# r3fang/alignTools.C

Hardware: AMD Instinct MI355X
Metric: GCUPS (DP cell updates/s), SW affine-gap 150bp pairs (higher is better)
Workload: dtype int16; 1 GPU; C2: local affine-gap, 100000 x (150x150 bp) pairs per GPU, uniform ACGT, m=2 u=-2 o=-5 e=-2, scores+tracebacks+rendered strings; pairs_per_gpu=100000, l1=150, l2=150, bits_per_base=2, streams=3, parallelism=pairs sharded over 1 GPU(s), one process per GPU

## Files before the change

aligntools/c_amd/csrc/at_hip.hip:

```cpp
#include "at_launch.h"
#include "at_classes.h"
#include "at_ragplan.h"
#include "at_pack.hip.h"
#include "at_render.hip.h"
#include "at_myers.hip.h"
#include "at_search.hip.h"
#include "at_revcomp.hip.h"
#include "at_cigar.hip.h"
#include "at_edit_tb.hip.h"
#include "at_infix.hip.h"
#include "at_scan.hip.h"
#include "at_scanhits.hip.h"
#include "at_pairhits.hip.h"
#include "../../../include/aligntools_hip.h"

#include <algorithm>
#include <chrono>
#include <condition_variable>
#include <mutex>
#include <cstdarg>
#include <cstdio>
#include <cstdlib>
#include <cstring>
#include <functional>
// ... 921 lines not shown
			HIP_TRY(h, hipGetLastError());
			snprintf(h->cfg, sizeof h->cfg, "myers-infix bits=2 words/lane=%d (64 pairs/wave) lds=%zuB waves/cu<=%d grid=%lld", w, lds, occ, grid);
			return AT_OK;
		}
		if (!d_ops || !d_ops_off || !d_nops) return fail(h, AT_ERR_ARG, "traceback wanted but ops buffers are NULL");
		const long long slab_words = (long long)std::max(max_len2, 1) * w * 128;
		const long long cap = env_ll("AT_WS_CAP_MB", 16384) << 20;
		if (slab_words * 4 > cap)
			return fail(h, AT_ERR_NOMEM, "edit infix alignments: one work item needs %lld workspace bytes (cap %lld)", slab_words * 4, cap);
		const long long per_cu = std::max(1LL, std::min<long long>(occ, env_ll("AT_WAVES_PER_CU", 16)));
		const long long grid = std::max(1LL, std::min<long long>(std::min<long long>((npairs + 63) / 64, per_cu * h->ncu), cap / (slab_words * 4)));
		{
			void *p = h->d_ws; size_t have = h->ws_bytes;
			int rc = grow(h, &p, &have, (size_t)(grid * slab_words * 4), "ws");
			h->d_ws = (uint32_t *)p; h->ws_bytes = have;
			if (rc) return rc;
		}
		ia.ops = d_ops; ia.ops_off = (const long long *)d_ops_off;
		ia.slab = h->d_ws; ia.slab_words = slab_words;
		ia.anchor_end = h->infix_anchor;
		if (int rcq = ensure_queue(h, stream)) return rcq;
		ia.m.queue = h->d_queue;
		hipLaunchKernelGGL(fn, dim3((unsigned)grid), dim3(64), lds, stream, ia);
		HIP_TRY(h, hipGetLastError());
		snprintf(h->cfg, sizeof h->cfg, "myers-infix-tb bits=2 words/lane=%d (64 pairs/wave) lds=%zuB slab=%lldB waves/cu<=%lld grid=%lld", w, lds,
		         slab_words * 4, per_cu, grid);
		return AT_OK;
	}

	int thresh16 = 0, ts = 0;
	if (!uniform_shape && !rag && !only_if && ap_n == 0 && npairs >= 4096 && !d_order && kmode <= at::K_FITJ &&
	    env_ll("AT_AUTO_UNIFORM", 1) && (bits == 8 || scores_fit_byte(h, mode)) &&
	    packed_ok(h, mode, bits, max_len1, max_len2, 4, &thresh16)) {
		int *flag = h->d_rflag + 8;
		HIP_TRY(h, hipMemsetAsync(flag, 0xff, 4, stream));
		const unsigned cg = (unsigned)std::min<int64_t>((npairs + 255) / 256, 4LL * h->ncu);
		hipLaunchKernelGGL(at::at_check_uniform, dim3(cg), dim3(256), 0, stream, d_len1, d_len2, (long long)npairs, max_len1, max_len2, flag);
		int rc = align_device(h, mode, npairs, d_seq, bits, d_woff1, d_len1, d_woff2, d_len2, max_len1, max_len2, 1, want_traceback,
		                      d_score, d_end_i, d_end_j, d_state, d_ops, d_ops_off, d_nops, stream_, 0, 0, nullptr, 0, flag, -1);
		if (rc) return rc;
		std::string packed_cfg = h->cfg;
		rc = align_device(h, mode, npairs, d_seq, bits, d_woff1, d_len1, d_woff2, d_len2, max_len1, max_len2, 0, want_traceback,
		                  d_score, d_end_i, d_end_j, d_state, d_ops, d_ops_off, d_nops, stream_, 0, 0, nullptr, 0, flag, 0);
		if (rc) return rc;
		snprintf(h->cfg, sizeof h->cfg, "auto: [%.140s] if every pair is %dx%d, else [%.120s]", packed_cfg.c_str(), max_len1, max_len2,
		         std::string(h->cfg).c_str());
		return AT_OK;
	}
	if ((uniform_shape || rag) && ap_n == 0) {
		if (packed_ok(h, mode, bits, max_len1, max_len2, 4, &thresh16)) ts = 4;
		else if ((!rag || kmode == at::K_OVERLAP) && packed_ok(h, mode, bits, max_len1, max_len2, 2, &thresh16)) ts = 2;
		if (kmode == at::K_OVERLAP && (!tb || getenv("AT_NO_PACKED_OVERLAP"))) ts = 0;
	}
	if (rag && (!ts || (kmode > at::K_FITJ && !(kmode == at::K_OVERLAP && rag == 64)) || max_len1 > at::rag_group_top(rag) || !d_order))
		return fail(h, AT_ERR_ARG, "ragged packed launch outside its domain");
	Layout16 P;
	if (ts) {
		P = layout16_for(tb, kmode == at::K_FITJ, max_len1, max_len2, ts, rag, kmode == at::K_OVERLAP, kmode,
		                 rag && kmode == at::K_OVERLAP ? at::class_rows(at::kClassOvl, max_len1) : 0);
		const double min_rounds = getenv("AT_PACKED_MIN_ROUNDS") ? atof(getenv("AT_PACKED_MIN_ROUNDS")) : 1.0;
		if (!rag && P.g == 64 && (double)((npairs + 1) / 2) < min_rounds * 12.0 * h->ncu) ts = 0;
		if (P.words >= (1LL << 24)) { if (rag) return fail(h, AT_ERR_ARG, "ragged packed launch outside its domain (slot too large)"); ts = 0; }
		Layout16 PTq = P;
		const bool tailq = !rag && !only_if && P.g <= 16 && kmode != at::K_OVERLAP && env_ll("AT_TAIL_SPLIT", 1);
		if (tailq) PTq = layout16_for(tb, kmode == at::K_FITJ, max_len1, max_len2, ts, at::AT_TAIL_G, false, kmode, at::at_tail_k(P.g, P.k));
		if (ts && !packed16_kernel_exists(kmode, P, tb, ts, bits, rag, tailq ? &PTq : nullptr)) {
			if (rag) return fail(h, AT_ERR_ARG, "ragged packed launch outside its domain (frame too long for LDS)");
			ts = 0;
		}
	}
	bool two_pass = false;
	int tp_split = 0;
	const char *ck_note = "";
	const long long tp_mode = env_ll("AT_TWO_PASS", 1);
	if (ts && tb && !rag && kmode <= at::K_FITJ && tp_mode) {
		Layout16 P2 = layout16_for(false, kmode == at::K_FITJ, max_len1, max_len2, ts, 0, false, kmode, 0, 1);
		const bool narrow_default = P2.g == 8 && tp_split_narrow_default(kmode, max_len1, max_len2);
		const bool split_default = P2.g == 64 || narrow_default;
		const bool split_want = env_ll("AT_TP_SPLIT", split_default ? 1 : 0) && at_pick_walk16(kmode, P2.g, P2.k, ts, bits);
		const int split_req = split_want && !h->ck_alloc_failed && !h->ck_skip ? 1 : 0;
		if (split_want && !split_req) ck_note = h->ck_skip ? " [one work item's checkpoints exceed AT_CK_CAP_MB: no separate pass 2]"
		                                                   : " [checkpoint buffer unavailable on this handle: no separate pass 2]";
		if ((P2.g == 64 || tp_mode >= 2 || (split_req && narrow_default)) && (long long)P2.g * P2.k >= max_len1 && at_pick16_tp(kmode, P2.g, P2.k, ts, bits) &&
		    choose_store(P2.off_ptr, 1, true) == 1) {
			two_pass = true;
			tp_split = split_req;
			if (tp_split) P2 = layout16_for(false, kmode == at::K_FITJ, max_len1, max_len2, ts, 0, false, kmode, 0, 2);
			P = P2;
		}
	}
	if (ts) {
		const int per_wave = 2 * (64 / P.g);
		const bool tail_ok = !rag && !only_if && P.g <= 16 && kmode != at::K_OVERLAP && env_ll("AT_TAIL_SPLIT", 1) &&
		                     (!tp_split || P.g == 8);
		Layout16 PT = P;
		if (tail_ok) PT = layout16_for(tb && !two_pass, kmode == at::K_FITJ, max_len1, max_len2, ts, at::AT_TAIL_G, false, kmode, at::at_tail_k(P.g, P.k), two_pass ? (tp_split ? 2 : 1) : 0);
		TpLayout tpm{}, tpt{};
		if (two_pass) { tpm = tp_layout(P, kmode, max_len2, tp_split != 0); tpt = tp_layout(PT, kmode, max_len2, tp_split != 0); }
		int64_t piece = npairs;
		int64_t brow_words = 0;
		if (tp_split) {
			const long long cap = env_ll("AT_CK_CAP_MB", 8192) << 20;
			brow_words = (tpm.brow_words + 63) & ~63LL;
			const long long tail_reserve = tail_ok ? 16LL * h->ncu * tpt.words * 4 : 0;
			const long long items = (cap - tail_reserve - brow_words * 4) / (tpm.words * 4 + 16LL * per_wave);
			if (items < 1) {
				struct SkipForThisCall {
					at_handle *h;
					explicit SkipForThisCall(at_handle *hh) : h(hh) { h->ck_skip = true; }
					~SkipForThisCall() { h->ck_skip = false; }
				} skip(h);
				return align_device(h, mode, npairs, d_seq, bits, d_woff1, d_len1, d_woff2, d_len2, max_len1, max_len2, uniform_shape, want_traceback,
				                    d_score, d_end_i, d_end_j, d_state, d_ops, d_ops_off, d_nops, stream_, ap_n, ap_first, d_order, rag, only_if, only_val);
			}
			piece = std::min<int64_t>(npairs, items * per_wave);
			const long long forced = env_ll("AT_CK_PIECE_PAIRS", 0);
			if (forced > 0) piece = std::min<int64_t>(piece, std::max<long long>(1, forced / per_wave) * per_wave);
		}
		auto walk_lane_words = [&](const Layout16 &L) -> long long {
			const int cb = at::ck_steps(L.g);
			return L.k * (cb / 4) + (kmode == at::K_FITJ ? (L.k + 3) / 4 * (cb / 4) : 0);
		};
		auto walk_lds = [&](const Layout16 &L, bool ptr_in_lds) -> size_t {
			const int cb = at::ck_steps(L.g), nsm = kmode == at::K_FITJ ? L.nsm : 0;
			return (size_t)((nsm + 1) / 2 * 2 + (L.k > 16 ? 0 : (cb + 1) * 128) + (ptr_in_lds ? 64 * walk_lane_words(L) : 0)) * 4;
		};
		std::string cfg_first, walk_last;
		for (int64_t first = 0; first < npairs; first += piece) {
		const int64_t np = std::min<int64_t>(piece, npairs - first);
		Sweep16Args b;
		memset(&b, 0, sizeof b);
		b.npairs = np; b.seq = d_seq;
		b.woff1 = (const long long *)d_woff1 + first; b.woff2 = (const long long *)d_woff2 + first;
		b.len1 = d_len1 + first; b.len2 = d_len2 + first;
		b.l1 = max_len1; b.l2 = max_len2;
		const int sc = 1 << ts;
		b.m16 = h->m * sc; b.u16 = h->u * sc; b.o16 = h->o * sc; b.e16 = h->e * sc; b.g16 = h->j * sc; b.thresh16 = thresh16;
		if (kmode == at::K_FITJ) {
			int rcs = ensure_sitemask(h, max_len2, stream);
			if (rcs) return rcs;
			b.sitemask = h->d_sitemask;
		}
		b.score = d_score + first; b.end_i = d_end_i ? d_end_i + first : nullptr; b.end_j = d_end_j ? d_end_j + first : nullptr;
		b.state = d_state ? d_state + first : nullptr;
		b.ops = d_ops; b.ops_off = d_ops_off ? (const long long *)d_ops_off + first : nullptr; b.nops = d_nops ? d_nops + first : nullptr;
		b.order = rag ? d_order : nullptr;
		b.only_if = only_if; b.only_val = only_val;
		b.off_refb = P.off_refb; b.off_bound = P.off_bound; b.ptr_lanes = P.ptr_lanes; b.off_sm = P.off_sm; b.nsm = P.nsm;
		Plan pl;
		char tag16[128];
		snprintf(tag16, sizeof tag16, "packed16 x%d bits=%d %dx%d-lane groups (%d pairs/wave)%s", 1 << ts, bits, 64 / P.g, P.g, per_wave,
		         rag ? " ragged frames" : "");
		if (two_pass) snprintf(tag16 + strlen(tag16), sizeof tag16 - strlen(tag16), " two-pass%s ck=%d", tp_split ? " (walk kernel)" : "", at::ck_steps(P.g));
		auto pick = [&](int st) {
			if (two_pass) return st == 1 ? at_pick16_tp(kmode, P.g, P.k, ts, bits, tp_split) : (at_sweep16_fn) nullptr;
			return rag ? at_pick16_rag(kmode, P.g, P.k, st, tb, bits) : at_pick16(kmode, P.g, P.k, ts, st, tb, bits);
		};
		const long long nwork = (np + per_wave - 1) / per_wave;
		int rc = plan_launch(h, tag16, P.k, nwork, std::max(P.off_ptr, PT.off_ptr),
		                     tp_split ? 64 : two_pass ? std::max(tpm.words, tpt.words) : std::max(P.words - P.off_ptr, PT.words - PT.off_ptr), &pl, stream,
		                     [&](int st) { return (const void *)pick(st); }, P.g < 64 || rag || two_pass);
		if (rc) return rc;
		if (tp_split) {
			const long long rsv = env_ll("AT_TP_RESERVE", 0) * h->ncu;
			if (rsv > 0 && pl.grid > rsv && nwork > pl.grid - rsv) {
				pl.grid = std::max<long long>(h->ncu, pl.grid - rsv);
				cfg_append(h, " (AT_TP_RESERVE: sweep grid=%lld)", pl.grid);
			}
		}
		int64_t n_tail = 0;
		if (tail_ok && nwork > pl.grid) {
			const long long sliver = nwork % pl.grid;
			if (sliver > 0 && sliver * 4 <= pl.grid) n_tail = np - (nwork - sliver) * per_wave;
		}
		Sweep16Args bt = b;
		bt.npairs = 0;
		const int64_t nm = np - n_tail;
		if (n_tail > 0) {
			b.npairs = nm;
			bt.npairs = n_tail;
			bt.woff1 += nm; bt.woff2 += nm; bt.len1 += nm; bt.len2 += nm;
			bt.score += nm;
			if (bt.end_i) bt.end_i += nm;
			if (bt.end_j) bt.end_j += nm;
			if (bt.state) bt.state += nm;
			if (bt.ops_off) bt.ops_off += nm;
			if (bt.nops) bt.nops += nm;
			bt.off_refb = PT.off_refb; bt.off_bound = PT.off_bound; bt.ptr_lanes = PT.ptr_lanes; bt.off_sm = PT.off_sm; bt.nsm = PT.nsm;
		}
		b.off_ptr = pl.off_ptr; b.ws = pl.ws; b.ws_slot_words = pl.slot_words; b.queue = h->d_queue;
		bt.off_ptr = pl.store == 1 ? 0 : PT.off_ptr; bt.ws = pl.ws; bt.ws_slot_words = pl.slot_words; bt.queue = h->d_queue;
		if (two_pass) {
			if (pl.store != 1) return fail(h, AT_ERR_RANGE, "two-pass tracebacks need the s2 windows in LDS (store=%d)", pl.store);
			b.off_brow = tpm.off_brow; b.off_rck = tpm.off_rck; b.off_cck = tpm.off_cck; b.off_rptr = tpm.off_rptr; b.off_rjpl = tpm.off_rjpl;
			bt.off_brow = tpt.off_brow; bt.off_rck = tpt.off_rck; bt.off_cck = tpt.off_cck; bt.off_rptr = tpt.off_rptr; bt.off_rjpl = tpt.off_rjpl;
		}
		if (tp_split) {
			const long long n_main_items = (nm + per_wave - 1) / per_wave, n_tail_items = (n_tail + 2 * (64 / at::AT_TAIL_G) - 1) / (2 * (64 / at::AT_TAIL_G));
			const long long end_words = ((np * 4) + 63) & ~63LL;
			const size_t need = (size_t)(brow_words + end_words + n_main_items * tpm.words + n_tail_items * tpt.words) * 4;
			void *pc = h->d_ck; size_t have = h->ck_bytes;
			const std::string err_before = h->err, g_err_before = g_err;
			rc = grow(h, &pc, &have, need, "ck");
			h->d_ck = (uint32_t *)pc; h->ck_bytes = have;
			if (rc && first == 0) {
				h->ck_alloc_failed = true;
				rc = align_device(h, mode, npairs, d_seq, bits, d_woff1, d_len1, d_woff2, d_len2, max_len1, max_len2, uniform_shape, want_traceback,
				                  d_score, d_end_i, d_end_j, d_state, d_ops, d_ops_off, d_nops, stream_, ap_n, ap_first, d_order, rag, only_if, only_val);
				if (rc == AT_OK) {
					snprintf(h->err, sizeof h->err, "%s", err_before.c_str());
					snprintf(g_err, sizeof g_err, "%s", g_err_before.c_str());
				}
				return rc;
			}
			if (rc) return rc;
			b.ck_brow = h->d_ck; bt.ck_brow = h->d_ck;
			b.tp_end = (int4 *)(h->d_ck + brow_words); bt.tp_end = b.tp_end + nm;
			b.ck = h->d_ck + brow_words + end_words; b.ck_item_words = tpm.words;
			bt.ck = b.ck + n_main_items * tpm.words; bt.ck_item_words = tpt.words;
		}
		at_sweep16_fn fn16 = pick(pl.store);
		if (!fn16 || (P.g != 64 && pl.store == 2)) return fail(h, AT_ERR_RANGE, "no packed kernel for this shape (rows/lane=%d, store=%d)", P.k, pl.store);
		if (pl.dyn_lds > 48 * 1024)
			HIP_TRY(h, hipFuncSetAttribute((const void *)fn16, hipFuncAttributeMaxDynamicSharedMemorySize, (int)pl.dyn_lds));
		hipLaunchKernelGGL(fn16, dim3((unsigned)pl.grid), dim3(64), pl.dyn_lds, stream, b, bt);
		HIP_TRY(h, hipGetLastError());
		if (tp_split && !(AT_DIAG_SWEEP_ONLY && env_ll("AT_DIAG_NO_WALK_KERNEL", 0))) {
			const bool teams = env_ll("AT_WALK_TEAMS", P.g == 64 ? 1 : 0) && at_pick_walk16(kmode, P.g, P.k, ts, bits, 1);
			at_walk16_fn wf = at_pick_walk16(kmode, P.g, P.k, ts, bits, teams);
			if (!wf) return fail(h, AT_ERR_RANGE, "no walk kernel for %d-lane groups x %d rows", P.g, P.k);
			const size_t lds = std::max(walk_lds(P, true), tail_ok ? walk_lds(PT, true) : 0);
			if (lds > 48 * 1024) HIP_TRY(h, hipFuncSetAttribute((const void *)wf, hipFuncAttributeMaxDynamicSharedMemorySize, (int)lds));
			const long long wcap = env_ll("AT_WALK_WAVES_PER_CU", 0);
			const long long wmain = std::max<long long>(1, wcap > 0 ? std::min<long long>((nm + 127) / 128, wcap * h->ncu) : (nm + 127) / 128);
			HIP_TRY(h, hipMemsetAsync(h->d_queue + 8, 0, 16, stream));
			const int tpw = 64 / at_walk16_team_lanes(P.g);
			const long long wteams = ((nm + 1) / 2 + tpw - 1) / tpw;
			hipLaunchKernelGGL(wf, dim3((unsigned)((teams ? wteams : wmain) + (n_tail + 127) / 128)), dim3(64), lds, stream, b, bt);
			char wnote[128];
			snprintf(wnote, sizeof wnote, " [walkers: %lld wavefronts%s for %lld alignments]", teams ? wteams : wmain, teams ? " of teams" : "", (long long)nm);
			cfg_append(h, "%s", wnote);
			walk_last = wnote;
			HIP_TRY(h, hipGetLastError());
		}
		if (n_tail > 0)
			cfg_append(h, " + last %lld pairs as 32-lane items (rows/lane=%d)", (long long)n_tail, PT.k);
		if (first == 0) cfg_first = h->cfg;
		}
		if (piece < npairs) snprintf(h->cfg, sizeof h->cfg, "%.360s; in pieces of %lld pairs%s%s", cfg_first.c_str(), (long long)piece,
		                              walk_last.empty() ? "" : "; last piece", walk_last.c_str());
		if (ck_note[0]) cfg_append(h, "%s", ck_note);
		return AT_OK;
	}

	if (edit_tb) {
		const size_t lds = at::myers_window_bytes(64, max_len2);
		if (h->u != 1) return fail(h, AT_ERR_DOMAIN, "edit alignments need the unit mismatch cost: u = %d, not 1", h->u);
		if (bits != 2) return fail(h, AT_ERR_DOMAIN, "edit alignments need a 2-bit batch: some base is not one of ACGT");
		if (max_len1 > 1024) return fail(h, AT_ERR_DOMAIN, "edit alignments: max_len1 = %d exceeds 1024", max_len1);
		if (lds > 60 * 1024) return fail(h, AT_ERR_DOMAIN, "edit alignments: max_len2 = %d exceeds 3792 (64 windows of packed words in 60 KB of LDS)", max_len2);
		const int w = at::class_rows(at::kMyersLaneWords, max_len1);
		at_edit_tb_fn fn = at_pick_edit_tb(w);
		if (!fn) return fail(h, AT_ERR_ARG, "no edit alignment kernel for %d words per lane", w);
		const long long slab_words = (long long)std::max(max_len2, 1) * w * 128;
		const long long cap = env_ll("AT_WS_CAP_MB", 16384) << 20;
		if (slab_words * 4 > cap)
			return fail(h, AT_ERR_NOMEM, "edit alignments: one work item needs %lld workspace bytes (cap %lld)", slab_words * 4, cap);
		int occ = 0;
		if (hipOccupancyMaxActiveBlocksPerMultiprocessor(&occ, (const void *)fn, 64, lds) != hipSuccess || occ <= 0) occ = 8;
		const long long per_cu = std::max(1LL, std::min<long long>(occ, env_ll("AT_WAVES_PER_CU", 16)));
		const long long grid = std::max(1LL, std::min<long long>(std::min<long long>((npairs + 63) / 64, per_cu * h->ncu), cap / (slab_words * 4)));
		{
			void *p = h->d_ws; size_t have = h->ws_bytes;
			int rc = grow(h, &p, &have, (size_t)(grid * slab_words * 4), "ws");
			h->d_ws = (uint32_t *)p; h->ws_bytes = have;
			if (rc) return rc;
		}
		at::EditTbArgs ea;
		memset(&ea, 0, sizeof ea);
		ea.m.npairs = npairs; ea.m.seq = d_seq;
		ea.m.woff1 = (const long long *)d_woff1; ea.m.woff2 = (const long long *)d_woff2; ea.m.len1 = d_len1; ea.m.len2 = d_len2;
		ea.m.max_l1 = max_len1; ea.m.max_l2 = max_len2;
		ea.m.score = d_score; ea.m.end_i = d_end_i; ea.m.end_j = d_end_j; ea.m.state = d_state; ea.m.nops = d_nops;
		ea.m.order = d_order;
		ea.ops = d_ops; ea.ops_off = (const long long *)d_ops_off;
		ea.slab = h->d_ws; ea.slab_words = slab_words;
		if (int rcq = ensure_queue(h, stream)) return rcq;
		ea.m.queue = h->d_queue;
		hipLaunchKernelGGL(fn, dim3((unsigned)grid), dim3(64), lds, stream, ea);
		HIP_TRY(h, hipGetLastError());
		snprintf(h->cfg, sizeof h->cfg, "myers-tb bits=2 words/lane=%d (64 pairs/wave) lds=%zuB slab=%lldB waves/cu<=%lld grid=%lld", w, lds,
		         slab_words * 4, per_cu, grid);
		return AT_OK;
	}

	auto myers_windows = [&](int n) { return at::myers_window_bytes(n, max_len2); };
	if (kmode == at::K_EDIT && h->u == 1 && bits == 2 && max_len1 <= 32768 && myers_windows(2) <= 60 * 1024 && env_ll("AT_MYERS", 1)) {
		const long long lane_max = env_ll("AT_MYERS_LANE_MAX", 1024);
		const bool per_lane = max_len1 <= lane_max && max_len1 <= 1024 && myers_windows(64) <= 60 * 1024 &&
		                      (max_len1 <= 256 || npairs >= env_ll("AT_MYERS_LANE_MIN_PAIRS", 16384)) && env_ll("AT_MYERS_GROUP", 1) == 1;
		const int g = per_lane ? 1 : max_len1 <= 256 && myers_windows(8) <= 60 * 1024 ? 8 : 32;
		const int w = per_lane ? at::class_rows(at::kMyersLaneWords, max_len1) : at::class_rows(at::kMyersGroupWords, max_len1);
		at_myers_fn fn = at_pick_myers(w, g);
		const int per_wave = 64 / g;
		at::MyersArgs m;
		memset(&m, 0, sizeof m);
		m.npairs = npairs; m.seq = d_seq;
		m.woff1 = (const long long *)d_woff1; m.woff2 = (const long long *)d_woff2; m.len1 = d_len1; m.len2 = d_len2;
		m.max_l1 = max_len1; m.max_l2 = max_len2;
// ... 1940 lines not shown
```

aligntools/c_amd/csrc/at_k16.hip:

```cpp
#include "at_launch.h"
#define AT_DECL(b)                                                                 \
	at_sweep16_fn at_pick16_g64_ts4_b##b(int kmode, int k, int store, bool tb);    \
	at_sweep16_fn at_pick16_g64_ts2_b##b(int kmode, int k, int store, bool tb);    \
	at_sweep16_fn at_pick16_g16_b##b(int kmode, int k, int store, bool tb);        \
	at_sweep16_fn at_pick16_g32_b##b(int kmode, int k, int store, bool tb);        \
	at_sweep16_fn at_pick16_g8_b##b(int kmode, int k, int store, bool tb);         \
	at_sweep16_fn at_pick16_g4_b##b(int kmode, int k, int store, bool tb);         \
	at_sweep16_fn at_pick16_rag_impl_b##b(int k, int store, bool tb);                \
	at_sweep16_fn at_pick16_rag8a_b##b(int kmode, int k, int store, bool tb);      \
	at_sweep16_fn at_pick16_rag8b_b##b(int kmode, int k, int store, bool tb);      \
	at_sweep16_fn at_pick16_rag8c_b##b(int kmode, int k, int store, bool tb);      \
	at_sweep16_fn at_pick16_rag8d_b##b(int kmode, int k, int store, bool tb);      \
	at_sweep16_fn at_pick16_rag16_b##b(int kmode, int k, int store, bool tb);      \
	at_sweep16_fn at_pick16_rag16b_b##b(int kmode, int k, int store, bool tb);     \
	at_sweep16_fn at_pick16_rag32_b##b(int kmode, int k, int store, bool tb);      \
	at_sweep16_fn at_pick16_ragovl_b##b(int k, int store);                           \
	at_sweep16_fn at_pick16_tp8_b##b(int kmode, int k, int split);                             \
	at_sweep16_fn at_pick16_tp64_b##b(int kmode, int k, int ts, int split);                  \
	at_walk16_fn at_pick_walk16_g8_b##b(int kmode, int g, int k, bool teams);                    \
	at_walk16_fn at_pick_walk16_g64_b##b(int kmode, int k, int ts, bool teams);
AT_DECL(2)
AT_DECL(8)
#undef AT_DECL
at_sweep16_fn at_pick16(int kmode, int g, int k, int ts, int store, bool tb, int bits)
{
	if (g == 8) return ts != 4 ? nullptr : bits == 8 ? at_pick16_g8_b8(kmode, k, store, tb) : at_pick16_g8_b2(kmode, k, store, tb);
	if (g == 4) return ts != 4 ? nullptr : bits == 8 ? at_pick16_g4_b8(kmode, k, store, tb) : at_pick16_g4_b2(kmode, k, store, tb);
	if (g == 32) return ts != 4 ? nullptr : bits == 8 ? at_pick16_g32_b8(kmode, k, store, tb) : at_pick16_g32_b2(kmode, k, store, tb);
	if (bits == 8) {
		if (g == 16) return ts == 4 ? at_pick16_g16_b8(kmode, k, store, tb) : nullptr;
		return ts == 4 ? at_pick16_g64_ts4_b8(kmode, k, store, tb) : at_pick16_g64_ts2_b8(kmode, k, store, tb);
	}
	if (g == 16) return ts == 4 ? at_pick16_g16_b2(kmode, k, store, tb) : nullptr;
	return ts == 4 ? at_pick16_g64_ts4_b2(kmode, k, store, tb) : at_pick16_g64_ts2_b2(kmode, k, store, tb);
}
at_sweep16_fn at_pick16_rag(int kmode, int g, int k, int store, bool tb, int bits)
{
	if (g == 8) {
		if (k == 6 || k == 8) return bits == 8 ? at_pick16_rag8d_b8(kmode, k, store, tb) : at_pick16_rag8d_b2(kmode, k, store, tb);
		if (bits == 8) return k >= 19 ? at_pick16_rag8c_b8(kmode, k, store, tb) : k >= 13 ? at_pick16_rag8b_b8(kmode, k, store, tb) : at_pick16_rag8a_b8(kmode, k, store, tb);
		return k >= 19 ? at_pick16_rag8c_b2(kmode, k, store, tb) : k >= 13 ? at_pick16_rag8b_b2(kmode, k, store, tb) : at_pick16_rag8a_b2(kmode, k, store, tb);
	}
	if (kmode == at::K_OVERLAP) return g != 64 || !tb ? nullptr : bits == 8 ? at_pick16_ragovl_b8(k, store) : at_pick16_ragovl_b2(k, store);
	if (g == 32) return bits == 8 ? at_pick16_rag32_b8(kmode, k, store, tb) : at_pick16_rag32_b2(kmode, k, store, tb);
	if (g != 16) return nullptr;
	if (k >= 16) return bits == 8 ? at_pick16_rag16b_b8(kmode, k, store, tb) : at_pick16_rag16b_b2(kmode, k, store, tb);
	if (kmode == at::K_LOCAL) return bits == 8 ? at_pick16_rag_impl_b8(k, store, tb) : at_pick16_rag_impl_b2(k, store, tb);
	return bits == 8 ? at_pick16_rag16_b8(kmode, k, store, tb) : at_pick16_rag16_b2(kmode, k, store, tb);
}
at_sweep16_fn at_pick16_tp(int kmode, int g, int k, int ts, int bits, int split)
{
	if (g == 8) return ts != 4 ? nullptr : bits == 8 ? at_pick16_tp8_b8(kmode, k, split) : at_pick16_tp8_b2(kmode, k, split);
	if (g == 64) return bits == 8 ? at_pick16_tp64_b8(kmode, k, ts, split) : at_pick16_tp64_b2(kmode, k, ts, split);
	return nullptr;
}
int at_walk16_team_lanes_b2();
int at_walk16_team_lanes8_b2();
int at_walk16_team_lanes(int g) { return g == 64 ? at_walk16_team_lanes_b2() : at_walk16_team_lanes8_b2(); }
at_walk16_fn at_pick_walk16(int kmode, int g, int k, int ts, int bits, int teams)
{
	if (g == 64) return bits == 8 ? at_pick_walk16_g64_b8(kmode, k, ts, teams != 0) : at_pick_walk16_g64_b2(kmode, k, ts, teams != 0);
	if (ts != 4) return nullptr;
	return bits == 8 ? at_pick_walk16_g8_b8(kmode, g, k, teams != 0) : at_pick_walk16_g8_b2(kmode, g, k, teams != 0);
}
```

aligntools/c_amd/csrc/at_k16_g16a.hip:

```cpp
#include "at_launch.h"
template <int MODE, int K>
static at_sweep16_fn q3(int store, bool tb)
{
	if (!tb) return at::at_sweep16<MODE, 16, K, 4, true, true, false, false, AT_BITS16>;
	if (store == 0) return at::at_sweep16<MODE, 16, K, 4, true, true, true, false, AT_BITS16>;
	return at::at_sweep16<MODE, 16, K, 4, true, false, true, false, AT_BITS16>;
}
template <int MODE>
static at_sweep16_fn q2(int k, int store, bool tb)
{
	switch (k) {
	case 4: return q3<MODE, 4>(store, tb);
	case 5: return q3<MODE, 5>(store, tb);
	case 6: return q3<MODE, 6>(store, tb);
	case 7: return q3<MODE, 7>(store, tb);
	default: return nullptr;
	}
}
at_sweep16_fn AT_NAME(at_pick16_g16a)(int kmode, int k, int store, bool tb)
{
	switch (kmode) {
	case at::K_GLOBAL: return q2<at::K_GLOBAL>(k, store, tb);
	case at::K_LOCAL: return q2<at::K_LOCAL>(k, store, tb);
	case at::K_FITJ: return q2<at::K_FITJ>(k, store, tb);
	default: return q2<at::K_FIT>(k, store, tb);
	}
}
```

aligntools/c_amd/csrc/at_k16_g16b.hip:

```cpp
#include "at_launch.h"
template <int MODE, int K>
static at_sweep16_fn q3(int store, bool tb)
{
	if (!tb) return at::at_sweep16<MODE, 16, K, 4, true, true, false, false, AT_BITS16>;
	if (store == 0) return at::at_sweep16<MODE, 16, K, 4, true, true, true, false, AT_BITS16>;
	return at::at_sweep16<MODE, 16, K, 4, true, false, true, false, AT_BITS16>;
}
template <int MODE>
static at_sweep16_fn q2(int k, int store, bool tb)
{
	switch (k) {
	case 10: return q3<MODE, 10>(store, tb);
	case 13: return q3<MODE, 13>(store, tb);
	default: return nullptr;
	}
}
at_sweep16_fn AT_NAME(at_pick16_g16b)(int kmode, int k, int store, bool tb)
{
	switch (kmode) {
	case at::K_GLOBAL: return q2<at::K_GLOBAL>(k, store, tb);
	case at::K_LOCAL: return q2<at::K_LOCAL>(k, store, tb);
	case at::K_FITJ: return q2<at::K_FITJ>(k, store, tb);
	default: return q2<at::K_FIT>(k, store, tb);
	}
}
```

aligntools/c_amd/csrc/at_k16_g16c.hip:

```cpp
#include "at_launch.h"
template <int MODE, int K>
static at_sweep16_fn r3(bool tb)
{
	if (!tb) return at::at_sweep16<MODE, 16, K, 4, true, true, false, false, AT_BITS16>;
	return at::at_sweep16<MODE, 16, K, 4, true, false, true, false, AT_BITS16>;
}
template <int MODE>
static at_sweep16_fn r2(int k, bool tb)
{
	switch (k) {
	case 16: return r3<MODE, 16>(tb);
	case 19: return r3<MODE, 19>(tb);
	default: return nullptr;
	}
}
at_sweep16_fn AT_NAME(at_pick16_g16c)(int kmode, int k, int store, bool tb)
{
	if (tb && store != 1) return nullptr;
	switch (kmode) {
	case at::K_GLOBAL: return r2<at::K_GLOBAL>(k, tb);
	case at::K_LOCAL: return r2<at::K_LOCAL>(k, tb);
	case at::K_FITJ: return r2<at::K_FITJ>(k, tb);
	default: return r2<at::K_FIT>(k, tb);
	}
}
```

aligntools/c_amd/csrc/at_k16_g32.hip:

```cpp
#include "at_launch.h"
template <int MODE, int K>
static at_sweep16_fn g3(int store, bool tb)
{
	if (!tb) return at::at_sweep16<MODE, 32, K, 4, true, true, false, false, AT_BITS16>;
	if (store == 0) return at::at_sweep16<MODE, 32, K, 4, true, true, true, false, AT_BITS16>;
	return at::at_sweep16<MODE, 32, K, 4, true, false, true, false, AT_BITS16>;
}
template <int MODE>
static at_sweep16_fn g2(int k, int store, bool tb)
{
	switch (k) {
	case 7: return g3<MODE, 7>(store, tb);
	case 8: return g3<MODE, 8>(store, tb);
	case 10: return g3<MODE, 10>(store, tb);
	case 13: return g3<MODE, 13>(store, tb);
	default: return nullptr;
	}
}
at_sweep16_fn AT_NAME(at_pick16_g32b)(int kmode, int k, int store, bool tb);
at_sweep16_fn AT_NAME(at_pick16_g32)(int kmode, int k, int store, bool tb)
{
	if (k == 12 || k >= 16) return AT_NAME(at_pick16_g32b)(kmode, k, store, tb);
	switch (kmode) {
	case at::K_GLOBAL: return g2<at::K_GLOBAL>(k, store, tb);
	case at::K_LOCAL: return g2<at::K_LOCAL>(k, store, tb);
	case at::K_FITJ: return g2<at::K_FITJ>(k, store, tb);
	default: return g2<at::K_FIT>(k, store, tb);
	}
}
```

aligntools/c_amd/csrc/at_k16_g32b.hip:

```cpp
#include "at_launch.h"
template <int MODE, int K>
static at_sweep16_fn s3(bool tb)
{
	if (!tb) return at::at_sweep16<MODE, 32, K, 4, true, true, false, false, AT_BITS16>;
	return at::at_sweep16<MODE, 32, K, 4, true, false, true, false, AT_BITS16>;
}
template <int MODE>
static at_sweep16_fn s2(int k, bool tb)
{
	switch (k) {
	case 12: return s3<MODE, 12>(tb);
	case 16: return s3<MODE, 16>(tb);
	case 19: return s3<MODE, 19>(tb);
	default: return nullptr;
	}
}
at_sweep16_fn AT_NAME(at_pick16_g32b)(int kmode, int k, int store, bool tb)
{
	if (tb && store != 1) return nullptr;
	switch (kmode) {
	case at::K_GLOBAL: return s2<at::K_GLOBAL>(k, tb);
	case at::K_LOCAL: return s2<at::K_LOCAL>(k, tb);
	case at::K_FITJ: return s2<at::K_FITJ>(k, tb);
	default: return s2<at::K_FIT>(k, tb);
	}
}
```

aligntools/c_amd/csrc/at_k16_g4.hip:

```cpp
#include "at_launch.h"
template <int MODE, int K>
static at_sweep16_fn f3(bool tb)
{
	if (!tb) return at::at_sweep16<MODE, 4, K, 4, true, true, false, false, AT_BITS16>;
	return at::at_sweep16<MODE, 4, K, 4, true, false, true, false, AT_BITS16>;
}
template <int MODE>
static at_sweep16_fn f2(int k, bool tb)
{
	switch (k) {
	case 9: return f3<MODE, 9>(tb);
	case 10: return f3<MODE, 10>(tb);
	case 13: return f3<MODE, 13>(tb);
	default: return nullptr;
	}
}
at_sweep16_fn AT_NAME(at_pick16_g4b)(int kmode, int k, int store, bool tb);
at_sweep16_fn AT_NAME(at_pick16_g4)(int kmode, int k, int store, bool tb)
{
	if (k >= 16) return AT_NAME(at_pick16_g4b)(kmode, k, store, tb);
	if (tb && store != 1) return nullptr;
	switch (kmode) {
	case at::K_GLOBAL: return f2<at::K_GLOBAL>(k, tb);
	case at::K_LOCAL: return f2<at::K_LOCAL>(k, tb);
	case at::K_FITJ: return f2<at::K_FITJ>(k, tb);
	default: return f2<at::K_FIT>(k, tb);
	}
}
```

aligntools/c_amd/csrc/at_k16_g4b.hip:

```cpp
#include "at_launch.h"
template <int MODE, int K>
static at_sweep16_fn f3(bool tb)
{
	if (!tb) return at::at_sweep16<MODE, 4, K, 4, true, true, false, false, AT_BITS16>;
	return at::at_sweep16<MODE, 4, K, 4, true, false, true, false, AT_BITS16>;
}
template <int MODE>
static at_sweep16_fn f2(int k, bool tb)
{
	switch (k) {
	case 16: return f3<MODE, 16>(tb);
	case 19: return f3<MODE, 19>(tb);
	default: return nullptr;
	}
}
at_sweep16_fn AT_NAME(at_pick16_g4b)(int kmode, int k, int store, bool tb)
{
	if (tb && store != 1) return nullptr;
	switch (kmode) {
	case at::K_GLOBAL: return f2<at::K_GLOBAL>(k, tb);
	case at::K_LOCAL: return f2<at::K_LOCAL>(k, tb);
	case at::K_FITJ: return f2<at::K_FITJ>(k, tb);
	default: return f2<at::K_FIT>(k, tb);
	}
}
```

aligntools/c_amd/csrc/at_k16_g64.hip:

```cpp
#include "at_launch.h"
template <int MODE, int K>
static at_sweep16_fn p3(int store, bool tb)
{
	if (!tb) return store < 2 ? at::at_sweep16<MODE, 64, K, 4, true, true, false, false, AT_BITS16> : at::at_sweep16<MODE, 64, K, 4, false, false, false, false, AT_BITS16>;
	if (store == 0) return at::at_sweep16<MODE, 64, K, 4, true, true, true, false, AT_BITS16>;
	if (store == 1) return at::at_sweep16<MODE, 64, K, 4, true, false, true, false, AT_BITS16>;
	return at::at_sweep16<MODE, 64, K, 4, false, false, true, false, AT_BITS16>;
}
template <int MODE>
static at_sweep16_fn p2(int k, int store, bool tb)
{
	switch (k) {
	case 1: return p3<MODE, 1>(store, tb);
	case 2: return p3<MODE, 2>(store, tb);
	case 3: return p3<MODE, 3>(store, tb);
	default: return p3<MODE, 4>(store, tb);
	}
}
at_sweep16_fn AT_NAME(at_pick16_g64_ts4)(int kmode, int k, int store, bool tb)
{
	switch (kmode) {
	case at::K_GLOBAL: return p2<at::K_GLOBAL>(k, store, tb);
	case at::K_LOCAL: return p2<at::K_LOCAL>(k, store, tb);
	case at::K_FITJ: return p2<at::K_FITJ>(k, store, tb);
	default: return p2<at::K_FIT>(k, store, tb);
	}
}
```

aligntools/c_amd/csrc/at_k16_g8a.hip:

```cpp
#include "at_launch.h"
template <int MODE, int K>
static at_sweep16_fn h3(bool tb)
{
	if (!tb) return at::at_sweep16<MODE, 8, K, 4, true, true, false, false, AT_BITS16>;
	return at::at_sweep16<MODE, 8, K, 4, true, false, true, false, AT_BITS16>;
}
template <int MODE>
static at_sweep16_fn h2(int k, bool tb)
{
	switch (k) {
	case 5: return h3<MODE, 5>(tb);
	case 7: return h3<MODE, 7>(tb);
	case 10: return h3<MODE, 10>(tb);
	default: return nullptr;
	}
}
at_sweep16_fn AT_NAME(at_pick16_g8a)(int kmode, int k, int store, bool tb)
{
	if (tb && store != 1) return nullptr;
	switch (kmode) {
	case at::K_GLOBAL: return h2<at::K_GLOBAL>(k, tb);
	case at::K_LOCAL: return h2<at::K_LOCAL>(k, tb);
	case at::K_FITJ: return h2<at::K_FITJ>(k, tb);
	default: return h2<at::K_FIT>(k, tb);
	}
}
```

aligntools/c_amd/csrc/at_k16_g8b.hip:

```cpp
#include "at_launch.h"
template <int MODE, int K>
static at_sweep16_fn h3(bool tb)
{
	if (!tb) return at::at_sweep16<MODE, 8, K, 4, true, true, false, false, AT_BITS16>;
	return at::at_sweep16<MODE, 8, K, 4, true, false, true, false, AT_BITS16>;
}
template <int MODE>
static at_sweep16_fn h2(int k, bool tb)
{
	switch (k) {
	case 13: return h3<MODE, 13>(tb);
	case 16: return h3<MODE, 16>(tb);
	default: return nullptr;
	}
}
at_sweep16_fn AT_NAME(at_pick16_g8b)(int kmode, int k, int store, bool tb)
{
	if (tb && store != 1) return nullptr;
	switch (kmode) {
	case at::K_GLOBAL: return h2<at::K_GLOBAL>(k, tb);
	case at::K_LOCAL: return h2<at::K_LOCAL>(k, tb);
	case at::K_FITJ: return h2<at::K_FITJ>(k, tb);
	default: return h2<at::K_FIT>(k, tb);
	}
}
```

aligntools/c_amd/csrc/at_k16_g8c.hip:

```cpp
#include "at_launch.h"
template <int MODE, int K>
static at_sweep16_fn h3(bool tb)
{
	if (!tb) return at::at_sweep16<MODE, 8, K, 4, true, true, false, false, AT_BITS16>;
	return at::at_sweep16<MODE, 8, K, 4, true, false, true, false, AT_BITS16>;
}
template <int MODE>
static at_sweep16_fn h2(int k, bool tb)
{
	switch (k) {
	case 19: return h3<MODE, 19>(tb);
	default: return nullptr;
	}
}
at_sweep16_fn AT_NAME(at_pick16_g8c)(int kmode, int k, int store, bool tb)
{
	if (tb && store != 1) return nullptr;
	switch (kmode) {
	case at::K_GLOBAL: return h2<at::K_GLOBAL>(k, tb);
	case at::K_LOCAL: return h2<at::K_LOCAL>(k, tb);
	case at::K_FITJ: return h2<at::K_FITJ>(k, tb);
	default: return h2<at::K_FIT>(k, tb);
	}
}
```

aligntools/c_amd/csrc/at_k16_g8d.hip:

```cpp
#include "at_launch.h"
template <int MODE, int K>
static at_sweep16_fn h3(bool tb)
{
	if (!tb) return at::at_sweep16<MODE, 8, K, 4, true, true, false, false, AT_BITS16>;
	return at::at_sweep16<MODE, 8, K, 4, true, false, true, false, AT_BITS16>;
}
template <int MODE>
static at_sweep16_fn h2(int k, bool tb)
{
	switch (k) {
	case 6: return h3<MODE, 6>(tb);
	case 8: return h3<MODE, 8>(tb);
	default: return nullptr;
	}
}
at_sweep16_fn AT_NAME(at_pick16_g8d)(int kmode, int k, int store, bool tb)
{
	if (tb && store != 1) return nullptr;
	switch (kmode) {
	case at::K_GLOBAL: return h2<at::K_GLOBAL>(k, tb);
	case at::K_LOCAL: return h2<at::K_LOCAL>(k, tb);
	case at::K_FITJ: return h2<at::K_FITJ>(k, tb);
	default: return h2<at::K_FIT>(k, tb);
	}
}
```

aligntools/c_amd/csrc/at_k16_rag.hip:

```cpp
#include "at_launch.h"
template <int K>
static at_sweep16_fn r3(int store, bool tb)
{
	if (!tb) return at::at_sweep16<at::K_LOCAL, 16, K, 4, true, true, false, true, AT_BITS16>;
	if (store == 0) return at::at_sweep16<at::K_LOCAL, 16, K, 4, true, true, true, true, AT_BITS16>;
	return at::at_sweep16<at::K_LOCAL, 16, K, 4, true, false, true, true, AT_BITS16>;
}
at_sweep16_fn AT_NAME(at_pick16_rag_impl)(int k, int store, bool tb)
{
	switch (k) {
	case 4: return r3<4>(store, tb);
	case 5: return r3<5>(store, tb);
	case 6: return r3<6>(store, tb);
	case 7: return r3<7>(store, tb);
	case 10: return r3<10>(store, tb);
	case 13: return r3<13>(store, tb);
	default: return nullptr;
	}
}
```

aligntools/c_amd/csrc/at_k16_rag16b.hip:

```cpp
#include "at_launch.h"
template <int MODE, int K>
static at_sweep16_fn x3(bool tb)
{
	if (!tb) return at::at_sweep16<MODE, 16, K, 4, true, true, false, true, AT_BITS16>;
	return at::at_sweep16<MODE, 16, K, 4, true, false, true, true, AT_BITS16>;
}
template <int MODE>
static at_sweep16_fn x2(int k, bool tb)
{
	switch (k) {
	case 16: return x3<MODE, 16>(tb);
	case 19: return x3<MODE, 19>(tb);
	default: return nullptr;
	}
}
at_sweep16_fn AT_NAME(at_pick16_rag16b)(int kmode, int k, int store, bool tb)
{
	if (tb && store != 1) return nullptr;
	switch (kmode) {
	case at::K_GLOBAL: return x2<at::K_GLOBAL>(k, tb);
	case at::K_LOCAL: return x2<at::K_LOCAL>(k, tb);
	case at::K_FITJ: return x2<at::K_FITJ>(k, tb);
	default: return x2<at::K_FIT>(k, tb);
	}
}
```

aligntools/c_amd/csrc/at_k16_rag32.hip:

```cpp
#include "at_launch.h"
template <int MODE, int K>
static at_sweep16_fn y3(bool tb)
{
	if (!tb) return at::at_sweep16<MODE, 32, K, 4, true, true, false, true, AT_BITS16>;
	return at::at_sweep16<MODE, 32, K, 4, true, false, true, true, AT_BITS16>;
}
template <int MODE>
static at_sweep16_fn y2(int k, bool tb)
{
	switch (k) {
	case 10: return y3<MODE, 10>(tb);
	case 12: return y3<MODE, 12>(tb);
	case 13: return y3<MODE, 13>(tb);
	case 16: if constexpr (MODE == at::K_LOCAL || MODE == at::K_GLOBAL) return y3<MODE, 16>(tb); else return nullptr;
	case 19: if constexpr (MODE == at::K_LOCAL) return y3<MODE, 19>(tb); else return nullptr;
	default: return nullptr;
	}
}
at_sweep16_fn AT_NAME(at_pick16_rag32)(int kmode, int k, int store, bool tb)
{
	if (tb && store != 1) return nullptr;
	switch (kmode) {
	case at::K_GLOBAL: return y2<at::K_GLOBAL>(k, tb);
	case at::K_LOCAL: return y2<at::K_LOCAL>(k, tb);
	case at::K_FITJ: return y2<at::K_FITJ>(k, tb);
	default: return y2<at::K_FIT>(k, tb);
	}
}
at_sweep16_fn AT_NAME(at_pick16_ragovl)(int k, int store)
{
	if (store != 1) return nullptr;
	if (k == 16) return at::at_sweep16<at::K_OVERLAP, 64, 16, 2, true, false, true, true, AT_BITS16>;
	if (k == 4) return at::at_sweep16<at::K_OVERLAP, 64, 4, 2, true, false, true, true, AT_BITS16>;
	return nullptr;
}
```

aligntools/c_amd/csrc/at_k16_tp.hip:

```cpp
#include "at_launch.h"
template <int MODE>
static at_sweep16_fn tp8(int k, int split)
{
	if (k != 19) return nullptr;
	return split ? at::at_sweep16<MODE, 8, 19, 4, true, false, false, false, AT_BITS16, at::ck_steps(8), 1>
	             : at::at_sweep16<MODE, 8, 19, 4, true, false, false, false, AT_BITS16, at::ck_steps(8)>;
}
at_sweep16_fn AT_NAME(at_pick16_tp8)(int kmode, int k, int split)
{
	switch (kmode) {
	case at::K_GLOBAL: return tp8<at::K_GLOBAL>(k, split);
	case at::K_LOCAL: return tp8<at::K_LOCAL>(k, split);
	case at::K_FITJ: return tp8<at::K_FITJ>(k, split);
	default: return tp8<at::K_FIT>(k, split);
	}
}
```

aligntools/c_amd/csrc/at_k16_tp64.hip:

```cpp
#include "at_launch.h"
template <int MODE, int TS>
static at_sweep16_fn tp64(int k, int split)
{
	switch (k) {
	case 16: return split ? at::at_sweep16<MODE, 64, 16, TS, true, false, false, false, AT_BITS16, at::ck_steps(64), 1>
	                      : at::at_sweep16<MODE, 64, 16, TS, true, false, false, false, AT_BITS16, at::ck_steps(64)>;
	default: return nullptr;
	}
}
at_sweep16_fn AT_NAME(at_pick16_tp64)(int kmode, int k, int ts, int split)
{
	if (ts == 2) {
		switch (kmode) {
		case at::K_GLOBAL: return tp64<at::K_GLOBAL, 2>(k, split);
		case at::K_LOCAL: return tp64<at::K_LOCAL, 2>(k, split);
		case at::K_FIT: return tp64<at::K_FIT, 2>(k, split);
		default: return nullptr;
		}
	}
	switch (kmode) {
	case at::K_GLOBAL: return tp64<at::K_GLOBAL, 4>(k, split);
	case at::K_LOCAL: return tp64<at::K_LOCAL, 4>(k, split);
	case at::K_FITJ: return tp64<at::K_FITJ, 4>(k, split);
	default: return tp64<at::K_FIT, 4>(k, split);
	}
}
```

aligntools/c_amd/csrc/at_launch.h:

```cpp
#pragma once
#include "at_sweep16.hip.h"

typedef void (*at_sweep_fn)(const at::SweepArgs);
typedef void (*at_sweep16_fn)(const at::Sweep16Args, const at::Sweep16Args);
namespace at { struct MyersArgs; }
typedef void (*at_myers_fn)(const at::MyersArgs);
at_myers_fn at_pick_myers(int w, int g);
at_myers_fn at_pick_myers_semi(int w);

at_sweep_fn at_pick32_b2(int kmode, int k, int store, bool tb);
at_sweep_fn at_pick32_b8(int kmode, int k, int store, bool tb);
at_sweep16_fn at_pick16_rag(int kmode, int g, int k, int store, bool tb, int bits);
at_sweep16_fn at_pick16(int kmode, int g, int k, int ts, int store, bool tb, int bits);
at_sweep16_fn at_pick16_tp(int kmode, int g, int k, int ts, int bits, int split = 0);
typedef void (*at_walk16_fn)(const at::Sweep16Args, const at::Sweep16Args);
at_walk16_fn at_pick_walk16(int kmode, int g, int k, int ts, int bits, int teams = 0);
int at_walk16_team_lanes(int g);
#ifndef AT_BITS16
#define AT_BITS16 2
#endif
#define AT_CAT_(a, b) a##b
#define AT_CAT(a, b) AT_CAT_(a, b)
#define AT_NAME(f) AT_CAT(f, AT_CAT(_b, AT_BITS16))

template <int MODE, int BITS, int K>
static at_sweep_fn at_pick3(int store, bool tb)
{
	if constexpr (MODE == at::K_EDIT) {
		return store < 2 ? at::at_sweep<MODE, BITS, K, true, true, false> : at::at_sweep<MODE, BITS, K, false, false, false>;
	} else {
		if (!tb) return store < 2 ? at::at_sweep<MODE, BITS, K, true, true, false> : at::at_sweep<MODE, BITS, K, false, false, false>;
		if (store == 0) return at::at_sweep<MODE, BITS, K, true, true, true>;
		if (store == 1) return at::at_sweep<MODE, BITS, K, true, false, true>;
		return at::at_sweep<MODE, BITS, K, false, false, true>;
	}
}
template <int MODE, int BITS>
static at_sweep_fn at_pick2(int k, int store, bool tb)
{
	if constexpr (MODE == at::K_OVERLAP || MODE == at::K_EDIT) {
		if (!tb || MODE == at::K_EDIT) {
			if (k == 8) return store < 2 ? at::at_sweep<MODE, BITS, 8, true, true, false> : at::at_sweep<MODE, BITS, 8, false, false, false>;
			if (k == 16) return store < 2 ? at::at_sweep<MODE, BITS, 16, true, true, false> : at::at_sweep<MODE, BITS, 16, false, false, false>;
		}
	}
	switch (k) {
	case 1: return at_pick3<MODE, BITS, 1>(store, tb);
	case 2: return at_pick3<MODE, BITS, 2>(store, tb);
	case 3: return at_pick3<MODE, BITS, 3>(store, tb);
	default: return at_pick3<MODE, BITS, 4>(store, tb);
	}
}
template <int BITS>
static at_sweep_fn at_pick1(int kmode, int k, int store, bool tb)
{
	switch (kmode) {
	case at::K_GLOBAL: return at_pick2<at::K_GLOBAL, BITS>(k, store, tb);
	case at::K_LOCAL: return at_pick2<at::K_LOCAL, BITS>(k, store, tb);
	case at::K_FIT: return at_pick2<at::K_FIT, BITS>(k, store, tb);
	case at::K_FITJ: return at_pick2<at::K_FITJ, BITS>(k, store, tb);
	case at::K_OVERLAP: return at_pick2<at::K_OVERLAP, BITS>(k, store, tb);
	default: return at_pick2<at::K_EDIT, BITS>(k, store, tb);
	}
}
```

aligntools/c_amd/csrc/at_sweep16.hip.h:

```cpp
#pragma once
#include "at_sweep.hip.h"
#include <utility>

#ifndef AT_WALK_AHEAD
#define AT_WALK_AHEAD 4
#endif
#ifndef AT_DIAG_NO_WALK
#define AT_DIAG_NO_WALK 0
#endif
#ifndef AT_GLOBAL_WALK_AHEAD
#define AT_GLOBAL_WALK_AHEAD 1
#endif
#ifndef AT_LOCAL_WALK_AHEAD
#define AT_LOCAL_WALK_AHEAD 1
#endif
#ifndef AT_WALK_PRIO
#define AT_WALK_PRIO 2
#endif
#ifndef AT_JPLANE
#define AT_JPLANE 1
#endif
#ifndef AT_OVL_BITS
#define AT_OVL_BITS 2
#endif
// ... 31 lines not shown
	int4 *tp_end;
};

AT_DEV uint32_t pk2(int v) { return ((uint32_t)v & 0xffffu) | ((uint32_t)v << 16); }
AT_DEV uint32_t pminu(uint32_t a, uint32_t b)
{
	uint32_t d;
	asm("v_pk_min_u16 %0, %1, %2" : "=v"(d) : "v"(a), "v"(b));
	return d;
}
AT_DEV uint32_t pmad(uint32_t a, uint32_t b, uint32_t c)
{
	uint32_t d;
	asm("v_pk_mad_i16 %0, %1, %2, %3" : "=v"(d) : "v"(a), "v"(b), "v"(c));
	return d;
}
AT_DEV uint32_t padd(uint32_t a, uint32_t b)
{
	return __builtin_bit_cast(uint32_t, __builtin_elementwise_add_sat(__builtin_bit_cast(s16x2, a), __builtin_bit_cast(s16x2, b)));
}
AT_DEV uint32_t psub(uint32_t a, uint32_t b)
{
	return __builtin_bit_cast(uint32_t, __builtin_elementwise_sub_sat(__builtin_bit_cast(s16x2, a), __builtin_bit_cast(s16x2, b)));
}
AT_DEV uint32_t pmax(uint32_t a, uint32_t b)
{
	return __builtin_bit_cast(uint32_t, __builtin_elementwise_max(__builtin_bit_cast(s16x2, a), __builtin_bit_cast(s16x2, b)));
}
AT_DEV uint32_t pshl4(uint32_t a)
{
	return __builtin_bit_cast(uint32_t, __builtin_bit_cast(s16x2, a) << (s16x2)(4));
}
template <int N>
AT_DEV uint32_t pshln(uint32_t a)
{
	return __builtin_bit_cast(uint32_t, __builtin_bit_cast(s16x2, a) << (s16x2)(N));
}
AT_DEV uint32_t pshl8(uint32_t a)
{
	return __builtin_bit_cast(uint32_t, __builtin_bit_cast(s16x2, a) << (s16x2)(8));
}
AT_DEV uint32_t pneg(uint32_t a)
{
	return __builtin_bit_cast(uint32_t, __builtin_bit_cast(s16x2, a) >> (s16x2)(15));
}
AT_DEV int half(uint32_t v, int h) { return (int)(short)(h ? (v >> 16) : (v & 0xffffu)); }

constexpr uint32_t kClean2 = 0xfff0fff0u, kTagL2 = 0x000f000fu, kTagM2 = 0x000a000au, kTagU2 = 0x00010001u;
constexpr int kNeg16 = -32768;

template <int MODE>
AT_DEV void border16(int i, int j, int o16, int e16, int &L, int &M, int &U)
{
	if constexpr (MODE == K_GLOBAL) {
		if (i == 0 && j == 0) { L = o16; M = 0; U = o16; }
		else if (j == 0) { L = o16 + e16 * i; M = kNeg16; U = kNeg16; }
		else { L = kNeg16; M = kNeg16; U = o16 + e16 * j; }
	} else if constexpr (MODE == K_LOCAL) {
		L = 0; M = 0; U = 0;
	} else {
		if (i == 0) { L = kNeg16; M = 0; U = 0; }
		else { L = kNeg16; M = kNeg16; U = kNeg16; }
	}
}
AT_DEV int sat16(int v) { return v < -32768 ? -32768 : (v > 32767 ? 32767 : v); }

#ifndef AT_WAVES16
#define AT_WAVES16(G, K) ((G) == 8 || (G) == 4 ? ((K) >= 16 ? 2 : (K) >= 10 ? 3 : 1) : ((G) == 16 && (K) >= 16) || ((G) == 32 && (K) >= 10) ? 2 : (G) == 16 && (K) >= 10 ? 3 : 1)
#endif

template <int G>
AT_DEV uint32_t grp_up1(uint32_t old, uint32_t src)
{
	if constexpr (G == 64) return (uint32_t)__builtin_amdgcn_update_dpp((int)old, (int)src, 0x138 , 0xf, 0xf, false);
	else if constexpr (G == 32) {
		const uint32_t v = (uint32_t)__builtin_amdgcn_update_dpp((int)old, (int)src, 0x138 , 0xf, 0xf, false);
		return threadIdx.x == 32 ? old : v;
	}
	else if constexpr (G == 8) {
		const uint32_t v = (uint32_t)__builtin_amdgcn_update_dpp((int)old, (int)src, 0x111 , 0xf, 0xf, false);
		return (threadIdx.x & 15) == 8 ? old : v;
	}
	else if constexpr (G == 4) {
		const uint32_t v = (uint32_t)__builtin_amdgcn_update_dpp((int)old, (int)src, 0x111 , 0xf, 0xf, false);
		return (threadIdx.x & 3) == 0 ? old : v;
	}
	else return (uint32_t)__builtin_amdgcn_update_dpp((int)old, (int)src, 0x111 , 0xf, 0xf, false);
}

template <int PB>
AT_DEV int cell_shift(int sw)
{
	return PB == 8 ? 8 * sw : PB == 4 ? 8 * (sw & 1) + 4 * (sw >> 1) : 8 * (sw & 1) + 4 * ((sw >> 1) & 1) + 2 * (sw >> 2);
}

template <int MODE, int TS, int CK>
struct PtrTags {
	static constexpr bool XOR3 = MODE == K_LOCAL && TS == 4 && CK == 0;
	static constexpr int L = XOR3 ? 12 : TS == 4 ? 15 : 3, M = XOR3 ? 6 : TS == 4 ? 10 : 2, U = XOR3 ? 3 : 1;
};
__host__ __device__ constexpr uint32_t xor3_cell(uint32_t m, uint32_t l, uint32_t u) { return m ^ ~(l | u); }
constexpr uint32_t kXor3Lut = xor3_cell(0xf0u, 0xccu, 0xaau) & 0xffu;
static_assert(kXor3Lut == 0xe1u, "v_bitop3_b32 computes xor3_cell");
AT_DEV uint32_t xor3_cell_v(uint32_t m, uint32_t l, uint32_t u)
{
#if __has_builtin(__builtin_amdgcn_bitop3_b32)
	return __builtin_amdgcn_bitop3_b32(m, l, u, kXor3Lut);
#else
	return xor3_cell(m, l, u);
#endif
}
__host__ __device__ constexpr int xor3_next(int st, uint32_t n)
{
	const uint32_t code = (n >> 1) & 3u;
	const uint32_t m3 = (n >> 2) & ~(n >> 1) & 1u, m0 = ~(n >> 2) & (n >> 1) & 1u;
	return st == 3 ? (((n >> 3) & 1u) == m3 ? 3 : 2) : st == 2 ? (int)((0xB4u >> (2 * code)) & 3u) : ((n & 1u) == m0 ? 1 : 2);
}
__host__ __device__ constexpr uint32_t xor3_table(int st)
{
	uint32_t t = 0;
	for (uint32_t n = 0; n < 16; ++n) t |= (uint32_t)xor3_next(st, n) << (2 * n);
	return t;
}
constexpr bool xor3_proof()
{
	for (int st = 1; st <= 3; ++st)
		for (uint32_t n = 0; n < 16; ++n)
			if ((int)((xor3_table(st) >> (2 * n)) & 3u) != xor3_next(st, n | 0xabcdef00u)) return false;
	using T = PtrTags<K_LOCAL, 4, 0>;
	const uint32_t ms[4] = {(uint32_t)T::L, (uint32_t)T::M, (uint32_t)T::U, 0u}, ls[2] = {(uint32_t)T::L, (uint32_t)T::M}, us[2] = {(uint32_t)T::M, (uint32_t)T::U};
	const int mstate[4] = {3, 2, 1, 0};
	const uint32_t junk[4] = {0u, 0xfffffff0u, 0x5a5aa5a0u, 0xa5a55a50u};
	uint32_t seen = 0;
	for (int m = 0; m < 4; ++m)
		for (int l = 0; l < 2; ++l)
			for (int u = 0; u < 2; ++u)
				for (int j = 0; j < 64; ++j) {
					const uint32_t c = xor3_cell(ms[m] | junk[j & 3], ls[l] | junk[(j >> 2) & 3], us[u] | junk[j >> 4]);
					if (xor3_next(2, c) != mstate[m]) return false;
					if ((xor3_next(3, c) == 3) != (l == 0)) return false;
					if ((xor3_next(1, c) == 1) != (u == 1)) return false;
					if (xor3_next(3, c) != 3 && xor3_next(3, c) != 2) return false;
					if (xor3_next(1, c) != 1 && xor3_next(1, c) != 2) return false;
					if (j == 0) {
						if (seen & (1u << (c & 15u))) return false;
						seen |= 1u << (c & 15u);
					}
				}
	return seen == 0xffffu && T::L > T::M && T::M > T::U && T::U > 0 && T::L < 16;
}
static_assert(xor3_proof(), "XOR3 cells: the decode returns m's state, `L extended` and `U extended` for all 16 inputs");
static_assert(PtrTags<K_GLOBAL, 4, 0>::L == 15 && PtrTags<K_LOCAL, 4, 16>::M == 10 && PtrTags<K_LOCAL, 2, 0>::L == 3 && PtrTags<K_FIT, 4, 0>::U == 1, "every other family keeps its tags");

template <bool LDS, int K>
AT_DEV int pidx(int wr, int r, int lane, int NL)
{
	constexpr int KF = K / 4 * 4, KR = K - KF;
	if constexpr (LDS) return __mul24(wr * K + r, NL) + lane;
	else return r < KF ? __mul24(wr, NL * K) + __mul24(r & ~3, NL) + lane * 4 + (r & 3) : __mul24(wr, NL * K) + KF * NL + lane * KR + (r - KF);
}

#ifndef AT_TP_STATS
#define AT_TP_STATS 0
#endif
#ifndef AT_TP_ONEBODY
#define AT_TP_ONEBODY 1
#endif
#ifndef AT_CK_STEPS
#define AT_CK_STEPS 16
#endif
#ifndef AT_CK_STEPS64
#define AT_CK_STEPS64 32
#endif
#ifndef AT_TP_WAVES64
#define AT_TP_WAVES64 2
#endif
#ifndef AT_CK_W64
#define AT_CK_W64 3
#endif
constexpr int ck_steps(int g) { return g == 64 ? AT_CK_STEPS64 : AT_CK_STEPS; }
template <int MODE> constexpr int ck_es() { return 2; }
template <int MODE, int K> constexpr int ck_nq() { return ((MODE == K_FITJ ? 3 : 2) * K + 3) / 4; }
constexpr int ck_log2(int v) { return v <= 1 ? 0 : 1 + ck_log2(v / 2); }
#ifndef AT_CK_ROW_TILE
#define AT_CK_ROW_TILE 4
#endif
#ifndef AT_CK_COL_QUAD
#define AT_CK_COL_QUAD 4
#endif
template <int ES>
AT_DEV int ck_rck_word(int e, int slot_lane)
{
	constexpr int RT = AT_CK_ROW_TILE;
	const int t = e - 1;
	return e <= 0 ? slot_lane * ES : 64 * ES + ((t / RT) * 64 + slot_lane) * (RT * ES) + (t % RT) * ES;
}
template <int ES> constexpr int ck_rck_step() { return AT_CK_ROW_TILE > 1 ? ES : 64 * ES; }
template <int NQ>
AT_DEV int ck_cck_word(int c, int slot_lane, int q)
{
	constexpr int Q = AT_CK_COL_QUAD, NQQ = (NQ + Q - 1) / Q;
	return (((c * NQQ + q / Q) * 64 + slot_lane) * Q + q % Q) * 4;
}

template <int G, int K, int CB>
struct CkPattern {
	static constexpr int LCB = ck_log2(CB);
	static constexpr bool FIXED = G == 64;
	static constexpr int W = AT_CK_W64, NB = G / W;
	static constexpr int MHr = (W * CB - K) / 2, MH = MHr < 0 ? 0 : MHr > CB ? CB : MHr;
	static constexpr int MU = 3, ML = 3;
	int b, c0, thi1, horiz;
	AT_DEV void set(int ci, int cj, bool hz)
	{
		b = (ci - 1) / K;
		const int rho = (ci - 1) - b * K, T0 = cj - 1 + b;
		c0 = T0 >> LCB; thi1 = T0 - rho - 2; horiz = hz ? 1 : 0;
	}
	AT_DEV int ctop(int dr) const { return dr == 0 ? c0 : (thi1 - (dr - 1) * (K + 1) + MH) >> LCB; }
	AT_DEV void band(int dr, int &chi, int &n) const
	{
		if constexpr (FIXED) { chi = ctop(dr); n = W; }
		else {
			const int thi = thi1 - (dr - 1) * (K + 1);
			const int tlo = dr == 0 ? thi1 + 2 : thi - (K - 1);
			chi = dr == 0 ? c0 : (thi + MU) >> LCB;
			const int clo = imax((tlo - ML) >> LCB, 0);
			n = imax(chi - clo + 1, 0);
		}
	}
	AT_DEV void block(int q, int T, int &bl, int &c, bool &valid) const
	{
		bl = -1; c = 0;
		if (horiz) { bl = b; c = c0 - q; }
		else if constexpr (FIXED) { const int dr = q / W; if (dr < NB) { bl = b - dr; c = ctop(dr) - q % W; } }
		else {
			int ql = q;
			for (int dr = 0; dr <= b; ++dr) {
				int chi, n;
				band(dr, chi, n);
				if (ql < n) { bl = b - dr; c = chi - ql; break; }
				ql -= n;
			}
		}
		valid = bl >= 0 && c >= 0 && c * CB < T && (c + 1) * CB > bl;
	}
	AT_DEV int slot(int bl, int c) const
	{
		const int dr = b - bl;
		if (horiz) { const int w = c0 - c; return dr == 0 && w >= 0 && w < G ? w : -1; }
		if constexpr (FIXED) {
			if (dr < 0 || dr >= NB) return -1;
			const int w = ctop(dr) - c;
			return w >= 0 && w < W ? dr * W + w : -1;
		} else {
			if (dr < 0) return -1;
			int chi, n, s0 = 0;
			for (int d = 0; d < dr; ++d) { band(d, chi, n); s0 += n; if (s0 >= G) return -1; }
			band(dr, chi, n);
			const int w = chi - c;
			return w >= 0 && w < n && s0 + w < G ? s0 + w : -1;
		}
	}
};

template <typename F, int... Q>
AT_DEV void static_for_impl(F &f, std::integer_sequence<int, Q...>) { (f(std::integral_constant<int, Q>{}), ...); }
template <int N, typename F>
AT_DEV void static_for(F &f) { static_for_impl(f, std::make_integer_sequence<int, N>{}); }

template <int KQ>
AT_DEV int ridx(int s4, int r, int lane) { return (s4 * KQ + (r >> 2)) * 256 + lane * 4 + (r & 3); }
constexpr int ck_stage_words(int cb) { return 64 * (cb + 1) * 2; }
template <int G> constexpr int ck_walk_blocks() { return G == 64 ? 4 : 1; }
template <int MODE, int K, int CB>
constexpr int ck_walk_words() { return (K + 3) / 4 * CB + (MODE == K_FITJ ? ((K + 3) / 4 + 3) / 4 * CB : 0); }

AT_DEV uint32_t pk2h(int lo, int hi) { return ((uint32_t)lo & 0xffffu) | ((uint32_t)hi << 16); }
AT_DEV uint32_t lohi(uint32_t lo, uint32_t hi)
{
	return __builtin_amdgcn_perm(hi, lo, 0x07060100u);
}
struct ck_u3 { uint32_t x, y, z; };
template <bool HASJ>
AT_DEV uint2 ck_entry(uint32_t eL, uint32_t eM, uint32_t eU, uint32_t eJ, uint32_t e2, uint32_t o2, uint32_t tagL, uint32_t tagM, uint32_t tagU)
{
	const uint32_t tl = eL | tagL, tm = eM | tagM;
	uint32_t xx = pmax(pmax(tl, tm), eU | tagU);
	if constexpr (HASJ) xx = pmax(xx, eJ);
	return make_uint2(xx, pmax(padd(tl, e2), padd(tm, o2)));
}

#ifndef AT_REPLAY_INLINE
#define AT_REPLAY_INLINE 1
#endif
#if AT_REPLAY_INLINE
#define AT_REPLAY_FN AT_DEV
#else
#define AT_REPLAY_FN __device__ __noinline__
#endif
template <int MODE, int G, int K, int TS, bool SMALL, int BITS, int CB>
AT_REPLAY_FN void replay16_block(const Sweep16Args &a, const Slot<SMALL> &mem, uint32_t *gs, const int refoff,
                           const uint32_t *qA, const uint32_t *qB, const int l1A, const int l1B,
                           const int blA, const int cA, const int blB, const int cB)
{
	constexpr bool HASJ = MODE == K_FITJ;
	static_assert(!HASJ || (TS == 4 && AT_JPLANE), "two-pass jump state: scores x16, 4-bit cells + bit plane");
	static_assert(MODE == K_GLOBAL || MODE == K_LOCAL || MODE == K_FIT || MODE == K_FITJ, "two-pass tracebacks: the affine modes");
	static_assert(CB % 4 == 0, "pointer words hold 4 steps");
	constexpr int TMASK = (1 << TS) - 1;
	constexpr int TGL = TS == 4 ? 15 : 3, TGM = TS == 4 ? 10 : 2, TGU = 1;
	constexpr int KG = (K + 3) / 4, ES = ck_es<MODE>(), NQ = ck_nq<MODE, K>();
	constexpr int PADW = kPad / 4;
	(void)PADW;
	const int lane = threadIdx.x, grp = lane / G;
	const int o16 = a.o16, e16 = a.e16;
	uint32_t o2 = pk2(o16), e2 = pk2(e16);
	uint32_t lut_lo = ((uint32_t)a.m16 & 0xffu) | (((uint32_t)a.u16 & 0xffu) * 0x01010100u);
	uint32_t lut_hi = (((uint32_t)a.m16 >> 8) & 0xffu) | ((((uint32_t)a.u16 >> 8) & 0xffu) * 0x01010100u);
	uint32_t cClean = (uint32_t)(0xffff & ~TMASK) * 0x00010001u, cTagM = (uint32_t)TGM * 0x00010001u;
	uint32_t cTagL = (uint32_t)TGL * 0x00010001u, cTagU = (uint32_t)TGU * 0x00010001u;
	uint32_t cM3 = 0x00030003u, cM7 = 0x00070007u, cF0 = 0x00f000f0u, cF000 = 0xf000f000u, c8888 = 0x88888888u;
	uint32_t gmo2 = pk2(a.g16 - a.o16), neg2 = 0x80008000u;
	uint32_t c1 = 0x00010001u, umm2 = pk2(a.u16 - a.m16), m2 = pk2(a.m16);
	asm volatile("" : "+v"(c8888), "+v"(gmo2), "+v"(neg2), "+v"(c1), "+v"(umm2), "+v"(m2));
	asm volatile("" : "+v"(o2), "+v"(e2), "+v"(lut_lo), "+v"(lut_hi));
	asm volatile("" : "+v"(cClean), "+v"(cTagM), "+v"(cTagL), "+v"(cTagU), "+v"(cM3), "+v"(cM7), "+v"(cF0), "+v"(cF000));

	const int orgA = imax(cA * CB, blA), orgB = imax(cB * CB, blB);
	const uint32_t mck = (cA * CB > blA ? 0x0000ffffu : 0u) | (cB * CB > blB ? 0xffff0000u : 0u);
	const int i0A = blA * K, i0B = blB * K;
	auto entA = [&](int x) { return blA == 0 ? a.off_brow + (orgA + x) * ES : a.off_rck + ck_rck_word<ES>(orgA - 1 + x, grp * G + blA - 1); };
	auto entB = [&](int x) { return blB == 0 ? a.off_brow + (orgB + x) * ES : a.off_rck + ck_rck_word<ES>(orgB - 1 + x, grp * G + blB - 1); };
	const int stg = a.off_bound + lane * 2;
	{
		static_assert(ES == 2, "row checkpoint entries: (X', L of the row below), ck_entry");
		uint2 ra[CB + 1], rb[CB + 1];
#pragma unroll
		for (int x = 0; x <= CB; ++x) { ra[x] = *(const uint2 *)(gs + entA(x)); rb[x] = *(const uint2 *)(gs + entB(x)); }
#pragma unroll
		for (int x = 0; x <= CB; ++x) mem.st2(stg + x * 128, lohi(ra[x].x, rb[x].x), lohi(ra[x].y, rb[x].y));
	}

	uint32_t Mo_l[K], U_l[K], Xl[2][K], J_l[HASJ ? K : 1], qsel[K], acc[K];
	uint32_t jA[HASJ ? KG : 1], jB[HASJ ? KG : 1];
	(void)jA; (void)jB; (void)J_l;
	uint32_t Ad, lraw0;
	{
		const uint2 e0 = mem.ld2(stg);
		Ad = e0.x; lraw0 = e0.y;
	}
	{
		const int ckA = a.off_cck, ckB = a.off_cck;
		auto put = [&](auto XC, uint32_t val) {
			constexpr int x = decltype(XC)::value;
			if constexpr (x < K) Mo_l[x] = val;
			else if constexpr (x < 2 * K) U_l[x - K] = val;
			else if constexpr (HASJ && x < 3 * K) J_l[x - 2 * K] = val;
		};
		uint4 cva[NQ], cvb[NQ];
#pragma unroll
		for (int q = 0; q < NQ; ++q) { cva[q] = *(const uint4 *)(gs + ckA + ck_cck_word<NQ>(cA, grp * G + blA, q)); cvb[q] = *(const uint4 *)(gs + ckB + ck_cck_word<NQ>(cB, grp * G + blB, q)); }
		auto chunk = [&](auto QC) {
			constexpr int q = decltype(QC)::value;
			const uint4 va = cva[q], vb = cvb[q];
			put(std::integral_constant<int, 4 * q>{}, lohi(va.x, vb.x)); put(std::integral_constant<int, 4 * q + 1>{}, lohi(va.y, vb.y));
			put(std::integral_constant<int, 4 * q + 2>{}, lohi(va.z, vb.z)); put(std::integral_constant<int, 4 * q + 3>{}, lohi(va.w, vb.w));
		};
		static_for<NQ>(chunk);
		uint32_t lraw = lraw0;
		constexpr int BPW = 32 / BITS, LBP = BITS == 2 ? 4 : 2, NWQ = (K + BPW - 2) / BPW + 1;
		const int wqa = imin(i0A, l1A - 1) >> LBP, wqb = imin(i0B, l1B - 1) >> LBP;
		const int lwa = (l1A - 1) >> LBP, lwb = (l1B - 1) >> LBP;
		uint32_t qwa[NWQ], qwb[NWQ];
#pragma unroll
		for (int x = 0; x < NWQ; ++x) { qwa[x] = qA[imin(wqa + x, lwa)]; qwb[x] = qB[imin(wqb + x, lwb)]; }
#pragma unroll
		for (int r = 0; r < K; ++r) {
			const uint32_t vMo = Mo_l[r], vU = U_l[r];
			uint32_t vJ = neg2;
			if constexpr (HASJ) vJ = J_l[r];
			int La, Ma, Ua, Lb, Mb, Ub;
			border16<MODE>(i0A + r + 1, 0, o16, e16, La, Ma, Ua);
			border16<MODE>(i0B + r + 1, 0, o16, e16, Lb, Mb, Ub);
			La = sat16(La); Lb = sat16(Lb);
			const uint32_t bMo = pk2h(sat16((Ma | TGM) + o16), sat16((Mb | TGM) + o16));
			const uint32_t bU = pk2h(Ua | TGU, Ub | TGU);
			const uint32_t bX = pk2h(imax3(La | TGL, Ma | TGM, Ua | TGU), imax3(Lb | TGL, Mb | TGM, Ub | TGU));
			const uint32_t kMo = vMo | cTagM, kU = vU | cTagU;
			const uint32_t Lc = lraw | cTagL, Mc = psub(vMo, o2) | cTagM;
			uint32_t kX = pmax(pmax(Lc, Mc), kU);
			if constexpr (HASJ) kX = pmax(kX, vJ);
			lraw = pmax(padd(Lc, e2), kMo);
			Mo_l[r] = vbfi(mck, kMo, bMo);
			U_l[r] = vbfi(mck, kU, bU);
			Xl[0][r] = vbfi(mck, kX, bX);
			Xl[1][r] = Xl[0][r];
			if constexpr (HASJ) J_l[r] = vbfi(mck, vJ, neg2);
			const int qi = imin(i0A + r, l1A - 1), qj = imin(i0B + r, l1B - 1);
			const uint32_t wa = pick<NWQ>(qwa, (qi >> LBP) - wqa), wb = pick<NWQ>(qwb, (qj >> LBP) - wqb);
			uint32_t ca, cb;
			if constexpr (BITS == 2) { ca = (wa >> ((qi & 15) * 2)) & 3u; cb = (wb >> ((qj & 15) * 2)) & 3u; }
			else { ca = (wa >> ((qi & 3) * 8)) & 0xffu; cb = (wb >> ((qj & 3) * 8)) & 0xffu; }
			qsel[r] = (ca * 0x00000101u + cb * 0x01010000u) | (BITS == 2 ? 0x04000400u : 0u);
			acc[r] = 0;
		}
	}
	if constexpr (HASJ) {
#pragma unroll
		for (int g = 0; g < KG; ++g) { jA[g] = 0; jB[g] = 0; }
	}
	const int jA0 = orgA - blA, jB0 = orgB - blB;

	for (int s4 = 0; s4 < CB / 4; ++s4) {
		uint32_t wA, wB, smA = 0, smB = 0;
		{
			const int eA = jA0 + 4 * s4 + kPad, eB = jB0 + 4 * s4 + kPad;
			const int xa = refoff + (eA >> 2), xb = refoff + a.off_refb + (eB >> 2);
			const uint32_t a0 = mem.ld(xa), a1 = mem.ld(xa + 1), b0 = mem.ld(xb), b1 = mem.ld(xb + 1);
			wA = __builtin_amdgcn_alignbit(a1, a0, (eA & 3) * 8);
			wB = __builtin_amdgcn_alignbit(b1, b0, (eB & 3) * 8);
		}
		if constexpr (HASJ) {
			const int eA = jA0 + 4 * s4 + 1 + 64, eB = jB0 + 4 * s4 + 1 + 64;
			smA = __builtin_amdgcn_alignbit(mem.ld(a.off_sm + (eA >> 5) + 1), mem.ld(a.off_sm + (eA >> 5)), eA & 31);
			smB = __builtin_amdgcn_alignbit(mem.ld(a.off_sm + (eB >> 5) + 1), mem.ld(a.off_sm + (eB >> 5)), eB & 31);
		}
		auto step = [&](auto KC) {
			constexpr int k = decltype(KC)::value;
			constexpr uint32_t SELK = (uint32_t)k * 0x00000101u + (uint32_t)(4 + k) * 0x01010000u;
			const uint2 eup = mem.ld2(stg + (1 + 4 * s4 + k) * 128);
			const uint32_t Aup = eup.x, Bup = eup.y;
			uint32_t gopen = neg2;
			if constexpr (HASJ) gopen = lohi(((smA >> k) & 1u) ? gmo2 : neg2, ((smB >> k) & 1u) ? gmo2 : neg2);
			const uint32_t selw = __builtin_amdgcn_perm(wB, wA, SELK);
			uint32_t diag = Ad, lraw = Bup, jn = 0;
			(void)jn;
#pragma unroll
			for (int r = 0; r < K; ++r) {
				uint32_t S;
				if constexpr (BITS == 2) S = __builtin_amdgcn_perm(lut_hi, lut_lo, selw ^ qsel[r]);
				else S = pmad(pminu(selw ^ qsel[r], c1), umm2, m2);
				uint32_t Mraw = padd(diag, S);
				if constexpr (MODE == K_LOCAL) Mraw = pmax(Mraw, 0u);
				const uint32_t Mc = vandor(Mraw, cClean, cTagM);
				const uint32_t Lc = lraw | cTagL;
				const uint32_t Uraw = pmax(Mo_l[r], padd(U_l[r], e2));
				const uint32_t Uc = vandor(Uraw, cClean, cTagU);
				const uint32_t Mo = padd(Mc, o2);
				uint32_t Xo = pmax(pmax(Lc, Mc), Uc);
				uint32_t Jraw = 0;
				if constexpr (HASJ) {
					Jraw = pmax(padd(Mo_l[r], gopen), J_l[r]);
					const uint32_t Jc = Jraw & cClean;
					Xo = pmax(Xo, Jc);
					J_l[r] = Jc;
				}
				const uint32_t Ld = pmax(padd(Lc, e2), Mo);
				uint32_t c;
				if constexpr (TS == 4) c = vbfi(cM7, vbfi(cM3, Mraw, lraw), Uraw);
				else c = vbfi(cM7, vbfi(cM3, Mraw, pshln<2>(lraw)), pshln<3>(Uraw));
				if constexpr (HASJ) {
					const int q = r & 3, gq = r >> 2;
					if (q == 0) jn = Jraw;
					else if (q == 1) jn = __builtin_amdgcn_perm(Jraw, jn, 0x06020400u);
					else if (q == 2) jn = vbfi(cF0, pshln<4>(Jraw), jn);
					else jn = vbfi(cF000, pshln<12>(Jraw), jn);
					if (q == 3 || r == K - 1) {
						if (q == 0) jn &= 0x000f000fu; else if (q == 1) jn &= 0x0f0f0f0fu; else if (q == 2) jn &= 0x0fff0fffu;
						if constexpr (k == 0) jA[gq] = jn;
						else if constexpr (k == 1) jA[gq] = vbfi(c8888, jn, jA[gq]);
						else if constexpr (k == 2) jB[gq] = jn;
						else jB[gq] = vbfi(c8888, jn, jB[gq]);
					}
				}
				if constexpr (k == 0) acc[r] = c;
				else if constexpr (k == 1) acc[r] = __builtin_amdgcn_perm(c, acc[r], 0x06020400u);
				else if constexpr (k == 2) acc[r] = vbfi(cF0, pshln<4>(c), acc[r]);
				else acc[r] = vbfi(cF000, pshln<12>(c), acc[r]);
				diag = Xl[k & 1][r];
				Xl[(k & 1) ^ 1][r] = Xo;
				lraw = Ld;
				Mo_l[r] = Mo; U_l[r] = Uc;
			}
			Ad = Aup;
		};
		step(std::integral_constant<int, 0>{}); step(std::integral_constant<int, 1>{});
		step(std::integral_constant<int, 2>{}); step(std::integral_constant<int, 3>{});
		{
			constexpr int KQ = (K + 3) / 4;
#pragma unroll
			for (int r = 0; r < K; r += 4)
				*(uint4 *)(gs + a.off_rptr + ridx<KQ>(s4, r, lane)) = make_uint4(acc[r], r + 1 < K ? acc[r + 1 < K ? r + 1 : 0] : 0u, r + 2 < K ? acc[r + 2 < K ? r + 2 : 0] : 0u, r + 3 < K ? acc[r + 3 < K ? r + 3 : 0] : 0u);
		}
		if constexpr (HASJ) {
			constexpr int GQ = (KG + 3) / 4;
			uint32_t jO[KG];
#pragma unroll
			for (int g = 0; g < KG; ++g) jO[g] = jA[g] | (jB[g] >> 1);
#pragma unroll
			for (int g = 0; g < KG; g += 4)
				*(uint4 *)(gs + a.off_rjpl + ridx<GQ>(s4, g, lane)) = make_uint4(jO[g], g + 1 < KG ? jO[g + 1 < KG ? g + 1 : 0] : 0u, g + 2 < KG ? jO[g + 2 < KG ? g + 2 : 0] : 0u, g + 3 < KG ? jO[g + 3 < KG ? g + 3 : 0] : 0u);
		}
	}
}

template <int MODE, int G, int K, int TS, bool SMALL, bool PTRLDS, bool TB, bool RAG = false, int BITS = 2, int CK = 0, int SPLIT = 0>
AT_DEV long long sweep16_items(const Sweep16Args &a, long long wnext, const long long wbase)
{
	static_assert(!SPLIT || CK > 0, "a walk kernel follows a sweep that leaves checkpoints");
	constexpr bool TP = CK > 0;
	static_assert(!TP || (!TB && !RAG && MODE != K_OVERLAP && !PTRLDS), "two-pass tracebacks: uniform batches of the affine modes, checkpoints in the global slot");
	static_assert(BITS == 2 || BITS == 8, "sequence words: 16 two-bit codes or 4 bytes");
	static_assert(!RAG || G <= 32 || MODE == K_OVERLAP, "ragged frames: one strip (the host sizes the frame for it)");
	static_assert(MODE == K_GLOBAL || MODE == K_LOCAL || MODE == K_FIT || MODE == K_FITJ || MODE == K_OVERLAP, "packed path: the affine modes, overlap");
	constexpr bool OVL = MODE == K_OVERLAP;
	static_assert(!OVL || (TB && TS == 2), "packed overlap: scores x4 with 2-bit tags, tracebacks");
	constexpr bool HASJ = MODE == K_FITJ;
	constexpr bool ISFIT = MODE == K_FIT || MODE == K_FITJ;
	static_assert(TS == 4 || TS == 2, "scores x16 or x4");
	constexpr int TMASK = (1 << TS) - 1;
	constexpr int CS = TMASK + 1, NCH = (K + CS - 1) / CS;
	using Tags = PtrTags<MODE, TS, CK>;
	constexpr bool X3 = Tags::XOR3;
	constexpr int OTGL = Tags::L, OTGM = Tags::M, OTGU = Tags::U;
	constexpr uint32_t XT1 = xor3_table(1), XT2 = xor3_table(2), XT3 = xor3_table(3);
	constexpr int TGL = TB ? OTGL : 0, TGM = TB ? OTGM : 0, TGU = TB ? OTGU : 0;
	constexpr bool JPL = HASJ && TB && TS == 4 && AT_JPLANE;
	constexpr int KG = (K + 3) / 4;
	constexpr int PB = OVL ? AT_OVL_BITS : (HASJ && !JPL) ? 8 : 4;
	static_assert(!OVL || G == 64, "packed overlap: one 64-lane group");
	constexpr int SPW = 16 / PB;
	static_assert(G == 64 || G == 32 || G == 16 || G == 8 || G == 4, "group width");
	constexpr int NG = 64 / G;
	constexpr int BLK = G <= 16 ? 4 : 8;
	constexpr bool ONEBODY = G <= 16 || (CK > 0 && AT_TP_ONEBODY);
	constexpr int RPB = BLK / SPW;
	constexpr int RS = G * K;
	constexpr int PADW = kPad / 4;
	const int lane = threadIdx.x;
	const int grp = lane / G, lg = lane % G;
	Slot<SMALL> mem;
	mem.g = SMALL ? nullptr : a.ws + (long long)blockIdx.x * a.ws_slot_words;
	PtrStore<PTRLDS> pm;
	pm.g = PTRLDS ? nullptr : a.ws + (long long)blockIdx.x * a.ws_slot_words;
	const int l1 = a.l1, l2 = a.l2, NL = a.ptr_lanes;
	const int o16 = a.o16, e16 = a.e16;
	uint32_t o2 = pk2(a.o16), e2 = pk2(a.e16);
	const int mS = OVL ? a.m16 | 2 : a.m16, uS = OVL ? a.u16 | 2 : a.u16;
	uint32_t lut_lo = ((uint32_t)mS & 0xffu) | (((uint32_t)uS & 0xffu) * 0x01010100u);
	uint32_t lut_hi = (((uint32_t)mS >> 8) & 0xffu) | ((((uint32_t)uS >> 8) & 0xffu) * 0x01010100u);
	uint32_t oL2 = pk2(a.o16 | 3), oR2 = pk2(a.o16 | 1);
	asm volatile("" : "+v"(oL2), "+v"(oR2));
	uint32_t cClean = (uint32_t)(0xffff & ~TMASK) * 0x00010001u, cTagM = (uint32_t)TGM * 0x00010001u;
	uint32_t cTagL = (uint32_t)TGL * 0x00010001u, cTagU = (uint32_t)TGU * 0x00010001u;
	uint32_t cM3 = 0x00030003u, cM7 = 0x00070007u, cNib = 0x000f000fu, cF0 = 0x00f000f0u, cF000 = 0xf000f000u;
	uint32_t c8888 = 0x88888888u, c3333 = 0x33333333u;
	asm volatile("" : "+v"(c8888), "+v"(c3333));
	uint32_t cRTagL = (uint32_t)OTGL * 0x00010001u, cRTagM = (uint32_t)OTGM * 0x00010001u, cRTagU = (uint32_t)OTGU * 0x00010001u;
	(void)cRTagL; (void)cRTagM; (void)cRTagU;
	if constexpr (CK > 0) asm volatile("" : "+v"(cRTagL), "+v"(cRTagM), "+v"(cRTagU));
	uint32_t gmo2 = pk2(a.g16 - a.o16), neg2 = 0x80008000u;
	asm volatile("" : "+v"(gmo2), "+v"(neg2));
	uint32_t c1 = 0x00010001u, umm2 = pk2(a.u16 - a.m16), m2 = pk2(mS);
	asm volatile("" : "+v"(c1), "+v"(umm2), "+v"(m2));
	asm volatile("" : "+v"(o2), "+v"(e2), "+v"(lut_lo), "+v"(lut_hi));
	if constexpr (X3) asm volatile("" : "+v"(cClean), "+v"(cTagM), "+v"(cTagL), "+v"(cTagU), "+v"(cNib), "+v"(cF0), "+v"(cF000));
	else asm volatile("" : "+v"(cClean), "+v"(cTagM), "+v"(cTagL), "+v"(cTagU), "+v"(cM3), "+v"(cM7), "+v"(cNib), "+v"(cF0), "+v"(cF000));
	const int nstrips = (l1 + RS - 1) / RS;
	const int tbk_frame = (l2 + G - 1 + BLK - 1) / BLK;
	const int wps = tbk_frame * RPB * K;
	const int wpj = tbk_frame * (BLK / 4) * KG;
	const int jpl_base0 = a.off_ptr + __mul24(nstrips * wps, NL);
	const long long nwork = (a.npairs + 2 * NG - 1) / (2 * NG);
	const int refoff = grp * 2 * a.off_refb;
	uint32_t *gs = TP ? a.ws + (long long)blockIdx.x * a.ws_slot_words : nullptr;
	constexpr int ES = ck_es<MODE>();
	const int ck_T = tbk_frame * BLK;
	(void)gs; (void)ck_T;
	if constexpr (TP) {
		uint32_t *const brow = SPLIT ? a.ck_brow : gs + a.off_brow;
		for (int j = lane; j <= l2; j += 64) {
			int L, M, U;
			border16<MODE>(0, j, o16, e16, L, M, U);
			const uint2 en = ck_entry<HASJ>(pk2(sat16(L)), pk2(M), pk2(U), 0x80008000u, e2, o2, cRTagL, cRTagM, cRTagU);
			brow[j * ES] = en.x; brow[j * ES + 1] = en.y;
		}
	}

	while (wnext - wbase < nwork) {
		const long long wk = wnext - wbase;
		long long st_item = 0;
		(void)st_item;
		if (TP && AT_TP_STATS) st_item = (long long)__builtin_amdgcn_s_memtime();
		wnext = next_work(a.queue, lane);
		if constexpr (TP && SPLIT) gs = a.ck + wk * a.ck_item_words;
		const long long last = a.npairs - 1;
		long long pA = (wk * NG + grp) * 2 < a.npairs ? (wk * NG + grp) * 2 : last;
		long long pB = (wk * NG + grp) * 2 + 1 < a.npairs ? (wk * NG + grp) * 2 + 1 : last;
		int l1A = l1, l1B = l1, l2A = l2, l2B = l2;
		int il1 = l1, il2 = l2;
		long long pout = 0;
		bool filler = false;
		int own_len = l1 + l2;
		if constexpr (RAG) {
			const long long pc = wk * 2 * NG + lane < a.npairs ? wk * 2 * NG + lane : last;
			const int oraw = lane < 2 * NG ? a.order[pc] : 0;
			filler = oraw < 0;
			pout = filler ? (long long)~oraw : (long long)oraw;
			const int o1 = lane < 2 * NG ? a.len1[pout] : 0, o2l = lane < 2 * NG ? a.len2[pout] : 0;
			own_len = o1 + o2l;
			pA = __shfl((int)pout, 2 * grp); pB = __shfl((int)pout, 2 * grp + 1);
			l1A = __shfl(o1, 2 * grp); l1B = __shfl(o1, 2 * grp + 1);
			l2A = __shfl(o2l, 2 * grp); l2B = __shfl(o2l, 2 * grp + 1);
			int mx = o2l;
#pragma unroll
			for (int d = 1; d < 2 * NG; d <<= 1) mx = imax(mx, __shfl_xor(mx, d));
			il2 = __builtin_amdgcn_readfirstlane(mx);
			if constexpr (MODE != K_LOCAL) il1 = __builtin_amdgcn_readfirstlane(o1);
			const bool bad = lane < 2 * NG && (o1 > l1 || o2l > l2 || o1 < 1 || o2l < 1 || (MODE != K_LOCAL && o1 != il1));
			if (__any(bad)) {
				if (lane < 2 * NG && wk * 2 * NG + lane < a.npairs && !filler) {
					a.score[pout] = INT32_MIN;
					if (a.nops) a.nops[pout] = -1;
				}
				continue;
			}
		} else {
			const long long pc = wk * 2 * NG + lane;
			pout = pc;
			const bool bad = lane < 2 * NG && pc < a.npairs && (a.len1[pc] != l1 || a.len2[pc] != l2);
			if (__any(bad)) {
				if (lane < 2 * NG && pc < a.npairs) {
					a.score[pc] = INT32_MIN;
					if (a.nops) a.nops[pc] = -1;
				}
				continue;
			}
		}
		const int tbk = RAG ? (il2 + G - 1 + BLK - 1) / BLK : tbk_frame;
		const int lastlane = il1 > 0 ? ((il1 - 1) % RS) / K : 0;
		const int rl = il1 > 0 ? ((il1 - 1) % RS) % K : 0;
		const uint32_t *qA = a.seq + a.woff1[pA], *qB = a.seq + a.woff1[pB];
		const uint32_t *rA = a.seq + a.woff2[pA], *rB = a.seq + a.woff2[pB];

		{
			constexpr int BPW = 32 / BITS;
			const int nw2 = (il2 + BPW - 1) / BPW;
			const int nwA = (l2A + BPW - 1) / BPW, nwB = (l2B + BPW - 1) / BPW;
			for (int w = lg; w < nw2; w += G) {
				const uint32_t va = rA[RAG ? imin(w, nwA - 1) : w], vb = rB[RAG ? imin(w, nwB - 1) : w];
				if constexpr (BITS == 8) {
					mem.st(refoff + PADW + w, va);
					mem.st(refoff + a.off_refb + PADW + w, vb);
				} else {
#pragma unroll
					for (int q = 0; q < 4; ++q) {
						const uint32_t ba = (va >> (8 * q)) & 0xffu, bb = (vb >> (8 * q)) & 0xffu;
						mem.st(refoff + PADW + 4 * w + q, (ba & 3u) | ((ba & 0xcu) << 6) | ((ba & 0x30u) << 12) | ((ba & 0xc0u) << 18));
						mem.st(refoff + a.off_refb + PADW + 4 * w + q, (bb & 3u) | ((bb & 0xcu) << 6) | ((bb & 0x30u) << 12) | ((bb & 0xc0u) << 18));
					}
				}
			}
		}
		if constexpr (HASJ) {
			for (int w = lane; w < a.nsm; w += 64) mem.st(a.off_sm + w, a.sitemask[w]);
		}
		for (int j = lane; j <= l2; j += 64) {
			int L, M, U;
			border16<MODE>(0, j, o16, e16, L, M, U);
			int x = imax3(L | TGL, M | TGM, U | TGU);
			const int ld = imax(sat16((L | TGL) + e16), sat16((M | TGM) + o16));
			if constexpr (OVL) x = j == 0 ? 0 : kNeg16;
			mem.st2(a.off_bound + 2 * j, pk2(x), pk2(ld));
		}
		mem.sync();

		int gbi[2] = {INT32_MAX, INT32_MAX}, gbj[2] = {INT32_MAX, INT32_MAX}, gbs[2] = {INT32_MIN, INT32_MIN};
		uint32_t bestM = pk2(a.thresh16), bestMj = 0, bestL = pk2(a.thresh16), bestLj = 0;
		uint32_t capL = 0, capM = 0, capU = 0;
		uint32_t Mo_l[K], U_l[K], Xl[2][K], L_l[K], J_l[K];
		uint32_t Lrow = 0;

		for (int s = 0; s < nstrips; ++s) {
			const int base = s * RS;
			const int i0 = base + lg * K;
			const int nl = imin(G, (il1 - base + K - 1) / K);
			const bool laststrip = s == nstrips - 1;
			const bool wb = G == 64 && !laststrip;
			uint32_t qsel[K], acc[K], keymask[K];
			uint32_t accH[OVL && PB == 2 ? K : 1];
			uint32_t jA[JPL ? KG : 1], jB[JPL ? KG : 1];
			(void)accH; (void)jA; (void)jB;
			if constexpr (JPL) {
#pragma unroll
				for (int g = 0; g < KG; ++g) { jA[g] = 0; jB[g] = 0; }
			}
			const int jpl_base = jpl_base0 + __mul24(s * wpj, NL);
#pragma unroll
			for (int r = 0; r < K; ++r) {
				const int qi = imin(i0 + r, l1A - 1), qj = imin(i0 + r, l1B - 1);
				uint32_t ca, cb;
				if constexpr (BITS == 2) { ca = (qA[qi >> 4] >> ((qi & 15) * 2)) & 3u; cb = (qB[qj >> 4] >> ((qj & 15) * 2)) & 3u; }
				else { ca = (qA[qi >> 2] >> ((qi & 3) * 8)) & 0xffu; cb = (qB[qj >> 2] >> ((qj & 3) * 8)) & 0xffu; }
				qsel[r] = (ca * 0x00000101u + cb * 0x01010000u) | (BITS == 2 ? 0x04000400u : 0u);
				acc[r] = 0;
				keymask[r] = (i0 + r < l1A ? (uint32_t)(0xffff & ~TMASK) : 0u) | (i0 + r < l1B ? (uint32_t)(0xffff & ~TMASK) << 16 : 0u);
				int L, M, U;
				border16<MODE>(i0 + r + 1, 0, o16, e16, L, M, U);
				L = sat16(L);
				Mo_l[r] = pk2(sat16((M | TGM) + o16));
				U_l[r] = pk2(U | TGU);
				L_l[r] = pk2(L | TGL);
				if constexpr (ISFIT) Lrow = L_l[r];
				J_l[r] = neg2;
				Xl[0][r] = pk2(imax3(L | TGL, M | TGM, U | TGU));
				if constexpr (OVL) Xl[0][r] = 0;
				Xl[1][r] = Xl[0][r];
			}
			uint32_t ckL = 0, ckM = 0, ckU = 0, ckJ = neg2;
			int ck_p = 0;
			(void)ckL; (void)ckM; (void)ckU; (void)ckJ; (void)ck_p;
			if constexpr (TP) {
				int L, M, U;
				border16<MODE>(i0 + K, 0, o16, e16, L, M, U);
				ckL = pk2(sat16(L)); ckM = pk2(M); ckU = pk2(U);
				const int p0 = a.off_rck + ck_rck_word<ES>(0, lane);
				const uint2 en = ck_entry<HASJ>(ckL, ckM, ckU, ckJ, e2, o2, cRTagL, cRTagM, cRTagU);
				gs[p0] = en.x; gs[p0 + 1] = en.y;
			}
			uint32_t A_prev = Xl[0][K - 1], B_prev = 0, Ad;
			{
				int L, M, U;
				border16<MODE>(base, 0, o16, e16, L, M, U);
				L = sat16(L);
				Ad = pk2(imax3(L | TGL, M | TGM, U | TGU));
				if constexpr (OVL) Ad = 0;
			}
			uint32_t best[NCH], bt[NCH];
#pragma unroll
			for (int c = 0; c < NCH; ++c) { best[c] = 0x80008000u; bt[c] = 0; }
			auto load_bound = [&](int t0, uint32_t &bx, uint32_t &bl) {
				const int jn = imin(t0 + 1 + (lane & (BLK - 1)), l2);
				const uint2 v = mem.ld2(a.off_bound + 2 * jn);
				bx = v.x; bl = v.y;
			};
			uint32_t bx, bl, bxn, bln;
			load_bound(0, bx, bl);
			const int ptr_base = a.off_ptr + s * wps * NL;

			for (int blk = 0; blk < tbk; ++blk) {
				const int t0 = blk * BLK;
				if constexpr (TP) ck_p = a.off_rck + ck_rck_word<ES>(t0 + 1, lane);
				load_bound(t0 + BLK, bxn, bln);
				uint32_t wA[2], wB[2];
				{
					const int e0 = t0 - lg + kPad;
					const int w = refoff + (e0 >> 2);
					const int sh = (e0 & 3) * 8;
					const uint32_t a0 = mem.ld(w), a1 = mem.ld(w + 1);
					const uint32_t b0 = mem.ld(a.off_refb + w), b1 = mem.ld(a.off_refb + w + 1);
					wA[0] = __builtin_amdgcn_alignbit(a1, a0, sh);
					wB[0] = __builtin_amdgcn_alignbit(b1, b0, sh);
					wA[1] = 0; wB[1] = 0;
					if constexpr (BLK == 8) {
						const uint32_t a2 = mem.ld(w + 2), b2 = mem.ld(a.off_refb + w + 2);
						wA[1] = __builtin_amdgcn_alignbit(a2, a1, sh);
						wB[1] = __builtin_amdgcn_alignbit(b2, b1, sh);
					}
				}
				uint32_t sm = 0;
				if constexpr (HASJ) {
					const int e0 = t0 - lg + 1 + 64;
					const uint32_t w0 = mem.ld(a.off_sm + (e0 >> 5)), w1 = mem.ld(a.off_sm + (e0 >> 5) + 1);
					sm = __builtin_amdgcn_alignbit(w1, w0, e0 & 31);
				}
				const int jm1_0 = t0 - lg;

				auto step = [&](auto KC, auto MASKED) {
					constexpr int k = decltype(KC)::value;
					constexpr bool masked = decltype(MASKED)::value;
					constexpr int kk = k & 3, hw = k >> 2;
					constexpr uint32_t SELK = (uint32_t)kk * 0x00000101u + (uint32_t)(4 + kk) * 0x01010000u;
					const int t = t0 + k;
					uint32_t tpk = pk2(t);
					asm("" : "+v"(tpk));
					const uint32_t Aup = grp_up1<G>((uint32_t)row_shl<k>((int)bx), A_prev);
					const uint32_t Bup = grp_up1<G>((uint32_t)row_shl<k>((int)bl), B_prev);
					const int jm1 = jm1_0 + k;
					bool active = true;
					if constexpr (masked) active = lg < nl && (unsigned)jm1 < (unsigned)il2;
					if (active) {
						uint32_t gopen = neg2;
						if constexpr (HASJ) gopen = ((sm >> k) & 1u) ? gmo2 : neg2;
						if constexpr (OVL) {
							if (laststrip) {
								const uint32_t jpk = pk2(jm1);
								uint32_t vM = pick<K>(Xl[k & 1], rl);
								if constexpr (RAG) {
									const uint32_t cm = (((uint32_t)((jm1 - l2A) >> 31)) & 0xffffu) | (((uint32_t)((jm1 - l2B) >> 31)) << 16);
									vM = vbfi(cm, vM, neg2);
								}
								uint32_t dM = psub(bestM, vM);
								asm("" : "+v"(dM));
								bestMj = vbfi(pneg(dM), jpk, bestMj); bestM = pmax(bestM, vM);
							}
						}
						if constexpr (ISFIT) {
							if (laststrip) {
								const uint32_t jpk = pk2(jm1);
								uint32_t vM = psub(pick<K>(Mo_l, rl), o2);
								uint32_t vL = Lrow;
								if constexpr (RAG) {
									const uint32_t cm = (((uint32_t)((jm1 - l2A) >> 31)) & 0xffffu) | (((uint32_t)((jm1 - l2B) >> 31)) << 16);
									vM = vbfi(cm, vM, neg2); vL = vbfi(cm, vL, neg2);
								}
								uint32_t dM = psub(bestM, vM);
								asm("" : "+v"(dM));
								bestMj = vbfi(pneg(dM), jpk, bestMj); bestM = pmax(bestM, vM);
								uint32_t dL = psub(bestL, vL);
								asm("" : "+v"(dL));
								bestLj = vbfi(pneg(dL), jpk, bestLj); bestL = pmax(bestL, vL);
							}
						}
						const uint32_t selw = __builtin_amdgcn_perm(wB[hw], wA[hw], SELK);
						uint32_t diag = Ad, lraw = Bup, up = 0, cmax[NCH];
						uint32_t capmask = 0;
						if constexpr (RAG && MODE == K_GLOBAL) {
							if (lg == lastlane) capmask = (jm1 + 1 == l2A ? 0xffffu : 0u) | (jm1 + 1 == l2B ? 0xffff0000u : 0u);
						}
						uint32_t upv = Aup;
						uint32_t jn = 0;
						(void)jn;
#pragma unroll
						for (int r = 0; r < K; ++r) {
							uint32_t S;
							if constexpr (BITS == 2) {
								S = __builtin_amdgcn_perm(lut_hi, lut_lo, selw ^ qsel[r]);
							} else {
								const uint32_t z = pminu(selw ^ qsel[r], c1);
								S = pmad(z, umm2, m2);
							}
							if constexpr (OVL) {
								const uint32_t left = Xl[k & 1][r];
								const uint32_t x = pmax(pmax(padd(left, oL2), padd(diag, S)), padd(upv, oR2));
								const uint32_t Mcl = x & cClean;
								constexpr int sw = k % SPW;
								if constexpr (PB == 4) {
									if constexpr (sw == 0) acc[r] = x;
									else if constexpr (sw == 1) acc[r] = __builtin_amdgcn_perm(x, acc[r], 0x06020400u);
									else if constexpr (sw == 2) acc[r] = vbfi(cF0, pshln<4>(x), acc[r]);
									else acc[r] = vbfi(cF000, pshln<12>(x), acc[r]);
								} else {
									if constexpr (sw == 0) acc[r] = x;
									else if constexpr (sw == 1) acc[r] = __builtin_amdgcn_perm(x, acc[r], 0x06020400u);
									else if constexpr (sw == 2) acc[r] = vbfi(cF0, pshln<4>(x), acc[r]);
									else if constexpr (sw == 3) acc[r] = vbfi(cF000, pshln<12>(x), acc[r]);
									else if constexpr (sw == 4) accH[r] = x;
									else if constexpr (sw == 5) accH[r] = __builtin_amdgcn_perm(x, accH[r], 0x06020400u);
									else if constexpr (sw == 6) accH[r] = vbfi(cF0, pshln<4>(x), accH[r]);
									else accH[r] = vbfi(cF000, pshln<12>(x), accH[r]);
								}
								diag = left;
								upv = Mcl;
								up = Mcl;
								Xl[(k & 1) ^ 1][r] = Mcl;
								continue;
							}
							uint32_t Mraw = padd(diag, S);
							if constexpr (MODE == K_LOCAL) Mraw = pmax(Mraw, 0u);
							const uint32_t Mc = TB ? vandor(Mraw, cClean, cTagM) : Mraw;
							const uint32_t Lc = !TB ? lraw : X3 ? vandor(lraw, cClean, cTagL) : (lraw | cTagL);
							const uint32_t Uraw = pmax(Mo_l[r], padd(U_l[r], e2));
							const uint32_t Uc = TB ? vandor(Uraw, cClean, cTagU) : Uraw;
							const uint32_t Mo = padd(Mc, o2);
							uint32_t Xo = pmax(pmax(Lc, Mc), Uc);
							uint32_t Jraw = 0;
							if constexpr (HASJ) {
								Jraw = pmax(padd(Mo_l[r], gopen), J_l[r]);
								const uint32_t Jc = TB ? (Jraw & cClean) : Jraw;
								Xo = pmax(Xo, Jc);
								J_l[r] = Jc;
							}
							const uint32_t Ld = pmax(padd(Lc, e2), Mo);
							if (TP && r == K - 1) {
								ckL = Lc; ckM = Mc; ckU = Uc;
								if constexpr (HASJ) ckJ = J_l[r];
							}
							if constexpr (RAG && MODE == K_GLOBAL) {
								if (r == rl) { capL = vbfi(capmask, Lc, capL); capM = vbfi(capmask, Mc, capM); capU = vbfi(capmask, Uc, capU); }
							}
							if constexpr (TB) {
								uint32_t c;
								if constexpr (X3) {
									c = xor3_cell_v(Mraw, lraw, Uraw);
								} else if constexpr (TS == 4) {
									c = vbfi(cM7, vbfi(cM3, Mraw, lraw), Uraw);
								} else {
									c = vbfi(cM7, vbfi(cM3, Mraw, pshln<2>(lraw)), pshln<3>(Uraw));
								}
								if constexpr (HASJ && !JPL) c = vbfi(cNib, c, pshln<TS == 4 ? 1 : 3>(Jraw));
								if constexpr (JPL) {
									const int q = r & 3, gq = r >> 2;
									if (q == 0) jn = Jraw;
									else if (q == 1) jn = __builtin_amdgcn_perm(Jraw, jn, 0x06020400u);
									else if (q == 2) jn = vbfi(cF0, pshln<4>(Jraw), jn);
									else jn = vbfi(cF000, pshln<12>(Jraw), jn);
									if (q == 3 || r == K - 1) {
										if (q == 0) jn &= 0x000f000fu; else if (q == 1) jn &= 0x0f0f0f0fu; else if (q == 2) jn &= 0x0fff0fffu;
										constexpr int sj = k & 3;
										if constexpr (sj == 0) jA[gq] = jn;
										else if constexpr (sj == 1) jA[gq] = vbfi(c8888, jn, jA[gq]);
										else if constexpr (sj == 2) jB[gq] = jn;
										else jB[gq] = vbfi(c8888, jn, jB[gq]);
									}
								}
								constexpr int sw = k % SPW;
								if constexpr (sw == 0) acc[r] = c;
								else if constexpr (sw == 1) acc[r] = __builtin_amdgcn_perm(c, acc[r], 0x06020400u);
								else if constexpr (sw == 2) acc[r] = vbfi(cF0, pshln<4>(c), acc[r]);
								else acc[r] = vbfi(cF000, pshln<12>(c), acc[r]);
							}
							if constexpr (MODE == K_LOCAL) {
								uint32_t rt = (uint32_t)(TMASK - r % CS) * 0x00010001u;
								const uint32_t key = (Mraw & keymask[r]) | rt;
								cmax[r / CS] = r % CS == 0 ? key : pmax(cmax[r / CS], key);
							}
							diag = Xl[k & 1][r];
							Xl[(k & 1) ^ 1][r] = Xo;
							lraw = Ld;
							up = Xo;
							Mo_l[r] = Mo; U_l[r] = Uc;
							if constexpr (MODE == K_GLOBAL) L_l[r] = Lc;
							if constexpr (ISFIT) Lrow = r == rl ? Lc : Lrow;
						}
						if constexpr (MODE == K_LOCAL) {
							if constexpr (RAG) {
								const uint32_t cm = (((uint32_t)((jm1 - l2A) >> 31)) & 0xffffu) | (((uint32_t)((jm1 - l2B) >> 31)) << 16);
#pragma unroll
								for (int c = 0; c < NCH; ++c) cmax[c] = vbfi(cm, cmax[c], neg2);
							}
#pragma unroll
							for (int c = 0; c < NCH; ++c) {
								uint32_t dlt = psub(best[c], cmax[c]);
								asm("" : "+v"(dlt));
								const uint32_t g = pneg(dlt);
								bt[c] = vbfi(g, tpk, bt[c]);
								best[c] = pmax(best[c], cmax[c]);
							}
						}
						A_prev = up; B_prev = lraw;
						if (wb && lane == 63) mem.st2(a.off_bound + 2 * (jm1 + 1), up, lraw);
					}
					Ad = Aup;
					if constexpr (TP) {
						static_assert(!TP || AT_CK_ROW_TILE <= 1 || BLK % AT_CK_ROW_TILE == 0 || AT_CK_ROW_TILE % BLK == 0, "a tile of row checkpoints and a block of steps: one holds the other");
						constexpr int RT = AT_CK_ROW_TILE > 1 ? AT_CK_ROW_TILE : 1;
						constexpr int so = RT >= BLK ? k * ES : (k / RT) * 64 * RT * ES + (k % RT) * ck_rck_step<ES>();
						*(uint2 *)(gs + ck_p + so) = ck_entry<HASJ>(ckL, ckM, ckU, ckJ, e2, o2, cRTagL, cRTagM, cRTagU);
					}
					if constexpr (TB) {
						if constexpr (OVL && PB == 2) {
							if constexpr ((k + 1) % SPW == 0) {
#pragma unroll
								for (int r = 0; r < K; ++r) acc[r] = vbfi(c3333, acc[r], accH[r] << 2);
							}
						}
						if ((k + 1) % SPW == 0 && lane < NL) {
							if constexpr (PTRLDS) {
#pragma unroll
								for (int r = 0; r < K; ++r) pm.st(ptr_base + pidx<true, K>(blk * RPB + k / SPW, r, lane, NL), acc[r]);
							} else {
								const int wr = blk * RPB + k / SPW;
#pragma unroll
								for (int r = 0; r + 3 < K; r += 4)
									pm.st4(ptr_base + pidx<false, K>(wr, r, lane, NL), acc[r], acc[r + 1], acc[r + 2], acc[r + 3]);
								constexpr int R4 = K / 4 * 4;
								if constexpr (K - R4 == 3) {
									pm.st(ptr_base + pidx<false, K>(wr, R4, lane, NL), acc[R4]);
									pm.st(ptr_base + pidx<false, K>(wr, R4 + 1, lane, NL), acc[R4 + 1]);
									pm.st(ptr_base + pidx<false, K>(wr, R4 + 2, lane, NL), acc[R4 + 2]);
								} else if constexpr (K - R4 == 2) {
									pm.st2(ptr_base + pidx<false, K>(wr, R4, lane, NL), acc[R4], acc[R4 + 1]);
								} else if constexpr (K - R4 == 1) {
									pm.st(ptr_base + pidx<false, K>(wr, R4, lane, NL), acc[R4]);
								}
							}
						}
						if constexpr (JPL) {
							if ((k & 3) == 3 && lane < NL) {
								const int wr = blk * (BLK / 4) + k / 4;
								uint32_t jO[KG];
#pragma unroll
								for (int g = 0; g < KG; ++g) jO[g] = jA[g] | (jB[g] >> 1);
								if constexpr (PTRLDS) {
#pragma unroll
									for (int g = 0; g < KG; ++g) pm.st(jpl_base + pidx<true, KG>(wr, g, lane, NL), jO[g]);
								} else {
#pragma unroll
									for (int g = 0; g + 3 < KG; g += 4)
										pm.st4(jpl_base + pidx<false, KG>(wr, g, lane, NL), jO[g], jO[g + 1], jO[g + 2], jO[g + 3]);
									constexpr int G4 = KG / 4 * 4;
									if constexpr (KG - G4 == 3) {
										pm.st(jpl_base + pidx<false, KG>(wr, G4, lane, NL), jO[G4]);
										pm.st(jpl_base + pidx<false, KG>(wr, G4 + 1, lane, NL), jO[G4 + 1]);
										pm.st(jpl_base + pidx<false, KG>(wr, G4 + 2, lane, NL), jO[G4 + 2]);
									} else if constexpr (KG - G4 == 2) {
										pm.st2(jpl_base + pidx<false, KG>(wr, G4, lane, NL), jO[G4], jO[G4 + 1]);
									} else if constexpr (KG - G4 == 1) {
										pm.st(jpl_base + pidx<false, KG>(wr, G4, lane, NL), jO[G4]);
									}
								}
							}
						}
					}
				};
				using T = std::true_type;
				using F = std::false_type;
#define AT_STEPS16(M)                                                                                    \
	step(std::integral_constant<int, 0>{}, M{}); step(std::integral_constant<int, 1>{}, M{});            \
	step(std::integral_constant<int, 2>{}, M{}); step(std::integral_constant<int, 3>{}, M{});            \
	if constexpr (BLK == 8) {                                                                            \
		step(std::integral_constant<int, 4>{}, M{}); step(std::integral_constant<int, 5>{}, M{});        \
// ... 2 lines not shown
				if constexpr (ONEBODY) { AT_STEPS16(T) }
				else if (t0 >= nl - 1 && t0 + BLK <= il2) { AT_STEPS16(F) }
				else { AT_STEPS16(T) }
#undef AT_STEPS16
				bx = bxn; bl = bln;
				if constexpr (TP) {
					if ((t0 + BLK) % CK == 0) {
						constexpr int NV = HASJ ? 3 : 2, NQ = ck_nq<MODE, K>();
						const int cb = a.off_cck, cidx = (t0 + BLK) / CK;
						auto val = [&](auto XC) -> uint32_t {
							constexpr int x = decltype(XC)::value;
							if constexpr (x < K) return Mo_l[x];
							else if constexpr (x < 2 * K) return U_l[x - K];
							else if constexpr (x < NV * K) return J_l[x - 2 * K];
							else return 0u;
						};
						auto chunk = [&](auto QC) {
							constexpr int q = decltype(QC)::value;
							*(uint4 *)(gs + cb + ck_cck_word<NQ>(cidx, lane, q)) = make_uint4(val(std::integral_constant<int, 4 * q>{}), val(std::integral_constant<int, 4 * q + 1>{}),
							                                          val(std::integral_constant<int, 4 * q + 2>{}), val(std::integral_constant<int, 4 * q + 3>{}));
						};
						static_for<NQ>(chunk);
					}
				}
			}
			if constexpr (MODE == K_LOCAL) {
#pragma unroll
				for (int c = 0; c < NCH; ++c) {
#pragma unroll
					for (int h = 0; h < 2; ++h) {
						const int key = half(best[c], h);
						const int sc = key & ~TMASK;
						const int row = i0 + c * CS + (TMASK - (key & TMASK)) + 1;
						if (key != kNeg16 && row <= (h == 0 ? l1A : l1B) && sc > gbs[h]) {
							gbs[h] = sc;
							gbi[h] = row;
							gbj[h] = (int)((bt[c] >> (16 * h)) & 0xffffu) - lg + 1;
						}
					}
				}
			}
			mem.sync();
		}

		pm.ready();
		int my_sc = 0, my_ci = 0, my_cj = 0, my_st = 2;
		bool my_ok = true;
		if constexpr (MODE == K_LOCAL) {
#pragma unroll
			for (int h = 0; h < 2; ++h) {
				int bs = gbs[h], bi = gbi[h], bj = gbj[h];
				for (int d = G / 2; d >= 1; d >>= 1) {
					const int ob = __shfl_xor(bs, d), oi = __shfl_xor(bi, d), oj = __shfl_xor(bj, d);
					const bool take = ob > bs || (ob == bs && (oi < bi || (oi == bi && oj < bj)));
					if (take) { bs = ob; bi = oi; bj = oj; }
				}
				gbs[h] = bs; gbi[h] = bi; gbj[h] = bj;
			}
		}
		{
			const int h = lane & 1;
			const int glane = (lane >> 1) * G;
			const int own = (glane + lastlane) & 63;
			int sc16 = 0, ci = 0, cj = 0, st = 2;
			bool ok = true;
			auto from = [&](uint32_t v, int src) { return (uint32_t)__shfl((int)v, src & 63); };
			if constexpr (MODE == K_LOCAL) {
				const int s0 = (int)from((uint32_t)gbs[0], glane), s1 = (int)from((uint32_t)gbs[1], glane);
				const int i0 = (int)from((uint32_t)gbi[0], glane), i1 = (int)from((uint32_t)gbi[1], glane);
				const int j0 = (int)from((uint32_t)gbj[0], glane), j1 = (int)from((uint32_t)gbj[1], glane);
				sc16 = h ? s1 : s0; ci = h ? i1 : i0; cj = h ? j1 : j0;
				st = 2;
			} else if constexpr (MODE == K_GLOBAL) {
				int eL, eM, eU;
				if constexpr (RAG) {
					eL = half(from(capL, own), h);
					eM = half(from(capM, own), h);
					eU = half(from(capU, own), h);
					const int ca = (int)from((uint32_t)l2A, glane), cb = (int)from((uint32_t)l2B, glane);
					cj = h ? cb : ca;
				} else {
					eL = half(from(pick<K>(L_l, rl), own), h);
					eM = half(psub(from(pick<K>(Mo_l, rl), own), pk2(o16)), h);
					eU = half(from(pick<K>(U_l, rl), own), h);
					cj = l2;
				}
				const int x = TB ? imax3(eL, eM, eU) : imax3(eL | OTGL, eM | OTGM, eU | OTGU);
				sc16 = x; st = x & 3; ci = il1;
			} else if constexpr (OVL) {
				sc16 = half(from(bestM, own), h);
				cj = half(from(bestMj, own), h);
				ci = il1; st = 2;
				ok = sc16 > a.thresh16;
			} else {
				const int bM = half(from(bestM, own), h);
				const int jM = half(from(bestMj, own), h);
				const int bL = half(from(bestL, own), h);
				const int jL = half(from(bestLj, own), h);
				ci = il1;
				if ((bL >> TS) > (bM >> TS) && bL > a.thresh16) { sc16 = bL; st = 3; cj = jL; }
				else { sc16 = bM; st = 2; cj = jM; }
				ok = sc16 > a.thresh16;
			}
			my_sc = sc16; my_ci = ci; my_cj = cj; my_st = st; my_ok = ok;
		}
		if constexpr (TP && SPLIT) {
			const long long pin = wk * 2 * NG + lane;
			if (lane < 2 * NG && pin < a.npairs) {
				a.score[pin] = my_ok ? (my_sc >> TS) : INT32_MIN;
				if (a.end_i) a.end_i[pin] = my_ci;
				if (a.end_j) a.end_j[pin] = my_cj;
				if (a.state) a.state[pin] = my_st == 3 ? 1 : my_st == 2 ? 2 : 3;
				a.tp_end[pin] = make_int4(my_ci, my_cj, my_st, my_ok ? 1 : 0);
			}
		} else if constexpr (TP) {
			constexpr int LCB = ck_log2(CK);
			constexpr int KG2 = (K + 3) / 4;
			const int g2 = lane >> 1, h = lane & 1;
			const long long pin = wk * 2 * NG + lane;
			const bool mine = lane < 2 * NG && pin < a.npairs;
			int ci = my_ci, cj = my_cj, st = my_st, cnt = 0;
			bool ok = my_ok;
			const bool walks = mine && a.nops != nullptr;
			uint8_t *ops = walks ? a.ops + a.ops_off[pin] : nullptr;
			asm volatile("s_waitcnt vmcnt(0)" ::: "memory");
			__builtin_amdgcn_fence(__ATOMIC_ACQUIRE, "agent");
			if (AT_WALK_PRIO) __builtin_amdgcn_s_setprio(AT_WALK_PRIO);
			CkPattern<G, K, CK> pat;
			(void)KG2;
			long long st_t0 = 0, st_rep = 0, st_walk = 0;
			int st_rounds = 0, st_fetch = 0, st_iters = 0;
			(void)st_t0; (void)st_rep; (void)st_walk; (void)st_rounds; (void)st_fetch; (void)st_iters;
			if (AT_TP_STATS) st_t0 = (long long)__builtin_amdgcn_s_memtime();
			for (int rounds = 0;; ++rounds) {
				const bool fin = !walks || !ok || ci <= 0 || (!ISFIT && cj <= 0) || (MODE == K_LOCAL && st == 0) || AT_DIAG_NO_WALK;
				if (!fin && (cj <= 0 || cnt >= own_len)) ok = false;
				bool go = !fin && ok;
				if (rounds > own_len + 8) { if (go) ok = false; go = false; }
				if (!__any(go)) break;
				pat.set(go ? ci : 1, go ? cj : 1, st == 1 || (HASJ && st == 0));
				int blk_bl[2], blk_c[2];
#pragma unroll
				for (int hh = 0; hh < 2; ++hh) {
					CkPattern<G, K, CK> q;
					q.b = __shfl(pat.b, 2 * grp + hh); q.c0 = __shfl(pat.c0, 2 * grp + hh);
					q.thi1 = __shfl(pat.thi1, 2 * grp + hh); q.horiz = __shfl(pat.horiz, 2 * grp + hh);
					const int alive = __shfl(go ? 1 : 0, 2 * grp + hh);
					bool v;
					q.block(lg, ck_T, blk_bl[hh], blk_c[hh], v);
					if (!v || !alive) { blk_bl[hh] = 0; blk_c[hh] = 0; }
				}
				long long st_a = 0;
				if (AT_TP_STATS) { st_a = (long long)__builtin_amdgcn_s_memtime(); ++st_rounds; }
				replay16_block<MODE, G, K, TS, SMALL, BITS, CK>(a, mem, gs, refoff, qA, qB, l1A, l1B, blk_bl[0], blk_c[0], blk_bl[1], blk_c[1]);
				asm volatile("s_waitcnt vmcnt(0)" ::: "memory");
				if (AT_TP_STATS) st_rep += (long long)__builtin_amdgcn_s_memtime() - st_a;
				__builtin_amdgcn_fence(__ATOMIC_ACQUIRE, "agent");
				if (AT_TP_STATS) st_a = (long long)__builtin_amdgcn_s_memtime();
				{
					constexpr int KQ = (K + 3) / 4, GQ = (KG2 + 3) / 4, S4N = CK / 4;
					constexpr int WSCR = ck_walk_words<MODE, K, CK>();
					constexpr int NBLK = ck_walk_blocks<G>();
					constexpr int NCHP = S4N * KQ, NCH = NCHP + (HASJ ? S4N * GQ : 0);
					constexpr int LPW = 64 / (2 * NG), CPL = (NBLK * NCH + LPW - 1) / LPW;
					const int sl0 = g2 * G;
					const int scr0 = a.off_bound + lane * (NBLK * WSCR);
					bool wgo = go;
					(void)GQ;
					for (;;) {
						int need[NBLK], tbl[NBLK], tc[NBLK];
#pragma unroll
						for (int k = 0; k < NBLK; ++k) { need[k] = -1; tbl[k] = -1; tc[k] = -1; }
						if (wgo) {
							if (ci <= 0 || (!ISFIT && cj <= 0) || (MODE == K_LOCAL && st == 0)) wgo = false;
							else if (cj <= 0 || cnt >= own_len || (st == 0 && !HASJ)) { ok = false; wgo = false; }
							else {
								const int bl = (ci - 1) / K, rr = (ci - 1) - bl * K;
								const int c = ((cj - 1) + bl) >> LCB;
								const int q = pat.slot(bl, c);
								if (q < 0) wgo = false;
								else {
									need[0] = sl0 + q; tbl[0] = bl; tc[0] = c;
									if constexpr (NBLK == 4) {
										const int c2 = ((cj - 1) - (rr + 1) + (bl - 1)) >> LCB;
										const int q1 = pat.slot(bl, c - 1), q2 = bl > 0 ? pat.slot(bl - 1, c2) : -1, q3 = bl > 0 ? pat.slot(bl - 1, c2 - 1) : -1;
										if (q1 >= 0) { need[1] = sl0 + q1; tbl[1] = bl; tc[1] = c - 1; }
										if (q2 >= 0) { need[2] = sl0 + q2; tbl[2] = bl - 1; tc[2] = c2; }
										if (q3 >= 0) { need[3] = sl0 + q3; tbl[3] = bl - 1; tc[3] = c2 - 1; }
									}
								}
							}
						}
						if (!__any(need[0] >= 0)) break;
						long long st_f0 = 0;
						if (AT_TP_STATS) st_f0 = (long long)__builtin_amdgcn_s_memtime();
						{
							const int w = lane / LPW, part = lane % LPW;
							const int dst = a.off_bound + w * (NBLK * WSCR);
							int src[NBLK];
#pragma unroll
							for (int k = 0; k < NBLK; ++k) src[k] = __shfl(need[k], w);
							uint4 tw[CPL];
#pragma unroll
							for (int x = 0; x < CPL; ++x) {
								const int id = part + x * LPW, k = id / NCH, ch = id - k * NCH;
								const int sl = imax(NBLK == 1 ? src[0] : pick<NBLK>(src, imin(k, NBLK - 1)), 0);
								const uint32_t *from = gs + (ch < NCHP ? a.off_rptr + (ch * 64 + sl) * 4 : a.off_rjpl + ((ch - NCHP) * 64 + sl) * 4);
								asm volatile("global_load_dwordx4 %0, %1, off" : "=&v"(tw[x]) : "v"(from) : "memory");
							}
							asm volatile("s_waitcnt vmcnt(0)" ::: "memory");
#pragma unroll
							for (int x = 0; x < CPL; ++x) {
								const int id = part + x * LPW, k = id / NCH, ch = id - k * NCH;
								const int sl = NBLK == 1 ? src[0] : pick<NBLK>(src, imin(k, NBLK - 1));
								if (sl >= 0 && k < NBLK) *(uint4 *)(&at_lds[dst + k * WSCR + 4 * ch]) = tw[x];
							}
							__builtin_amdgcn_fence(__ATOMIC_ACQ_REL, "wavefront");
						}
						if (AT_TP_STATS) st_fetch += (int)((long long)__builtin_amdgcn_s_memtime() - st_f0);
						if (need[0] >= 0) {
							int kb = 0;
							for (;;) {
								const int bl = NBLK == 1 ? tbl[0] : pick<NBLK>(tbl, kb), c = NBLK == 1 ? tc[0] : pick<NBLK>(tc, kb);
								const int scr = scr0 + kb * WSCR, scj = scr + KQ * CK;
								(void)scj;
								const int i_lo = bl * K, t_lo = imax(c << LCB, bl) - bl;
								for (;;) {
									const int rr = ci - 1 - i_lo, ss = cj - 1 - t_lo;
									if ((rr | ss) < 0 || cnt >= own_len || (st == 0 && !HASJ)) break;
									if constexpr (HASJ) {
										if (st == 0) {
											constexpr unsigned long long ORD = 0xfbea7362d9c85140ull;
											const int s4 = ss >> 2, tk = ss & 3;
											uint32_t cols = 0;
#pragma unroll
											for (int x = 0; x < 4; ++x) {
												const uint32_t w = at_lds[scj + imax(s4 - x, 0) * (GQ * 4) + (rr >> 2)];
												const uint32_t nib = (w >> (16 * h + cell_shift<4>(rr & 3))) & 15u;
												cols = (cols << 4) | ((uint32_t)(ORD >> (4 * nib)) & 15u);
											}
											cols = (cols << (3 - tk)) & 0xffffu;
											const int avail = 4 * imin(4, s4 + 1) - (3 - tk);
											const int lim = imin(imin(avail, cj), own_len - cnt);
											const int n = __clz((int)((cols << 16) | 0x8000u));
											const int steps = n < lim ? n + 1 : lim;
											if (n < lim) st = 2;
											for (int x = 0; x < steps; ++x) ops[cnt + x] = 3;
											cnt += steps; cj -= steps;
											continue;
										}
									}
									if (AT_TP_STATS) ++st_iters;
									const uint32_t ust = (uint32_t)st;
									const uint32_t inL = ust & (ust >> 1), inM = (ust >> 1) & ~ust & 1u;
									const int di = (int)(ust >> 1), dj = (int)(inL ^ 1u);
									const uint32_t mL = 0u - inL, mM = 0u - inM, mU = ~(mL | mM);
									uint32_t nbv[4], nst[4];
									int shv[4];
#pragma unroll
									for (int x = 0; x < 4; ++x) {
										const int rx = imax(rr - x * di, 0), sx = imax(ss - x * dj, 0);
										nbv[x] = at_lds[scr + (sx >> 2) * (KQ * 4) + rx];
										shv[x] = 16 * h + ((sx & 1) << 3) + ((sx & 2) << 1);
									}
#pragma unroll
									for (int x = 0; x < 4; ++x) {
										const uint32_t nb = nbv[x] >> shv[x];
										const uint32_t lres = 2u + ((nb >> 2) & 1u), mres = nb & 3u, ures = TS == 4 ? 1u + ((nb >> 3) & 1u) : 2u - ((nb >> 3) & 1u);
										nst[x] = (lres & mL) | (mres & mM) | (ures & mU);
									}
									const uint32_t e0 = ((nst[0] ^ ust) - 1u) >> 31, e1 = e0 & (((nst[1] ^ ust) - 1u) >> 31), e2 = e1 & (((nst[2] ^ ust) - 1u) >> 31);
									const int mdi = -di, mdj = -dj;
									const int lim = imin(imin((rr & mdi) | (3 & ~mdi), (ss & mdj) | (3 & ~mdj)), own_len - cnt - 1);
									const int n = imin(1 + (int)(e0 + e1 + e2), lim + 1);
									const uint32_t op4 = (inL | (2u & mU)) * 0x01010101u;
									if (__builtin_expect(cnt + 4 <= own_len, 1)) __builtin_memcpy(ops + cnt, &op4, 4);
									else {
#pragma nounroll
										for (int x = 0; x < n; ++x) ops[cnt + x] = (uint8_t)op4;
									}
									st = (int)(((nst[0] | (nst[1] << 4) | (nst[2] << 8) | (nst[3] << 12)) >> (4 * (n - 1))) & 15u);
									ci -= n * di; cj -= n * dj; cnt += n;
								}
								if constexpr (NBLK == 1) break;
								else {
									if (ci <= 0 || cj <= 0 || cnt >= own_len || st == 0) break;
									const int nbl = (ci - 1) / K, nc = ((cj - 1) + nbl) >> LCB;
									int kn = -1;
#pragma unroll
									for (int k = 0; k < NBLK; ++k) kn = (tbl[k] == nbl && tc[k] == nc) ? k : kn;
									if (kn < 0 || kn == kb) break;
									kb = kn;
								}
							}
						}
					}
				}
				if (AT_TP_STATS) st_walk += (long long)__builtin_amdgcn_s_memtime() - st_a;
			}
			if (AT_WALK_PRIO) __builtin_amdgcn_s_setprio(0);
			if (AT_TP_STATS) {
				const long long now = (long long)__builtin_amdgcn_s_memtime();
				int mxf = st_fetch, mxi = st_iters;
				for (int d = 1; d < 64; d <<= 1) mxi = imax(mxi, __shfl_xor(mxi, d));
				if (lane == 0) {
					atomicAdd(a.queue + 1, 1ull); atomicAdd(a.queue + 2, (unsigned long long)st_rounds);
					atomicAdd(a.queue + 3, (unsigned long long)st_walk); atomicAdd(a.queue + 4, (unsigned long long)mxf);
// ... 19 lines not shown
		} else
		{
			const int g = lane >> 1, h = lane & 1;
			const long long pin = (wk * NG + g) * 2 + h;
			const bool mine = lane < 2 * NG && pin < a.npairs && !filler;
			const long long p = RAG ? pout : pin;
			if (mine) {
				int ci = my_ci, cj = my_cj, st = my_st, cnt = 0;
				bool ok = my_ok;
				if constexpr (TB) {
					uint8_t *ops = a.ops + a.ops_off[p];
					const int glane = g * G;
					int guard = own_len + 2;
					if (AT_WALK_PRIO) __builtin_amdgcn_s_setprio(AT_WALK_PRIO);
					if (AT_DIAG_NO_WALK) {
					} else if (ok && OVL) {
						while (cj > 0 && --guard >= 0) {
							if (ci <= 0) { ok = false; break; }
							const int ss = G == 64 ? (ci - 1) / RS : 0, li = G == 64 ? (ci - 1) % RS : ci - 1;
							const int ln = li / K, r = li % K;
							const int t = (cj - 1) + ln;
							const uint32_t w = pm.ld(a.off_ptr + (G == 64 ? __mul24(ss, wps * NL) : 0) + pidx<PTRLDS, K>(t / SPW, r, glane + ln, NL));
							const uint32_t nb = (w >> (16 * h + cell_shift<PB>(t % SPW))) & 3u;
							if (nb == 0) { ok = false; break; }
							ops[cnt++] = (uint8_t)(nb == 3 ? 2 : nb == 2 ? 0 : 1);
							ci -= nb != 3; cj -= nb != 1;
						}
						if (guard < 0) ok = false;
					} else if (ok && (ISFIT || (AT_GLOBAL_WALK_AHEAD && MODE == K_GLOBAL && G < 64) || (AT_LOCAL_WALK_AHEAD && MODE == K_LOCAL && G < 64))) {
						constexpr int AHEAD = AT_WALK_AHEAD;
						while (ci > 0 && (ISFIT || cj > 0)) {
							if (MODE == K_LOCAL && st == 0) break;
							if (cj <= 0 || cnt >= own_len) { ok = false; break; }
							const bool inJ = JPL && st == 0;
							const int di = st >= 2 ? 1 : 0, dj = st == 3 ? 0 : 1;
							const int ss0 = G == 64 ? (ci - 1) / RS : 0, li0 = G == 64 ? (ci - 1) % RS : ci - 1;
							const int ln0 = li0 / K, r0 = li0 % K;
							uint32_t w[AHEAD];
							int sh[AHEAD];
#pragma unroll
							for (int q = 0; q < AHEAD; ++q) {
								int ss = ss0, ln = ln0, r = r0;
								if (q * di > 0 && q * di < ci) {
									if constexpr (K >= AHEAD) {
										r = r0 - q * di;
										if (r < 0) { r += K; --ln; }
										if (G == 64 && ln < 0) { ln += 64; --ss; }
									} else {
										const int qi = ci - q * di;
										ss = G == 64 ? (qi - 1) / RS : 0;
										const int li = G == 64 ? (qi - 1) % RS : qi - 1;
										ln = li / K; r = li % K;
									}
								}
								const int t = (imax(cj - q * dj, 1) - 1) + ln;
								int idx = a.off_ptr + (G == 64 ? __mul24(ss, wps * NL) : 0) + pidx<PTRLDS, K>(t / SPW, r, glane + ln, NL);
								sh[q] = 16 * h + cell_shift<PB>(t % SPW);
								if constexpr (JPL) {
									const int jidx = jpl_base0 + (G == 64 ? __mul24(ss0, wpj * NL) : 0) +
									                 pidx<PTRLDS, KG>(imax((((cj - 1) + ln0) >> 2) - q, 0), r0 >> 2, glane + ln0, NL);
									idx = inJ ? jidx : idx;
									sh[q] = inJ ? 16 * h + cell_shift<4>(r0 & 3) : sh[q];
								}
								w[q] = pm.ld(idx);
							}
							if constexpr (JPL) {
								if (inJ) {
									constexpr unsigned long long ORD = 0xfbea7362d9c85140ull;
									uint32_t cols = 0;
#pragma unroll
									for (int q = 0; q < AHEAD; ++q) cols = (cols << 4) | ((uint32_t)(ORD >> (4 * ((w[q] >> sh[q]) & 15u))) & 15u);
									const int tk = ((cj - 1) + ln0) & 3;
									cols = (cols << (16 - 4 * AHEAD + 3 - tk)) & 0xffffu;
									const int avail = 4 * AHEAD - (3 - tk);
									const int lim = imin(imin(avail, cj), own_len - cnt);
									const int n = __clz((int)((cols << 16) | 0x8000u));
									const int steps = n < lim ? n + 1 : lim;
									if (n < lim) st = 2;
									for (int x = 0; x < steps; ++x) ops[cnt + x] = 3;
									cnt += steps; cj -= steps;
									continue;
								}
							}
							bool go = true;
#pragma unroll
							for (int q = 0; q < AHEAD; ++q) {
								if (go) {
									const uint32_t nb = (w[q] >> sh[q]) & ((1u << PB) - 1u);
									const int was = st;
									int op = 0;
									if (st == 3) { st = X3 ? (int)((XT3 >> (2 * nb)) & 3u) : (nb & 4u) ? 3 : 2; op = 1; --ci; }
									else if (st == 2) { st = X3 ? (int)((XT2 >> (2 * nb)) & 3u) : (int)(nb & 3u); op = 0; --ci; --cj; }
									else if (st == 1) { st = X3 ? (int)((XT1 >> (2 * nb)) & 3u) : (TS == 4 ? (nb & 8u) != 0 : (nb & 8u) == 0) ? 2 : 1; op = 2; --cj; }
									else if (HASJ && !JPL) { st = (nb & 16u) ? 2 : 0; op = 3; --cj; }
									else { ok = false; go = false; }
									if (ok) {
										ops[cnt++] = (uint8_t)op;
										go = st == was && ci > 0 && cj > 0 && cnt < own_len;
									}
								}
							}
							if (!ok) break;
						}
						if constexpr (MODE == K_GLOBAL) {
							if (ok) {
								while (cj > 0) { ops[cnt++] = 2; --cj; }
								while (ci > 0) { ops[cnt++] = 1; --ci; }
							}
						}
					} else if (ok) {
						const int wpsNL = wps * NL;
						while (ci > 0 && cj > 0 && --guard >= 0) {
							if (MODE == K_LOCAL && st == 0) break;
							const int ss = G == 64 ? (ci - 1) / RS : 0, li = G == 64 ? (ci - 1) % RS : ci - 1;
							const int ln = li / K, r = li % K;
							const int t = (cj - 1) + ln;
							const uint32_t w = pm.ld(a.off_ptr + (G == 64 ? __mul24(ss, wpsNL) : 0) + pidx<PTRLDS, K>(t / SPW, r, glane + ln, NL));
							const uint32_t nb = (w >> (16 * h + cell_shift<PB>(t % SPW))) & ((1u << PB) - 1u);
							if (st == 0) { ok = false; break; }
							const bool u_open = TS == 4 ? (nb & 8u) != 0 : (nb & 8u) == 0;
							const int inL = st == 3, inM = st == 2;
							const int op = inL ? 1 : inM ? 0 : 2;
							if constexpr (X3) st = (int)(((inL ? XT3 : inM ? XT2 : XT1) >> (2 * nb)) & 3u);
							else st = inL ? ((nb & 4u) ? 3 : 2) : inM ? (int)(nb & 3u) : (u_open ? 2 : 1);
							ci -= inL | inM; cj -= inL ^ 1;
							ops[cnt++] = (uint8_t)op;
						}
						if constexpr (MODE == K_GLOBAL) {
							while (cj > 0) { ops[cnt++] = 2; --cj; }
							while (ci > 0) { ops[cnt++] = 1; --ci; }
						}
						if (guard < 0) ok = false;
					}
				}
				a.score[p] = ok ? (my_sc >> TS) : INT32_MIN;
				if (a.end_i) a.end_i[p] = my_ci;
				if (a.end_j) a.end_j[p] = my_cj;
				if (a.state) a.state[p] = my_st == 3 ? 1 : my_st == 2 ? 2 : 3;
				if (a.nops) a.nops[p] = ok ? cnt : -1;
			}
			if (TB && AT_WALK_PRIO) __builtin_amdgcn_s_setprio(0);
		}
		mem.sync();
	}
	return wnext;
}

constexpr int AT_TAIL_G = 32;
constexpr int at_tail_k(int g, int k)
{
	return (g * k + AT_TAIL_G - 1) / AT_TAIL_G < 2 ? 2 : (g * k + AT_TAIL_G - 1) / AT_TAIL_G;
}

template <int MODE, int G, int K, int TS, bool SMALL, bool PTRLDS, bool TB, bool RAG = false, int BITS = 2, int CK = 0, int SPLIT = 0>
__global__ __launch_bounds__(64, (CK > 0 && G == 64 ? AT_TP_WAVES64 : AT_WAVES16(G, K))) void at_sweep16(const Sweep16Args a, const Sweep16Args t)
{
	if (a.only_if && __builtin_amdgcn_readfirstlane(*a.only_if) != a.only_val) return;
	long long w = sweep16_items<MODE, G, K, TS, SMALL, PTRLDS, TB, RAG, BITS, CK, SPLIT>(a, (long long)blockIdx.x, 0);
	if constexpr (G <= 16 && !RAG && MODE != K_OVERLAP) {
		if (t.npairs > 0) {
			constexpr int NGm = 64 / G;
			const long long nmain = (a.npairs + 2 * NGm - 1) / (2 * NGm);
			sweep16_items<MODE, AT_TAIL_G, at_tail_k(G, K), TS, SMALL, PTRLDS, TB, false, BITS, CK, SPLIT>(t, w, nmain);
		}
	}
}

}
```

Before: 3336 GCUPS.

## Add profile-lookup scoring variant for local 2-bit int16 sweep kernels

Adds a PROF template variant of the packed int16 sweep and replay kernels for local mode with 2-bit codes and x16 scores. Instead of a byte-permute lookup followed by an add and a clamp at zero, it precomputes per-word profile values from the reference word and the match/mismatch difference, and computes the M cell with a fused prof_m_v helper. Reference bytes are stored in a profile-friendly encoding (s2_bytes<PROF>), and dispatch routes through an AT_KMODE_PROF flag when the scoring parameters allow it. This is meant to shorten the per-cell critical path, but it doubles kernel instantiations and adds per-word setup work.

Measured after the change: 3437 GCUPS, median of 6. 3.0% higher.

```diff
diff --git a/aligntools/c_amd/csrc/at_hip.hip b/aligntools/c_amd/csrc/at_hip.hip
--- a/aligntools/c_amd/csrc/at_hip.hip
+++ b/aligntools/c_amd/csrc/at_hip.hip
@@ -1097,9 +1097,10 @@
 		snprintf(tag16, sizeof tag16, "packed16 x%d bits=%d %dx%d-lane groups (%d pairs/wave)%s", 1 << ts, bits, 64 / P.g, P.g, per_wave,
 		         rag ? " ragged frames" : "");
 		if (two_pass) snprintf(tag16 + strlen(tag16), sizeof tag16 - strlen(tag16), " two-pass%s ck=%d", tp_split ? " (walk kernel)" : "", at::ck_steps(P.g));
+		const bool prof = kmode == at::K_LOCAL && bits == 2 && ts == 4 && at::profile_lookup_ok(h->m, h->u);
 		auto pick = [&](int st) {
-			if (two_pass) return st == 1 ? at_pick16_tp(kmode, P.g, P.k, ts, bits, tp_split) : (at_sweep16_fn) nullptr;
-			return rag ? at_pick16_rag(kmode, P.g, P.k, st, tb, bits) : at_pick16(kmode, P.g, P.k, ts, st, tb, bits);
+			if (two_pass) return st == 1 ? at_pick16_tp(kmode, P.g, P.k, ts, bits, tp_split, prof) : (at_sweep16_fn) nullptr;
+			return rag ? at_pick16_rag(kmode, P.g, P.k, st, tb, bits, prof) : at_pick16(kmode, P.g, P.k, ts, st, tb, bits, prof);
 		};
 		const long long nwork = (np + per_wave - 1) / per_wave;
 		int rc = plan_launch(h, tag16, P.k, nwork, std::max(P.off_ptr, PT.off_ptr),
diff --git a/aligntools/c_amd/csrc/at_k16.hip b/aligntools/c_amd/csrc/at_k16.hip
--- a/aligntools/c_amd/csrc/at_k16.hip
+++ b/aligntools/c_amd/csrc/at_k16.hip
@@ -6,7 +6,7 @@
 	at_sweep16_fn at_pick16_g32_b##b(int kmode, int k, int store, bool tb);        \
 	at_sweep16_fn at_pick16_g8_b##b(int kmode, int k, int store, bool tb);         \
 	at_sweep16_fn at_pick16_g4_b##b(int kmode, int k, int store, bool tb);         \
-	at_sweep16_fn at_pick16_rag_impl_b##b(int k, int store, bool tb);                \
+	at_sweep16_fn at_pick16_rag_impl_b##b(int kmode, int k, int store, bool tb);     \
 	at_sweep16_fn at_pick16_rag8a_b##b(int kmode, int k, int store, bool tb);      \
 	at_sweep16_fn at_pick16_rag8b_b##b(int kmode, int k, int store, bool tb);      \
 	at_sweep16_fn at_pick16_rag8c_b##b(int kmode, int k, int store, bool tb);      \
@@ -22,8 +22,13 @@
 AT_DECL(2)
 AT_DECL(8)
 #undef AT_DECL
-at_sweep16_fn at_pick16(int kmode, int g, int k, int ts, int store, bool tb, int bits)
+static int unit_kmode(int kmode, int ts, int bits, bool prof)
 {
+	return prof && kmode == at::K_LOCAL && ts == 4 && bits == 2 ? kmode | AT_KMODE_PROF : kmode;
+}
+at_sweep16_fn at_pick16(int kmode, int g, int k, int ts, int store, bool tb, int bits, bool prof)
+{
+	kmode = unit_kmode(kmode, ts, bits, prof);
 	if (g == 8) return ts != 4 ? nullptr : bits == 8 ? at_pick16_g8_b8(kmode, k, store, tb) : at_pick16_g8_b2(kmode, k, store, tb);
 	if (g == 4) return ts != 4 ? nullptr : bits == 8 ? at_pick16_g4_b8(kmode, k, store, tb) : at_pick16_g4_b2(kmode, k, store, tb);
 	if (g == 32) return ts != 4 ? nullptr : bits == 8 ? at_pick16_g32_b8(kmode, k, store, tb) : at_pick16_g32_b2(kmode, k, store, tb);
@@ -34,8 +39,10 @@
 	if (g == 16) return ts == 4 ? at_pick16_g16_b2(kmode, k, store, tb) : nullptr;
 	return ts == 4 ? at_pick16_g64_ts4_b2(kmode, k, store, tb) : at_pick16_g64_ts2_b2(kmode, k, store, tb);
 }
-at_sweep16_fn at_pick16_rag(int kmode, int g, int k, int store, bool tb, int bits)
+at_sweep16_fn at_pick16_rag(int kmode, int g, int k, int store, bool tb, int bits, bool prof)
 {
+	const bool local = kmode == at::K_LOCAL;
+	if (g != 8) kmode = unit_kmode(kmode, 4, bits, prof);
 	if (g == 8) {
 		if (k == 6 || k == 8) return bits == 8 ? at_pick16_rag8d_b8(kmode, k, store, tb) : at_pick16_rag8d_b2(kmode, k, store, tb);
 		if (bits == 8) return k >= 19 ? at_pick16_rag8c_b8(kmode, k, store, tb) : k >= 13 ? at_pick16_rag8b_b8(kmode, k, store, tb) : at_pick16_rag8a_b8(kmode, k, store, tb);
@@ -45,11 +52,12 @@
 	if (g == 32) return bits == 8 ? at_pick16_rag32_b8(kmode, k, store, tb) : at_pick16_rag32_b2(kmode, k, store, tb);
 	if (g != 16) return nullptr;
 	if (k >= 16) return bits == 8 ? at_pick16_rag16b_b8(kmode, k, store, tb) : at_pick16_rag16b_b2(kmode, k, store, tb);
-	if (kmode == at::K_LOCAL) return bits == 8 ? at_pick16_rag_impl_b8(k, store, tb) : at_pick16_rag_impl_b2(k, store, tb);
+	if (local) return bits == 8 ? at_pick16_rag_impl_b8(kmode, k, store, tb) : at_pick16_rag_impl_b2(kmode, k, store, tb);
 	return bits == 8 ? at_pick16_rag16_b8(kmode, k, store, tb) : at_pick16_rag16_b2(kmode, k, store, tb);
 }
-at_sweep16_fn at_pick16_tp(int kmode, int g, int k, int ts, int bits, int split)
+at_sweep16_fn at_pick16_tp(int kmode, int g, int k, int ts, int bits, int split, bool prof)
 {
+	kmode = unit_kmode(kmode, ts, bits, prof);
 	if (g == 8) return ts != 4 ? nullptr : bits == 8 ? at_pick16_tp8_b8(kmode, k, split) : at_pick16_tp8_b2(kmode, k, split);
 	if (g == 64) return bits == 8 ? at_pick16_tp64_b8(kmode, k, ts, split) : at_pick16_tp64_b2(kmode, k, ts, split);
 	return nullptr;
diff --git a/aligntools/c_amd/csrc/at_k16_g16a.hip b/aligntools/c_amd/csrc/at_k16_g16a.hip
--- a/aligntools/c_amd/csrc/at_k16_g16a.hip
+++ b/aligntools/c_amd/csrc/at_k16_g16a.hip
@@ -1,19 +1,19 @@
 #include "at_launch.h"
-template <int MODE, int K>
+template <int MODE, int K, bool PROF = false>
 static at_sweep16_fn q3(int store, bool tb)
 {
-	if (!tb) return at::at_sweep16<MODE, 16, K, 4, true, true, false, false, AT_BITS16>;
-	if (store == 0) return at::at_sweep16<MODE, 16, K, 4, true, true, true, false, AT_BITS16>;
-	return at::at_sweep16<MODE, 16, K, 4, true, false, true, false, AT_BITS16>;
+	if (!tb) return at::at_sweep16<MODE, 16, K, 4, true, true, false, false, AT_BITS16, 0, 0, PROF>;
+	if (store == 0) return at::at_sweep16<MODE, 16, K, 4, true, true, true, false, AT_BITS16, 0, 0, PROF>;
+	return at::at_sweep16<MODE, 16, K, 4, true, false, true, false, AT_BITS16, 0, 0, PROF>;
 }
-template <int MODE>
+template <int MODE, bool PROF = false>
 static at_sweep16_fn q2(int k, int store, bool tb)
 {
 	switch (k) {
-	case 4: return q3<MODE, 4>(store, tb);
-	case 5: return q3<MODE, 5>(store, tb);
-	case 6: return q3<MODE, 6>(store, tb);
-	case 7: return q3<MODE, 7>(store, tb);
+	case 4: return q3<MODE, 4, PROF>(store, tb);
+	case 5: return q3<MODE, 5, PROF>(store, tb);
+	case 6: return q3<MODE, 6, PROF>(store, tb);
+	case 7: return q3<MODE, 7, PROF>(store, tb);
 	default: return nullptr;
 	}
 }
@@ -22,6 +22,7 @@
 	switch (kmode) {
 	case at::K_GLOBAL: return q2<at::K_GLOBAL>(k, store, tb);
 	case at::K_LOCAL: return q2<at::K_LOCAL>(k, store, tb);
+	AT_CASE_LOCAL_PROF(q2<at::K_LOCAL, true>(k, store, tb))
 	case at::K_FITJ: return q2<at::K_FITJ>(k, store, tb);
 	default: return q2<at::K_FIT>(k, store, tb);
 	}
diff --git a/aligntools/c_amd/csrc/at_k16_g16b.hip b/aligntools/c_amd/csrc/at_k16_g16b.hip
--- a/aligntools/c_amd/csrc/at_k16_g16b.hip
+++ b/aligntools/c_amd/csrc/at_k16_g16b.hip
@@ -1,17 +1,17 @@
 #include "at_launch.h"
-template <int MODE, int K>
+template <int MODE, int K, bool PROF = false>
 static at_sweep16_fn q3(int store, bool tb)
 {
-	if (!tb) return at::at_sweep16<MODE, 16, K, 4, true, true, false, false, AT_BITS16>;
-	if (store == 0) return at::at_sweep16<MODE, 16, K, 4, true, true, true, false, AT_BITS16>;
-	return at::at_sweep16<MODE, 16, K, 4, true, false, true, false, AT_BITS16>;
+	if (!tb) return at::at_sweep16<MODE, 16, K, 4, true, true, false, false, AT_BITS16, 0, 0, PROF>;
+	if (store == 0) return at::at_sweep16<MODE, 16, K, 4, true, true, true, false, AT_BITS16, 0, 0, PROF>;
+	return at::at_sweep16<MODE, 16, K, 4, true, false, true, false, AT_BITS16, 0, 0, PROF>;
 }
-template <int MODE>
+template <int MODE, bool PROF = false>
 static at_sweep16_fn q2(int k, int store, bool tb)
 {
 	switch (k) {
-	case 10: return q3<MODE, 10>(store, tb);
-	case 13: return q3<MODE, 13>(store, tb);
+	case 10: return q3<MODE, 10, PROF>(store, tb);
+	case 13: return q3<MODE, 13, PROF>(store, tb);
 	default: return nullptr;
 	}
 }
@@ -20,6 +20,7 @@
 	switch (kmode) {
 	case at::K_GLOBAL: return q2<at::K_GLOBAL>(k, store, tb);
 	case at::K_LOCAL: return q2<at::K_LOCAL>(k, store, tb);
+	AT_CASE_LOCAL_PROF(q2<at::K_LOCAL, true>(k, store, tb))
 	case at::K_FITJ: return q2<at::K_FITJ>(k, store, tb);
 	default: return q2<at::K_FIT>(k, store, tb);
 	}
diff --git a/aligntools/c_amd/csrc/at_k16_g16c.hip b/aligntools/c_amd/csrc/at_k16_g16c.hip
--- a/aligntools/c_amd/csrc/at_k16_g16c.hip
+++ b/aligntools/c_amd/csrc/at_k16_g16c.hip
@@ -1,16 +1,16 @@
 #include "at_launch.h"
-template <int MODE, int K>
+template <int MODE, int K, bool PROF = false>
 static at_sweep16_fn r3(bool tb)
 {
-	if (!tb) return at::at_sweep16<MODE, 16, K, 4, true, true, false, false, AT_BITS16>;
-	return at::at_sweep16<MODE, 16, K, 4, true, false, true, false, AT_BITS16>;
+	if (!tb) return at::at_sweep16<MODE, 16, K, 4, true, true, false, false, AT_BITS16, 0, 0, PROF>;
+	return at::at_sweep16<MODE, 16, K, 4, true, false, true, false, AT_BITS16, 0, 0, PROF>;
 }
-template <int MODE>
+template <int MODE, bool PROF = false>
 static at_sweep16_fn r2(int k, bool tb)
 {
 	switch (k) {
-	case 16: return r3<MODE, 16>(tb);
-	case 19: return r3<MODE, 19>(tb);
+	case 16: return r3<MODE, 16, PROF>(tb);
+	case 19: return r3<MODE, 19, PROF>(tb);
 	default: return nullptr;
 	}
 }
@@ -20,6 +20,7 @@
 	switch (kmode) {
 	case at::K_GLOBAL: return r2<at::K_GLOBAL>(k, tb);
 	case at::K_LOCAL: return r2<at::K_LOCAL>(k, tb);
+	AT_CASE_LOCAL_PROF(r2<at::K_LOCAL, true>(k, tb))
 	case at::K_FITJ: return r2<at::K_FITJ>(k, tb);
 	default: return r2<at::K_FIT>(k, tb);
 	}
diff --git a/aligntools/c_amd/csrc/at_k16_g32.hip b/aligntools/c_amd/csrc/at_k16_g32.hip
--- a/aligntools/c_amd/csrc/at_k16_g32.hip
+++ b/aligntools/c_amd/csrc/at_k16_g32.hip
@@ -1,19 +1,19 @@
 #include "at_launch.h"
-template <int MODE, int K>
+template <int MODE, int K, bool PROF = false>
 static at_sweep16_fn g3(int store, bool tb)
 {
-	if (!tb) return at::at_sweep16<MODE, 32, K, 4, true, true, false, false, AT_BITS16>;
-	if (store == 0) return at::at_sweep16<MODE, 32, K, 4, true, true, true, false, AT_BITS16>;
-	return at::at_sweep16<MODE, 32, K, 4, true, false, true, false, AT_BITS16>;
+	if (!tb) return at::at_sweep16<MODE, 32, K, 4, true, true, false, false, AT_BITS16, 0, 0, PROF>;
+	if (store == 0) return at::at_sweep16<MODE, 32, K, 4, true, true, true, false, AT_BITS16, 0, 0, PROF>;
+	return at::at_sweep16<MODE, 32, K, 4, true, false, true, false, AT_BITS16, 0, 0, PROF>;
 }
-template <int MODE>
+template <int MODE, bool PROF = false>
 static at_sweep16_fn g2(int k, int store, bool tb)
 {
 	switch (k) {
-	case 7: return g3<MODE, 7>(store, tb);
-	case 8: return g3<MODE, 8>(store, tb);
-	case 10: return g3<MODE, 10>(store, tb);
-	case 13: return g3<MODE, 13>(store, tb);
+	case 7: return g3<MODE, 7, PROF>(store, tb);
+	case 8: return g3<MODE, 8, PROF>(store, tb);
+	case 10: return g3<MODE, 10, PROF>(store, tb);
+	case 13: return g3<MODE, 13, PROF>(store, tb);
 	default: return nullptr;
 	}
 }
@@ -24,6 +24,7 @@
 	switch (kmode) {
 	case at::K_GLOBAL: return g2<at::K_GLOBAL>(k, store, tb);
 	case at::K_LOCAL: return g2<at::K_LOCAL>(k, store, tb);
+	AT_CASE_LOCAL_PROF(g2<at::K_LOCAL, true>(k, store, tb))
 	case at::K_FITJ: return g2<at::K_FITJ>(k, store, tb);
 	default: return g2<at::K_FIT>(k, store, tb);
 	}
diff --git a/aligntools/c_amd/csrc/at_k16_g32b.hip b/aligntools/c_amd/csrc/at_k16_g32b.hip
--- a/aligntools/c_amd/csrc/at_k16_g32b.hip
+++ b/aligntools/c_amd/csrc/at_k16_g32b.hip
@@ -1,17 +1,17 @@
 #include "at_launch.h"
-template <int MODE, int K>
+template <int MODE, int K, bool PROF = false>
 static at_sweep16_fn s3(bool tb)
 {
-	if (!tb) return at::at_sweep16<MODE, 32, K, 4, true, true, false, false, AT_BITS16>;
-	return at::at_sweep16<MODE, 32, K, 4, true, false, true, false, AT_BITS16>;
+	if (!tb) return at::at_sweep16<MODE, 32, K, 4, true, true, false, false, AT_BITS16, 0, 0, PROF>;
+	return at::at_sweep16<MODE, 32, K, 4, true, false, true, false, AT_BITS16, 0, 0, PROF>;
 }
-template <int MODE>
+template <int MODE, bool PROF = false>
 static at_sweep16_fn s2(int k, bool tb)
 {
 	switch (k) {
-	case 12: return s3<MODE, 12>(tb);
-	case 16: return s3<MODE, 16>(tb);
-	case 19: return s3<MODE, 19>(tb);
+	case 12: return s3<MODE, 12, PROF>(tb);
+	case 16: return s3<MODE, 16, PROF>(tb);
+	case 19: return s3<MODE, 19, PROF>(tb);
 	default: return nullptr;
 	}
 }
@@ -21,6 +21,7 @@
 	switch (kmode) {
 	case at::K_GLOBAL: return s2<at::K_GLOBAL>(k, tb);
 	case at::K_LOCAL: return s2<at::K_LOCAL>(k, tb);
+	AT_CASE_LOCAL_PROF(s2<at::K_LOCAL, true>(k, tb))
 	case at::K_FITJ: return s2<at::K_FITJ>(k, tb);
 	default: return s2<at::K_FIT>(k, tb);
 	}
diff --git a/aligntools/c_amd/csrc/at_k16_g4.hip b/aligntools/c_amd/csrc/at_k16_g4.hip
--- a/aligntools/c_amd/csrc/at_k16_g4.hip
+++ b/aligntools/c_amd/csrc/at_k16_g4.hip
@@ -1,17 +1,17 @@
 #include "at_launch.h"
-template <int MODE, int K>
+template <int MODE, int K, bool PROF = false>
 static at_sweep16_fn f3(bool tb)
 {
-	if (!tb) return at::at_sweep16<MODE, 4, K, 4, true, true, false, false, AT_BITS16>;
-	return at::at_sweep16<MODE, 4, K, 4, true, false, true, false, AT_BITS16>;
+	if (!tb) return at::at_sweep16<MODE, 4, K, 4, true, true, false, false, AT_BITS16, 0, 0, PROF>;
+	return at::at_sweep16<MODE, 4, K, 4, true, false, true, false, AT_BITS16, 0, 0, PROF>;
 }
-template <int MODE>
+template <int MODE, bool PROF = false>
 static at_sweep16_fn f2(int k, bool tb)
 {
 	switch (k) {
-	case 9: return f3<MODE, 9>(tb);
-	case 10: return f3<MODE, 10>(tb);
-	case 13: return f3<MODE, 13>(tb);
+	case 9: return f3<MODE, 9, PROF>(tb);
+	case 10: return f3<MODE, 10, PROF>(tb);
+	case 13: return f3<MODE, 13, PROF>(tb);
 	default: return nullptr;
 	}
 }
@@ -23,6 +23,7 @@
 	switch (kmode) {
 	case at::K_GLOBAL: return f2<at::K_GLOBAL>(k, tb);
 	case at::K_LOCAL: return f2<at::K_LOCAL>(k, tb);
+	AT_CASE_LOCAL_PROF(f2<at::K_LOCAL, true>(k, tb))
 	case at::K_FITJ: return f2<at::K_FITJ>(k, tb);
 	default: return f2<at::K_FIT>(k, tb);
 	}
diff --git a/aligntools/c_amd/csrc/at_k16_g4b.hip b/aligntools/c_amd/csrc/at_k16_g4b.hip
--- a/aligntools/c_amd/csrc/at_k16_g4b.hip
+++ b/aligntools/c_amd/csrc/at_k16_g4b.hip
@@ -1,16 +1,16 @@
 #include "at_launch.h"
-template <int MODE, int K>
+template <int MODE, int K, bool PROF = false>
 static at_sweep16_fn f3(bool tb)
 {
-	if (!tb) return at::at_sweep16<MODE, 4, K, 4, true, true, false, false, AT_BITS16>;
-	return at::at_sweep16<MODE, 4, K, 4, true, false, true, false, AT_BITS16>;
+	if (!tb) return at::at_sweep16<MODE, 4, K, 4, true, true, false, false, AT_BITS16, 0, 0, PROF>;
+	return at::at_sweep16<MODE, 4, K, 4, true, false, true, false, AT_BITS16, 0, 0, PROF>;
 }
-template <int MODE>
+template <int MODE, bool PROF = false>
 static at_sweep16_fn f2(int k, bool tb)
 {
 	switch (k) {
-	case 16: return f3<MODE, 16>(tb);
-	case 19: return f3<MODE, 19>(tb);
+	case 16: return f3<MODE, 16, PROF>(tb);
+	case 19: return f3<MODE, 19, PROF>(tb);
 	default: return nullptr;
 	}
 }
@@ -20,6 +20,7 @@
 	switch (kmode) {
 	case at::K_GLOBAL: return f2<at::K_GLOBAL>(k, tb);
 	case at::K_LOCAL: return f2<at::K_LOCAL>(k, tb);
+	AT_CASE_LOCAL_PROF(f2<at::K_LOCAL, true>(k, tb))
 	case at::K_FITJ: return f2<at::K_FITJ>(k, tb);
 	default: return f2<at::K_FIT>(k, tb);
 	}
diff --git a/aligntools/c_amd/csrc/at_k16_g64.hip b/aligntools/c_amd/csrc/at_k16_g64.hip
--- a/aligntools/c_amd/csrc/at_k16_g64.hip
+++ b/aligntools/c_amd/csrc/at_k16_g64.hip
@@ -1,20 +1,20 @@
 #include "at_launch.h"
-template <int MODE, int K>
+template <int MODE, int K, bool PROF = false>
 static at_sweep16_fn p3(int store, bool tb)
 {
-	if (!tb) return store < 2 ? at::at_sweep16<MODE, 64, K, 4, true, true, false, false, AT_BITS16> : at::at_sweep16<MODE, 64, K, 4, false, false, false, false, AT_BITS16>;
-	if (store == 0) return at::at_sweep16<MODE, 64, K, 4, true, true, true, false, AT_BITS16>;
-	if (store == 1) return at::at_sweep16<MODE, 64, K, 4, true, false, true, false, AT_BITS16>;
-	return at::at_sweep16<MODE, 64, K, 4, false, false, true, false, AT_BITS16>;
+	if (!tb) return store < 2 ? at::at_sweep16<MODE, 64, K, 4, true, true, false, false, AT_BITS16, 0, 0, PROF> : at::at_sweep16<MODE, 64, K, 4, false, false, false, false, AT_BITS16, 0, 0, PROF>;
+	if (store == 0) return at::at_sweep16<MODE, 64, K, 4, true, true, true, false, AT_BITS16, 0, 0, PROF>;
+	if (store == 1) return at::at_sweep16<MODE, 64, K, 4, true, false, true, false, AT_BITS16, 0, 0, PROF>;
+	return at::at_sweep16<MODE, 64, K, 4, false, false, true, false, AT_BITS16, 0, 0, PROF>;
 }
-template <int MODE>
+template <int MODE, bool PROF = false>
 static at_sweep16_fn p2(int k, int store, bool tb)
 {
 	switch (k) {
-	case 1: return p3<MODE, 1>(store, tb);
-	case 2: return p3<MODE, 2>(store, tb);
-	case 3: return p3<MODE, 3>(store, tb);
-	default: return p3<MODE, 4>(store, tb);
+	case 1: return p3<MODE, 1, PROF>(store, tb);
+	case 2: return p3<MODE, 2, PROF>(store, tb);
+	case 3: return p3<MODE, 3, PROF>(store, tb);
+	default: return p3<MODE, 4, PROF>(store, tb);
 	}
 }
 at_sweep16_fn AT_NAME(at_pick16_g64_ts4)(int kmode, int k, int store, bool tb)
@@ -22,6 +22,7 @@
 	switch (kmode) {
 	case at::K_GLOBAL: return p2<at::K_GLOBAL>(k, store, tb);
 	case at::K_LOCAL: return p2<at::K_LOCAL>(k, store, tb);
+	AT_CASE_LOCAL_PROF(p2<at::K_LOCAL, true>(k, store, tb))
 	case at::K_FITJ: return p2<at::K_FITJ>(k, store, tb);
 	default: return p2<at::K_FIT>(k, store, tb);
 	}
diff --git a/aligntools/c_amd/csrc/at_k16_g8a.hip b/aligntools/c_amd/csrc/at_k16_g8a.hip
--- a/aligntools/c_amd/csrc/at_k16_g8a.hip
+++ b/aligntools/c_amd/csrc/at_k16_g8a.hip
@@ -1,17 +1,17 @@
 #include "at_launch.h"
-template <int MODE, int K>
+template <int MODE, int K, bool PROF = false>
 static at_sweep16_fn h3(bool tb)
 {
-	if (!tb) return at::at_sweep16<MODE, 8, K, 4, true, true, false, false, AT_BITS16>;
-	return at::at_sweep16<MODE, 8, K, 4, true, false, true, false, AT_BITS16>;
+	if (!tb) return at::at_sweep16<MODE, 8, K, 4, true, true, false, false, AT_BITS16, 0, 0, PROF>;
+	return at::at_sweep16<MODE, 8, K, 4, true, false, true, false, AT_BITS16, 0, 0, PROF>;
 }
-template <int MODE>
+template <int MODE, bool PROF = false>
 static at_sweep16_fn h2(int k, bool tb)
 {
 	switch (k) {
-	case 5: return h3<MODE, 5>(tb);
-	case 7: return h3<MODE, 7>(tb);
-	case 10: return h3<MODE, 10>(tb);
+	case 5: return h3<MODE, 5, PROF>(tb);
+	case 7: return h3<MODE, 7, PROF>(tb);
+	case 10: return h3<MODE, 10, PROF>(tb);
 	default: return nullptr;
 	}
 }
@@ -21,6 +21,7 @@
 	switch (kmode) {
 	case at::K_GLOBAL: return h2<at::K_GLOBAL>(k, tb);
 	case at::K_LOCAL: return h2<at::K_LOCAL>(k, tb);
+	AT_CASE_LOCAL_PROF(h2<at::K_LOCAL, true>(k, tb))
 	case at::K_FITJ: return h2<at::K_FITJ>(k, tb);
 	default: return h2<at::K_FIT>(k, tb);
 	}
diff --git a/aligntools/c_amd/csrc/at_k16_g8b.hip b/aligntools/c_amd/csrc/at_k16_g8b.hip
--- a/aligntools/c_amd/csrc/at_k16_g8b.hip
+++ b/aligntools/c_amd/csrc/at_k16_g8b.hip
@@ -1,16 +1,16 @@
 #include "at_launch.h"
-template <int MODE, int K>
+template <int MODE, int K, bool PROF = false>
 static at_sweep16_fn h3(bool tb)
 {
-	if (!tb) return at::at_sweep16<MODE, 8, K, 4, true, true, false, false, AT_BITS16>;
-	return at::at_sweep16<MODE, 8, K, 4, true, false, true, false, AT_BITS16>;
+	if (!tb) return at::at_sweep16<MODE, 8, K, 4, true, true, false, false, AT_BITS16, 0, 0, PROF>;
+	return at::at_sweep16<MODE, 8, K, 4, true, false, true, false, AT_BITS16, 0, 0, PROF>;
 }
-template <int MODE>
+template <int MODE, bool PROF = false>
 static at_sweep16_fn h2(int k, bool tb)
 {
 	switch (k) {
-	case 13: return h3<MODE, 13>(tb);
-	case 16: return h3<MODE, 16>(tb);
+	case 13: return h3<MODE, 13, PROF>(tb);
+	case 16: return h3<MODE, 16, PROF>(tb);
 	default: return nullptr;
 	}
 }
@@ -20,6 +20,7 @@
 	switch (kmode) {
 	case at::K_GLOBAL: return h2<at::K_GLOBAL>(k, tb);
 	case at::K_LOCAL: return h2<at::K_LOCAL>(k, tb);
+	AT_CASE_LOCAL_PROF(h2<at::K_LOCAL, true>(k, tb))
 	case at::K_FITJ: return h2<at::K_FITJ>(k, tb);
 	default: return h2<at::K_FIT>(k, tb);
 	}
diff --git a/aligntools/c_amd/csrc/at_k16_g8c.hip b/aligntools/c_amd/csrc/at_k16_g8c.hip
--- a/aligntools/c_amd/csrc/at_k16_g8c.hip
+++ b/aligntools/c_amd/csrc/at_k16_g8c.hip
@@ -1,15 +1,15 @@
 #include "at_launch.h"
-template <int MODE, int K>
+template <int MODE, int K, bool PROF = false>
 static at_sweep16_fn h3(bool tb)
 {
-	if (!tb) return at::at_sweep16<MODE, 8, K, 4, true, true, false, false, AT_BITS16>;
-	return at::at_sweep16<MODE, 8, K, 4, true, false, true, false, AT_BITS16>;
+	if (!tb) return at::at_sweep16<MODE, 8, K, 4, true, true, false, false, AT_BITS16, 0, 0, PROF>;
+	return at::at_sweep16<MODE, 8, K, 4, true, false, true, false, AT_BITS16, 0, 0, PROF>;
 }
-template <int MODE>
+template <int MODE, bool PROF = false>
 static at_sweep16_fn h2(int k, bool tb)
 {
 	switch (k) {
-	case 19: return h3<MODE, 19>(tb);
+	case 19: return h3<MODE, 19, PROF>(tb);
 	default: return nullptr;
 	}
 }
@@ -19,6 +19,7 @@
 	switch (kmode) {
 	case at::K_GLOBAL: return h2<at::K_GLOBAL>(k, tb);
 	case at::K_LOCAL: return h2<at::K_LOCAL>(k, tb);
+	AT_CASE_LOCAL_PROF(h2<at::K_LOCAL, true>(k, tb))
 	case at::K_FITJ: return h2<at::K_FITJ>(k, tb);
 	default: return h2<at::K_FIT>(k, tb);
 	}
diff --git a/aligntools/c_amd/csrc/at_k16_g8d.hip b/aligntools/c_amd/csrc/at_k16_g8d.hip
--- a/aligntools/c_amd/csrc/at_k16_g8d.hip
+++ b/aligntools/c_amd/csrc/at_k16_g8d.hip
@@ -1,16 +1,16 @@
 #include "at_launch.h"
-template <int MODE, int K>
+template <int MODE, int K, bool PROF = false>
 static at_sweep16_fn h3(bool tb)
 {
-	if (!tb) return at::at_sweep16<MODE, 8, K, 4, true, true, false, false, AT_BITS16>;
-	return at::at_sweep16<MODE, 8, K, 4, true, false, true, false, AT_BITS16>;
+	if (!tb) return at::at_sweep16<MODE, 8, K, 4, true, true, false, false, AT_BITS16, 0, 0, PROF>;
+	return at::at_sweep16<MODE, 8, K, 4, true, false, true, false, AT_BITS16, 0, 0, PROF>;
 }
-template <int MODE>
+template <int MODE, bool PROF = false>
 static at_sweep16_fn h2(int k, bool tb)
 {
 	switch (k) {
-	case 6: return h3<MODE, 6>(tb);
-	case 8: return h3<MODE, 8>(tb);
+	case 6: return h3<MODE, 6, PROF>(tb);
+	case 8: return h3<MODE, 8, PROF>(tb);
 	default: return nullptr;
 	}
 }
@@ -20,6 +20,7 @@
 	switch (kmode) {
 	case at::K_GLOBAL: return h2<at::K_GLOBAL>(k, tb);
 	case at::K_LOCAL: return h2<at::K_LOCAL>(k, tb);
+	AT_CASE_LOCAL_PROF(h2<at::K_LOCAL, true>(k, tb))
 	case at::K_FITJ: return h2<at::K_FITJ>(k, tb);
 	default: return h2<at::K_FIT>(k, tb);
 	}
diff --git a/aligntools/c_amd/csrc/at_k16_rag.hip b/aligntools/c_amd/csrc/at_k16_rag.hip
--- a/aligntools/c_amd/csrc/at_k16_rag.hip
+++ b/aligntools/c_amd/csrc/at_k16_rag.hip
@@ -1,20 +1,29 @@
 #include "at_launch.h"
-template <int K>
+template <int K, bool PROF>
 static at_sweep16_fn r3(int store, bool tb)
 {
-	if (!tb) return at::at_sweep16<at::K_LOCAL, 16, K, 4, true, true, false, true, AT_BITS16>;
-	if (store == 0) return at::at_sweep16<at::K_LOCAL, 16, K, 4, true, true, true, true, AT_BITS16>;
-	return at::at_sweep16<at::K_LOCAL, 16, K, 4, true, false, true, true, AT_BITS16>;
+	if (!tb) return at::at_sweep16<at::K_LOCAL, 16, K, 4, true, true, false, true, AT_BITS16, 0, 0, PROF>;
+	if (store == 0) return at::at_sweep16<at::K_LOCAL, 16, K, 4, true, true, true, true, AT_BITS16, 0, 0, PROF>;
+	return at::at_sweep16<at::K_LOCAL, 16, K, 4, true, false, true, true, AT_BITS16, 0, 0, PROF>;
 }
-at_sweep16_fn AT_NAME(at_pick16_rag_impl)(int k, int store, bool tb)
+template <bool PROF>
+static at_sweep16_fn r2(int k, int store, bool tb)
 {
 	switch (k) {
-	case 4: return r3<4>(store, tb);
-	case 5: return r3<5>(store, tb);
-	case 6: return r3<6>(store, tb);
-	case 7: return r3<7>(store, tb);
-	case 10: return r3<10>(store, tb);
-	case 13: return r3<13>(store, tb);
+	case 4: return r3<4, PROF>(store, tb);
+	case 5: return r3<5, PROF>(store, tb);
+	case 6: return r3<6, PROF>(store, tb);
+	case 7: return r3<7, PROF>(store, tb);
+	case 10: return r3<10, PROF>(store, tb);
+	case 13: return r3<13, PROF>(store, tb);
 	default: return nullptr;
 	}
 }
+at_sweep16_fn AT_NAME(at_pick16_rag_impl)(int kmode, int k, int store, bool tb)
+{
+	switch (kmode) {
+	case at::K_LOCAL: return r2<false>(k, store, tb);
+	AT_CASE_LOCAL_PROF(r2<true>(k, store, tb))
+	default: return nullptr;
+	}
+}
diff --git a/aligntools/c_amd/csrc/at_k16_rag16b.hip b/aligntools/c_amd/csrc/at_k16_rag16b.hip
--- a/aligntools/c_amd/csrc/at_k16_rag16b.hip
+++ b/aligntools/c_amd/csrc/at_k16_rag16b.hip
@@ -1,16 +1,16 @@
 #include "at_launch.h"
-template <int MODE, int K>
+template <int MODE, int K, bool PROF = false>
 static at_sweep16_fn x3(bool tb)
 {
-	if (!tb) return at::at_sweep16<MODE, 16, K, 4, true, true, false, true, AT_BITS16>;
-	return at::at_sweep16<MODE, 16, K, 4, true, false, true, true, AT_BITS16>;
+	if (!tb) return at::at_sweep16<MODE, 16, K, 4, true, true, false, true, AT_BITS16, 0, 0, PROF>;
+	return at::at_sweep16<MODE, 16, K, 4, true, false, true, true, AT_BITS16, 0, 0, PROF>;
 }
-template <int MODE>
+template <int MODE, bool PROF = false>
 static at_sweep16_fn x2(int k, bool tb)
 {
 	switch (k) {
-	case 16: return x3<MODE, 16>(tb);
-	case 19: return x3<MODE, 19>(tb);
+	case 16: return x3<MODE, 16, PROF>(tb);
+	case 19: return x3<MODE, 19, PROF>(tb);
 	default: return nullptr;
 	}
 }
@@ -20,6 +20,7 @@
 	switch (kmode) {
 	case at::K_GLOBAL: return x2<at::K_GLOBAL>(k, tb);
 	case at::K_LOCAL: return x2<at::K_LOCAL>(k, tb);
+	AT_CASE_LOCAL_PROF(x2<at::K_LOCAL, true>(k, tb))
 	case at::K_FITJ: return x2<at::K_FITJ>(k, tb);
 	default: return x2<at::K_FIT>(k, tb);
 	}
diff --git a/aligntools/c_amd/csrc/at_k16_rag32.hip b/aligntools/c_amd/csrc/at_k16_rag32.hip
--- a/aligntools/c_amd/csrc/at_k16_rag32.hip
+++ b/aligntools/c_amd/csrc/at_k16_rag32.hip
@@ -1,19 +1,19 @@
 #include "at_launch.h"
-template <int MODE, int K>
+template <int MODE, int K, bool PROF = false>
 static at_sweep16_fn y3(bool tb)
 {
-	if (!tb) return at::at_sweep16<MODE, 32, K, 4, true, true, false, true, AT_BITS16>;
-	return at::at_sweep16<MODE, 32, K, 4, true, false, true, true, AT_BITS16>;
+	if (!tb) return at::at_sweep16<MODE, 32, K, 4, true, true, false, true, AT_BITS16, 0, 0, PROF>;
+	return at::at_sweep16<MODE, 32, K, 4, true, false, true, true, AT_BITS16, 0, 0, PROF>;
 }
-template <int MODE>
+template <int MODE, bool PROF = false>
 static at_sweep16_fn y2(int k, bool tb)
 {
 	switch (k) {
-	case 10: return y3<MODE, 10>(tb);
-	case 12: return y3<MODE, 12>(tb);
-	case 13: return y3<MODE, 13>(tb);
-	case 16: if constexpr (MODE == at::K_LOCAL || MODE == at::K_GLOBAL) return y3<MODE, 16>(tb); else return nullptr;
-	case 19: if constexpr (MODE == at::K_LOCAL) return y3<MODE, 19>(tb); else return nullptr;
+	case 10: return y3<MODE, 10, PROF>(tb);
+	case 12: return y3<MODE, 12, PROF>(tb);
+	case 13: return y3<MODE, 13, PROF>(tb);
+	case 16: if constexpr (MODE == at::K_LOCAL || MODE == at::K_GLOBAL) return y3<MODE, 16, PROF>(tb); else return nullptr;
+	case 19: if constexpr (MODE == at::K_LOCAL) return y3<MODE, 19, PROF>(tb); else return nullptr;
 	default: return nullptr;
 	}
 }
@@ -23,6 +23,7 @@
 	switch (kmode) {
 	case at::K_GLOBAL: return y2<at::K_GLOBAL>(k, tb);
 	case at::K_LOCAL: return y2<at::K_LOCAL>(k, tb);
+	AT_CASE_LOCAL_PROF(y2<at::K_LOCAL, true>(k, tb))
 	case at::K_FITJ: return y2<at::K_FITJ>(k, tb);
 	default: return y2<at::K_FIT>(k, tb);
 	}
diff --git a/aligntools/c_amd/csrc/at_k16_tp.hip b/aligntools/c_amd/csrc/at_k16_tp.hip
--- a/aligntools/c_amd/csrc/at_k16_tp.hip
+++ b/aligntools/c_amd/csrc/at_k16_tp.hip
@@ -1,16 +1,17 @@
 #include "at_launch.h"
-template <int MODE>
+template <int MODE, bool PROF = false>
 static at_sweep16_fn tp8(int k, int split)
 {
 	if (k != 19) return nullptr;
-	return split ? at::at_sweep16<MODE, 8, 19, 4, true, false, false, false, AT_BITS16, at::ck_steps(8), 1>
-	             : at::at_sweep16<MODE, 8, 19, 4, true, false, false, false, AT_BITS16, at::ck_steps(8)>;
+	return split ? at::at_sweep16<MODE, 8, 19, 4, true, false, false, false, AT_BITS16, at::ck_steps(8), 1, PROF>
+	             : at::at_sweep16<MODE, 8, 19, 4, true, false, false, false, AT_BITS16, at::ck_steps(8), 0, PROF>;
 }
 at_sweep16_fn AT_NAME(at_pick16_tp8)(int kmode, int k, int split)
 {
 	switch (kmode) {
 	case at::K_GLOBAL: return tp8<at::K_GLOBAL>(k, split);
 	case at::K_LOCAL: return tp8<at::K_LOCAL>(k, split);
+	AT_CASE_LOCAL_PROF(tp8<at::K_LOCAL, true>(k, split))
 	case at::K_FITJ: return tp8<at::K_FITJ>(k, split);
 	default: return tp8<at::K_FIT>(k, split);
 	}
diff --git a/aligntools/c_amd/csrc/at_k16_tp64.hip b/aligntools/c_amd/csrc/at_k16_tp64.hip
--- a/aligntools/c_amd/csrc/at_k16_tp64.hip
+++ b/aligntools/c_amd/csrc/at_k16_tp64.hip
@@ -1,10 +1,10 @@
 #include "at_launch.h"
-template <int MODE, int TS>
+template <int MODE, int TS, bool PROF = false>
 static at_sweep16_fn tp64(int k, int split)
 {
 	switch (k) {
-	case 16: return split ? at::at_sweep16<MODE, 64, 16, TS, true, false, false, false, AT_BITS16, at::ck_steps(64), 1>
-	                      : at::at_sweep16<MODE, 64, 16, TS, true, false, false, false, AT_BITS16, at::ck_steps(64)>;
+	case 16: return split ? at::at_sweep16<MODE, 64, 16, TS, true, false, false, false, AT_BITS16, at::ck_steps(64), 1, PROF>
+	                      : at::at_sweep16<MODE, 64, 16, TS, true, false, false, false, AT_BITS16, at::ck_steps(64), 0, PROF>;
 	default: return nullptr;
 	}
 }
@@ -21,6 +21,7 @@
 	switch (kmode) {
 	case at::K_GLOBAL: return tp64<at::K_GLOBAL, 4>(k, split);
 	case at::K_LOCAL: return tp64<at::K_LOCAL, 4>(k, split);
+	AT_CASE_LOCAL_PROF(tp64<at::K_LOCAL, 4, true>(k, split))
 	case at::K_FITJ: return tp64<at::K_FITJ, 4>(k, split);
 	default: return tp64<at::K_FIT, 4>(k, split);
 	}
diff --git a/aligntools/c_amd/csrc/at_launch.h b/aligntools/c_amd/csrc/at_launch.h
--- a/aligntools/c_amd/csrc/at_launch.h
+++ b/aligntools/c_amd/csrc/at_launch.h
@@ -10,9 +10,9 @@
 
 at_sweep_fn at_pick32_b2(int kmode, int k, int store, bool tb);
 at_sweep_fn at_pick32_b8(int kmode, int k, int store, bool tb);
-at_sweep16_fn at_pick16_rag(int kmode, int g, int k, int store, bool tb, int bits);
-at_sweep16_fn at_pick16(int kmode, int g, int k, int ts, int store, bool tb, int bits);
-at_sweep16_fn at_pick16_tp(int kmode, int g, int k, int ts, int bits, int split = 0);
+at_sweep16_fn at_pick16_rag(int kmode, int g, int k, int store, bool tb, int bits, bool prof = false);
+at_sweep16_fn at_pick16(int kmode, int g, int k, int ts, int store, bool tb, int bits, bool prof = false);
+at_sweep16_fn at_pick16_tp(int kmode, int g, int k, int ts, int bits, int split = 0, bool prof = false);
 typedef void (*at_walk16_fn)(const at::Sweep16Args, const at::Sweep16Args);
 at_walk16_fn at_pick_walk16(int kmode, int g, int k, int ts, int bits, int teams = 0);
 int at_walk16_team_lanes(int g);
@@ -21,6 +21,12 @@
 #endif
 #define AT_CAT_(a, b) a##b
 #define AT_CAT(a, b) AT_CAT_(a, b)
+constexpr int AT_KMODE_PROF = 0x100;
+#if AT_BITS16 == 2
+#define AT_CASE_LOCAL_PROF(...) case at::K_LOCAL | AT_KMODE_PROF: return __VA_ARGS__;
+#else
+#define AT_CASE_LOCAL_PROF(...)
+#endif
 #define AT_NAME(f) AT_CAT(f, AT_CAT(_b, AT_BITS16))
 
 template <int MODE, int BITS, int K>
diff --git a/aligntools/c_amd/csrc/at_sweep16.hip.h b/aligntools/c_amd/csrc/at_sweep16.hip.h
--- a/aligntools/c_amd/csrc/at_sweep16.hip.h
+++ b/aligntools/c_amd/csrc/at_sweep16.hip.h
@@ -207,6 +207,64 @@
 static_assert(xor3_proof(), "XOR3 cells: the decode returns m's state, `L extended` and `U extended` for all 16 inputs");
 static_assert(PtrTags<K_GLOBAL, 4, 0>::L == 15 && PtrTags<K_LOCAL, 4, 16>::M == 10 && PtrTags<K_LOCAL, 2, 0>::L == 3 && PtrTags<K_FIT, 4, 0>::U == 1, "every other family keeps its tags");
 
+__host__ __device__ constexpr bool profile_lookup_ok(int m, int u) { return m >= 0 && u <= 0 && (m - u) * 16 <= 255; }
+__host__ __device__ constexpr uint32_t prof_word(uint32_t d, uint32_t code8) { return d << (code8 & 31u); }
+__host__ __device__ constexpr uint32_t prof_sel(uint32_t qa, uint32_t qb) { return qa | (qb << 16) | 0x0c040c00u; }
+constexpr uint32_t prof_perm_half(uint32_t word, uint32_t q) { return (word >> (8 * q)) & 0xffu; }
+constexpr uint32_t prof_m_half(uint32_t diag, uint32_t sp, uint32_t nu)
+{
+	const uint32_t t = (diag + sp) & 0xffffu;
+	return t > nu ? t - nu : 0u;
+}
+constexpr uint32_t old_m_half(uint32_t diag, int s)
+{
+	int v = (int)(short)diag + s;
+	v = v > 32767 ? 32767 : v < -32768 ? -32768 : v;
+	return (uint32_t)(v > 0 ? v : 0);
+}
+constexpr bool prof_proof(int m, int u, uint32_t lo, uint32_t hi)
+{
+	if (!profile_lookup_ok(m, u)) return false;
+	const int m16 = m * 16, u16 = u * 16;
+	const uint32_t d = (uint32_t)(m16 - u16), nu = (uint32_t)(-u16);
+	for (uint32_t a = 0; a < 4; ++a)
+		for (uint32_t q = 0; q < 4; ++q)
+			if (prof_perm_half(prof_word(d, 8 * a), q) != (a == q ? d : 0u)) return false;
+	for (uint32_t diag = lo; diag < hi && (int)diag + m16 <= 32767; ++diag)
+		if (prof_m_half(diag, d, nu) != old_m_half(diag, m16) || prof_m_half(diag, 0u, nu) != old_m_half(diag, u16)) return false;
+	return true;
+}
+#define AT_PROF_PROOF_(m, u, q) static_assert(prof_proof(m, u, (q) * 0x1000u, ((q) + 1) * 0x1000u), "profile lookup: add, subtract-and-clamp equals pmax(padd(diag, S), 0) bit for bit");
+#define AT_PROF_PROOF(m, u) AT_PROF_PROOF_(m, u, 0) AT_PROF_PROOF_(m, u, 1) AT_PROF_PROOF_(m, u, 2) AT_PROF_PROOF_(m, u, 3) AT_PROF_PROOF_(m, u, 4) AT_PROF_PROOF_(m, u, 5) AT_PROF_PROOF_(m, u, 6) AT_PROF_PROOF_(m, u, 7)
+AT_PROF_PROOF(0, 0) AT_PROF_PROOF(15, 0) AT_PROF_PROOF(0, -15) AT_PROF_PROOF(8, -7) AT_PROF_PROOF(1, -14) AT_PROF_PROOF(2, -2)
+#undef AT_PROF_PROOF
+#undef AT_PROF_PROOF_
+static_assert(prof_sel(3, 2) == 0x0c060c03u && !profile_lookup_ok(8, -8) && !profile_lookup_ok(-1, -2) && !profile_lookup_ok(1, 1), "the selector's bytes; the scorings that keep the LUT");
+template <int KK>
+AT_DEV uint32_t prof_word_v(uint32_t win, uint32_t d)
+{
+	uint32_t r;
+	if constexpr (KK == 0) asm("v_lshlrev_b32_sdwa %0, %1, %2 dst_sel:DWORD dst_unused:UNUSED_PAD src0_sel:BYTE_0 src1_sel:DWORD" : "=v"(r) : "v"(win), "v"(d));
+	else if constexpr (KK == 1) asm("v_lshlrev_b32_sdwa %0, %1, %2 dst_sel:DWORD dst_unused:UNUSED_PAD src0_sel:BYTE_1 src1_sel:DWORD" : "=v"(r) : "v"(win), "v"(d));
+	else if constexpr (KK == 2) asm("v_lshlrev_b32_sdwa %0, %1, %2 dst_sel:DWORD dst_unused:UNUSED_PAD src0_sel:BYTE_2 src1_sel:DWORD" : "=v"(r) : "v"(win), "v"(d));
+	else asm("v_lshlrev_b32_sdwa %0, %1, %2 dst_sel:DWORD dst_unused:UNUSED_PAD src0_sel:BYTE_3 src1_sel:DWORD" : "=v"(r) : "v"(win), "v"(d));
+	return r;
+}
+AT_DEV uint32_t prof_m_v(uint32_t diag, uint32_t pb, uint32_t pa, uint32_t psel, uint32_t nu2)
+{
+	uint32_t t, m;
+	const uint32_t sp = __builtin_amdgcn_perm(pb, pa, psel);
+	asm("v_pk_add_u16 %0, %1, %2" : "=v"(t) : "v"(diag), "v"(sp));
+	asm("v_pk_sub_u16 %0, %1, %2 clamp" : "=v"(m) : "v"(t), "s"(nu2));
+	return m;
+}
+template <bool PROF>
+AT_DEV uint32_t s2_bytes(uint32_t b)
+{
+	if constexpr (PROF) return ((b & 3u) << 3) | ((b & 0xcu) << 9) | ((b & 0x30u) << 15) | ((b & 0xc0u) << 21);
+	else return (b & 3u) | ((b & 0xcu) << 6) | ((b & 0x30u) << 12) | ((b & 0xc0u) << 18);
+}
+
 template <bool LDS, int K>
 AT_DEV int pidx(int wr, int r, int lane, int NL)
 {
@@ -354,7 +412,7 @@
 #else
 #define AT_REPLAY_FN __device__ __noinline__
 #endif
-template <int MODE, int G, int K, int TS, bool SMALL, int BITS, int CB>
+template <int MODE, int G, int K, int TS, bool SMALL, int BITS, int CB, bool PROF = false>
 AT_REPLAY_FN void replay16_block(const Sweep16Args &a, const Slot<SMALL> &mem, uint32_t *gs, const int refoff,
                            const uint32_t *qA, const uint32_t *qB, const int l1A, const int l1B,
                            const int blA, const int cA, const int blB, const int cB)
@@ -379,6 +437,10 @@
 	uint32_t gmo2 = pk2(a.g16 - a.o16), neg2 = 0x80008000u;
 	uint32_t c1 = 0x00010001u, umm2 = pk2(a.u16 - a.m16), m2 = pk2(a.m16);
 	asm volatile("" : "+v"(c8888), "+v"(gmo2), "+v"(neg2), "+v"(c1), "+v"(umm2), "+v"(m2));
+	if constexpr (PROF) lut_lo = (uint32_t)(a.m16 - a.u16);
+	const uint32_t &profD = lut_lo;
+	const uint32_t nu2 = pk2(-a.u16);
+	(void)profD; (void)nu2;
 	asm volatile("" : "+v"(o2), "+v"(e2), "+v"(lut_lo), "+v"(lut_hi));
 	asm volatile("" : "+v"(cClean), "+v"(cTagM), "+v"(cTagL), "+v"(cTagU), "+v"(cM3), "+v"(cM7), "+v"(cF0), "+v"(cF000));
 
@@ -457,7 +519,7 @@
 			uint32_t ca, cb;
 			if constexpr (BITS == 2) { ca = (wa >> ((qi & 15) * 2)) & 3u; cb = (wb >> ((qj & 15) * 2)) & 3u; }
 			else { ca = (wa >> ((qi & 3) * 8)) & 0xffu; cb = (wb >> ((qj & 3) * 8)) & 0xffu; }
-			qsel[r] = (ca * 0x00000101u + cb * 0x01010000u) | (BITS == 2 ? 0x04000400u : 0u);
+			qsel[r] = PROF ? prof_sel(ca, cb) : (ca * 0x00000101u + cb * 0x01010000u) | (BITS == 2 ? 0x04000400u : 0u);
 			acc[r] = 0;
 		}
 	}
@@ -488,16 +550,22 @@
 			const uint32_t Aup = eup.x, Bup = eup.y;
 			uint32_t gopen = neg2;
 			if constexpr (HASJ) gopen = lohi(((smA >> k) & 1u) ? gmo2 : neg2, ((smB >> k) & 1u) ? gmo2 : neg2);
-			const uint32_t selw = __builtin_amdgcn_perm(wB, wA, SELK);
+			uint32_t selw = 0, profA = 0, profB = 0;
+			(void)selw; (void)profA; (void)profB;
+			if constexpr (PROF) { profA = prof_word_v<k>(wA, profD); profB = prof_word_v<k>(wB, profD); }
+			else selw = __builtin_amdgcn_perm(wB, wA, SELK);
 			uint32_t diag = Ad, lraw = Bup, jn = 0;
 			(void)jn;
 #pragma unroll
 			for (int r = 0; r < K; ++r) {
-				uint32_t S;
+				uint32_t S = 0, Mraw;
+				if constexpr (PROF) Mraw = prof_m_v(diag, profB, profA, qsel[r], nu2);
+				else {
 				if constexpr (BITS == 2) S = __builtin_amdgcn_perm(lut_hi, lut_lo, selw ^ qsel[r]);
 				else S = pmad(pminu(selw ^ qsel[r], c1), umm2, m2);
-				uint32_t Mraw = padd(diag, S);
+				Mraw = padd(diag, S);
 				if constexpr (MODE == K_LOCAL) Mraw = pmax(Mraw, 0u);
+				}
 				const uint32_t Mc = vandor(Mraw, cClean, cTagM);
 				const uint32_t Lc = lraw | cTagL;
 				const uint32_t Uraw = pmax(Mo_l[r], padd(U_l[r], e2));
@@ -560,9 +628,10 @@
 	}
 }
 
-template <int MODE, int G, int K, int TS, bool SMALL, bool PTRLDS, bool TB, bool RAG = false, int BITS = 2, int CK = 0, int SPLIT = 0>
+template <int MODE, int G, int K, int TS, bool SMALL, bool PTRLDS, bool TB, bool RAG = false, int BITS = 2, int CK = 0, int SPLIT = 0, bool PROF = false>
 AT_DEV long long sweep16_items(const Sweep16Args &a, long long wnext, const long long wbase)
 {
+	static_assert(!PROF || (MODE == K_LOCAL && BITS == 2 && TS == 4), "profile lookup: local, 2-bit codes, scores x16");
 	static_assert(!SPLIT || CK > 0, "a walk kernel follows a sweep that leaves checkpoints");
 	constexpr bool TP = CK > 0;
 	static_assert(!TP || (!TB && !RAG && MODE != K_OVERLAP && !PTRLDS), "two-pass tracebacks: uniform batches of the affine modes, checkpoints in the global slot");
@@ -619,6 +688,10 @@
 	asm volatile("" : "+v"(gmo2), "+v"(neg2));
 	uint32_t c1 = 0x00010001u, umm2 = pk2(a.u16 - a.m16), m2 = pk2(mS);
 	asm volatile("" : "+v"(c1), "+v"(umm2), "+v"(m2));
+	if constexpr (PROF) lut_lo = (uint32_t)(a.m16 - a.u16);
+	const uint32_t &profD = lut_lo;
+	const uint32_t nu2 = pk2(-a.u16);
+	(void)profD; (void)nu2;
 	asm volatile("" : "+v"(o2), "+v"(e2), "+v"(lut_lo), "+v"(lut_hi));
 	if constexpr (X3) asm volatile("" : "+v"(cClean), "+v"(cTagM), "+v"(cTagL), "+v"(cTagU), "+v"(cNib), "+v"(cF0), "+v"(cF000));
 	else asm volatile("" : "+v"(cClean), "+v"(cTagM), "+v"(cTagL), "+v"(cTagU), "+v"(cM3), "+v"(cM7), "+v"(cNib), "+v"(cF0), "+v"(cF000));
@@ -712,8 +785,8 @@
 #pragma unroll
 					for (int q = 0; q < 4; ++q) {
 						const uint32_t ba = (va >> (8 * q)) & 0xffu, bb = (vb >> (8 * q)) & 0xffu;
-						mem.st(refoff + PADW + 4 * w + q, (ba & 3u) | ((ba & 0xcu) << 6) | ((ba & 0x30u) << 12) | ((ba & 0xc0u) << 18));
-						mem.st(refoff + a.off_refb + PADW + 4 * w + q, (bb & 3u) | ((bb & 0xcu) << 6) | ((bb & 0x30u) << 12) | ((bb & 0xc0u) << 18));
+						mem.st(refoff + PADW + 4 * w + q, s2_bytes<PROF>(ba));
+						mem.st(refoff + a.off_refb + PADW + 4 * w + q, s2_bytes<PROF>(bb));
 					}
 				}
 			}
@@ -758,7 +831,7 @@
 				uint32_t ca, cb;
 				if constexpr (BITS == 2) { ca = (qA[qi >> 4] >> ((qi & 15) * 2)) & 3u; cb = (qB[qj >> 4] >> ((qj & 15) * 2)) & 3u; }
 				else { ca = (qA[qi >> 2] >> ((qi & 3) * 8)) & 0xffu; cb = (qB[qj >> 2] >> ((qj & 3) * 8)) & 0xffu; }
-				qsel[r] = (ca * 0x00000101u + cb * 0x01010000u) | (BITS == 2 ? 0x04000400u : 0u);
+				qsel[r] = PROF ? prof_sel(ca, cb) : (ca * 0x00000101u + cb * 0x01010000u) | (BITS == 2 ? 0x04000400u : 0u);
 				acc[r] = 0;
 				keymask[r] = (i0 + r < l1A ? (uint32_t)(0xffff & ~TMASK) : 0u) | (i0 + r < l1B ? (uint32_t)(0xffff & ~TMASK) << 16 : 0u);
 				int L, M, U;
@@ -878,7 +951,10 @@
 								bestLj = vbfi(pneg(dL), jpk, bestLj); bestL = pmax(bestL, vL);
 							}
 						}
-						const uint32_t selw = __builtin_amdgcn_perm(wB[hw], wA[hw], SELK);
+						uint32_t selw = 0, profA = 0, profB = 0;
+						(void)selw; (void)profA; (void)profB;
+						if constexpr (PROF) { profA = prof_word_v<kk>(wA[hw], profD); profB = prof_word_v<kk>(wB[hw], profD); }
+						else selw = __builtin_amdgcn_perm(wB[hw], wA[hw], SELK);
 						uint32_t diag = Ad, lraw = Bup, up = 0, cmax[NCH];
 						uint32_t capmask = 0;
 						if constexpr (RAG && MODE == K_GLOBAL) {
@@ -889,8 +965,9 @@
 						(void)jn;
 #pragma unroll
 						for (int r = 0; r < K; ++r) {
-							uint32_t S;
-							if constexpr (BITS == 2) {
+							uint32_t S = 0;
+							if constexpr (PROF) {
+							} else if constexpr (BITS == 2) {
 								S = __builtin_amdgcn_perm(lut_hi, lut_lo, selw ^ qsel[r]);
 							} else {
 								const uint32_t z = pminu(selw ^ qsel[r], c1);
@@ -922,8 +999,12 @@
 								Xl[(k & 1) ^ 1][r] = Mcl;
 								continue;
 							}
-							uint32_t Mraw = padd(diag, S);
-							if constexpr (MODE == K_LOCAL) Mraw = pmax(Mraw, 0u);
+							uint32_t Mraw;
+							if constexpr (PROF) Mraw = prof_m_v(diag, profB, profA, qsel[r], nu2);
+							else {
+								Mraw = padd(diag, S);
+								if constexpr (MODE == K_LOCAL) Mraw = pmax(Mraw, 0u);
+							}
 							const uint32_t Mc = TB ? vandor(Mraw, cClean, cTagM) : Mraw;
 							const uint32_t Lc = !TB ? lraw : X3 ? vandor(lraw, cClean, cTagL) : (lraw | cTagL);
 							const uint32_t Uraw = pmax(Mo_l[r], padd(U_l[r], e2));
@@ -1232,7 +1313,7 @@
 				}
 				long long st_a = 0;
 				if (AT_TP_STATS) { st_a = (long long)__builtin_amdgcn_s_memtime(); ++st_rounds; }
-				replay16_block<MODE, G, K, TS, SMALL, BITS, CK>(a, mem, gs, refoff, qA, qB, l1A, l1B, blk_bl[0], blk_c[0], blk_bl[1], blk_c[1]);
+				replay16_block<MODE, G, K, TS, SMALL, BITS, CK, PROF>(a, mem, gs, refoff, qA, qB, l1A, l1B, blk_bl[0], blk_c[0], blk_bl[1], blk_c[1]);
 				asm volatile("s_waitcnt vmcnt(0)" ::: "memory");
 				if (AT_TP_STATS) st_rep += (long long)__builtin_amdgcn_s_memtime() - st_a;
 				__builtin_amdgcn_fence(__ATOMIC_ACQUIRE, "agent");
@@ -1558,16 +1639,16 @@
 	return (g * k + AT_TAIL_G - 1) / AT_TAIL_G < 2 ? 2 : (g * k + AT_TAIL_G - 1) / AT_TAIL_G;
 }
 
-template <int MODE, int G, int K, int TS, bool SMALL, bool PTRLDS, bool TB, bool RAG = false, int BITS = 2, int CK = 0, int SPLIT = 0>
+template <int MODE, int G, int K, int TS, bool SMALL, bool PTRLDS, bool TB, bool RAG = false, int BITS = 2, int CK = 0, int SPLIT = 0, bool PROF = false>
 __global__ __launch_bounds__(64, (CK > 0 && G == 64 ? AT_TP_WAVES64 : AT_WAVES16(G, K))) void at_sweep16(const Sweep16Args a, const Sweep16Args t)
 {
 	if (a.only_if && __builtin_amdgcn_readfirstlane(*a.only_if) != a.only_val) return;
-	long long w = sweep16_items<MODE, G, K, TS, SMALL, PTRLDS, TB, RAG, BITS, CK, SPLIT>(a, (long long)blockIdx.x, 0);
+	long long w = sweep16_items<MODE, G, K, TS, SMALL, PTRLDS, TB, RAG, BITS, CK, SPLIT, PROF>(a, (long long)blockIdx.x, 0);
 	if constexpr (G <= 16 && !RAG && MODE != K_OVERLAP) {
 		if (t.npairs > 0) {
 			constexpr int NGm = 64 / G;
 			const long long nmain = (a.npairs + 2 * NGm - 1) / (2 * NGm);
-			sweep16_items<MODE, AT_TAIL_G, at_tail_k(G, K), TS, SMALL, PTRLDS, TB, false, BITS, CK, SPLIT>(t, w, nmain);
+			sweep16_items<MODE, AT_TAIL_G, at_tail_k(G, K), TS, SMALL, PTRLDS, TB, false, BITS, CK, SPLIT, PROF>(t, w, nmain);
 		}
 	}
 }
```
